# NCAR/SPERR

Hardware: AMD Instinct MI355X
Metric: compress+decompress GB/s/GPU on 256^3 fp32 chunks @ BPP=2.0; bitstream-exact vs ref (higher is better)
Workload: dtype f64; 1 GPU; synthetic 1024^3 fp32 turbulence per GPU, 256^3 chunks, BPP=2.0, step = compress + decompress, volume and container resident in HBM; chunks_per_gpu=64, parallelism=chunks farmed over 1 GPU(s), no collective

## Files before the change

sperr_amd/csrc/engine.hip:

```cpp
#include <algorithm>
#include <array>
#include <chrono>
#include <cstdlib>
#include <cstring>
#include <atomic>
#include <deque>
#include <map>
#include <memory>
#include <condition_variable>
#include <mutex>
#include <numeric>
#include <thread>
#include <string>
#include <vector>

#include "../../include/sperr_hip.h"
#include "engine_internal.h"
#include "host_container.hpp"
#include "speck_dec.h"
#include "dequant.h"
#include "speck_enc.h"
#include "speck_tree_host.hpp"
#include "outlier.h"
#include "quality.h"
// ... 87 lines not shown

void prof_begin(const char* name, hipStream_t stream)
{
  Profiler* P = t_prof;
  if (!P || !P->on || (!P->only.empty() && P->only != name))
    return;
  std::lock_guard<std::mutex> lock(P->mu);
  if (!P->ref) {
    P->ref = P->get();
    if (P->ref)
      hipEventRecord(P->ref, stream);
  }
  t_prof_cur = name;
  t_prof_a = P->get();
  if (t_prof_a)
    hipEventRecord(t_prof_a, stream);
}

void prof_end(hipStream_t stream)
{
  Profiler* P = t_prof;
  if (!P || !P->on || !t_prof_cur)
    return;
  std::lock_guard<std::mutex> lock(P->mu);
  hipEvent_t b = P->get();
  if (b)
    hipEventRecord(b, stream);
  P->open.push_back({t_prof_cur, t_prof_a, b});
  t_prof_cur = nullptr;
}

thread_local bool t_shared_device = false;

namespace {

struct DevBuf {
  void* p = nullptr;
  size_t n = 0;
  void drop()
  {
    if (p)
      (void)hipFree(p);
    p = nullptr;
    n = 0;
  }
  int ensure(size_t bytes)
  {
    if (bytes <= n)
      return 0;
    if (p)
      (void)hipFree(p);
    p = nullptr;
    n = 0;
    size_t want = bytes < (size_t(256) << 20) ? bytes + bytes / 4 + 4096 : bytes;
    if (want != bytes && hipMalloc(&p, want) != hipSuccess) {
      (void)hipGetLastError();
      p = nullptr;
      want = bytes;
    }
    if (!p)
      HIP_CHECK(hipMalloc(&p, want));
    n = want;
    return 0;
  }
};

std::atomic<unsigned long long> g_dbg_counter[4];

struct Arena {
  char* base = nullptr;
  size_t cap = 0, used = 0;
  template <typename T>
  T* take(size_t count)
  {
    if (used > cap || count > (cap - used) / sizeof(T))
      return nullptr;
    const size_t bytes = (count * sizeof(T) + 255) / 256 * 256;
    if (bytes > cap - used)
      return nullptr;
    T* r = reinterpret_cast<T*>(base + used);
    used += bytes;
    return r;
  }
};

inline uint64_t bytes_of_bits(uint64_t bits)
{
  return bits / 8 + (bits % 8 != 0);
}

size_t round_up(size_t v, size_t m)
{
  return (v + m - 1) / m * m;
}

using hostc::Dims;
using hostc::chunk_count;
using hostc::box_chunks;
using hostc::chunk_volume;
using hostc::ContainerInfo;
using hostc::parse_container_host;
using hostc::keep_portion;

uint32_t condi_num_strides(size_t len)
{
  const size_t dflt = 2048;
  if (len % dflt == 0)
    return (uint32_t)dflt;
  for (size_t n = dflt; n <= 32768; n++)
    if (len % n == 0)
      return (uint32_t)n;
  size_t n = dflt;
  while (len % n != 0)
    n--;
  return (uint32_t)n;
}

struct LiftPass {
  int axis;
  uint32_t region[3];
};

struct ShapePlan {
  uint32_t dims[3];
  uint32_t N = 0;
  spk::HostTree ht;
  spk::Tree dtree{};
  DevBuf tables;
  const uint64_t* d_initLIS = nullptr;
  const uint32_t* d_initLen = nullptr;
  const uint32_t* d_levelOff = nullptr;
  const uint16_t* d_tileLevel = nullptr;
  const uint32_t* d_tileStart = nullptr;
  const uint32_t* d_levelFirstTile = nullptr;
  const uint32_t* d_levelNumTiles = nullptr;
  const uint32_t* d_depthBlocks = nullptr;
  const uint8_t* d_levelSlot = nullptr;
  const uint64_t* d_iRoots = nullptr;
  const uint8_t* d_slotLevel = nullptr;
  const spk::LevelClass* d_levelClass = nullptr;
  const uint32_t* d_wordLeaf = nullptr;
  const FusedRoot* d_fusedRoots = nullptr;
  const uint8_t* d_mxSlot = nullptr;
  const uint8_t* d_mxLevelGroup = nullptr;
  int l0Level = -1;
  int l1Level = -1;
  int l2Level = -1;
  int maxK = 0;
  std::vector<uint32_t> depthBlockOff;
  uint32_t nListTiles = 0, nSlots = 0, nPixTiles = 0, nstrides = 0;
  uint64_t maxPhaseBits = 0;
  size_t lisEntries = 0;
  std::vector<LiftPass> fwd;
};
bool use_tables(const ShapePlan& P);


std::vector<FusedRoot> fused_head_roots(const spk::HostTree& h)
{
  std::vector<FusedRoot> out;
  const uint32_t dx = h.dims[0], dy = h.dims[1], dz = h.dims[2];
  if (!(h.flags & spk::kTreeAllOct) || (h.flags & spk::kTree2D) || h.roots.empty() || h.roots.size() > (size_t)spk::kMaxRoots)
    return out;
  if ((dx & (dx - 1)) != 0 || dx < 8 || dx > (uint32_t)kPixTile / 2 || ((size_t)dx * dy) % kPixTile != 0 || dz % 2 != 0)
    return out;
  uint64_t covered = 0;
  for (const spk::Root& r : h.roots) {
    const spk::Grid& g = h.grids[r.gridFirst + r.Dmax - 1];
    const uint32_t side = r.len[0];
    if (!(g.kind & spk::kGridOct) || g.e[0] < 2 || g.e[1] != g.e[0] || g.e[2] != g.e[0] || r.org[0] % 8 != 0 ||
        r.org[1] % 2 != 0 || r.org[2] % 2 != 0 || r.len[1] != side || r.len[2] != side || side != (2u << g.e[0]))
      return std::vector<FusedRoot>();
    out.push_back(FusedRoot{(uint32_t)r.org[0] | ((uint32_t)r.org[1] << 16), (uint32_t)r.org[2] | (side << 16), g.nodeOff, g.e[0]});
    covered += (uint64_t)side * side * side;
  }
  if (covered != (uint64_t)dx * dy * dz)
    return std::vector<FusedRoot>();
  return out;
}

struct Blob {
  std::vector<char> bytes;
  template <typename T>
  size_t add(const std::vector<T>& v)
  {
    const size_t off = round_up(bytes.size(), 256);
    bytes.resize(off + std::max<size_t>(v.size(), 1) * sizeof(T), 0);
    if (!v.empty())
      memcpy(bytes.data() + off, v.data(), v.size() * sizeof(T));
    return off;
  }
};

int build_plan(ShapePlan& P, size_t dx, size_t dy, size_t dz, bool twoD = false)
{
  const unsigned __int128 samples = (unsigned __int128)dx * dy * dz;
  if (dx == 0 || dy == 0 || dz == 0 || dx > 0xffff || dy > 0xffff || dz > 0xffff || samples > (1ull << 31)) {
    fprintf(stderr, "[sperr_hip] chunk of %zu x %zu x %zu not supported (at most 65535 per axis, 2^31 samples)\n",
            dx, dy, dz);
    return -1;
  }
  P.dims[0] = (uint32_t)dx;
  P.dims[1] = (uint32_t)dy;
  P.dims[2] = (uint32_t)dz;
  P.N = (uint32_t)(dx * dy * dz);
  P.ht = spk::build_tree(dx, dy, dz, twoD, false);
  P.maxK = 0;
  for (const auto& lc : P.ht.levelClass)
    P.maxK = std::max<int>(P.maxK, lc.K);
  if (!use_tables(P))
    spk::build_mx_columns(P.ht);
  const spk::HostTree& h = P.ht;
  const uint32_t nlev = h.nlevels;

  std::vector<uint32_t> cap(nlev), levelOff(nlev + 1, 0), initLen(nlev);
  for (uint32_t l = 0; l < nlev; l++) {
    cap[l] = std::max<uint32_t>(h.levelCap[l], (uint32_t)h.initLIS[l].size());
    levelOff[l + 1] = levelOff[l] + cap[l];
    initLen[l] = (uint32_t)h.initLIS[l].size();
  }
  P.lisEntries = levelOff[nlev] + 8;
  std::vector<uint64_t> initLIS(levelOff[nlev] ? levelOff[nlev] : 1, 0);
  for (uint32_t l = 0; l < nlev; l++)
    for (size_t k = 0; k < h.initLIS[l].size(); k++)
      initLIS[levelOff[l] + k] = h.initLIS[l][k];

  std::vector<uint16_t> tileLevel;
  std::vector<uint32_t> tileStart, levelFirstTile(nlev, 0), levelNumTiles(nlev, 0);
  for (uint32_t l = nlev; l-- > 0;) {
    levelFirstTile[l] = (uint32_t)tileLevel.size();
    const uint32_t nt = (cap[l] + kListTile - 1) / kListTile;
    levelNumTiles[l] = nt;
    for (uint32_t t = 0; t < nt; t++) {
      tileLevel.push_back((uint16_t)l);
      tileStart.push_back(t * kListTile);
    }
  }
  P.nListTiles = (uint32_t)tileLevel.size();

  std::vector<uint32_t> depthBlocks;
  P.depthBlockOff.assign(h.maxDepth + 1, 0);
  for (uint32_t d = 0; d < h.maxDepth; d++) {
    P.depthBlockOff[d] = (uint32_t)depthBlocks.size();
    for (uint32_t b = 0; b < h.blockGrid.size(); b++)
      if (h.grids[h.blockGrid[b]].depth == d)
        depthBlocks.push_back(b);
  }
  P.depthBlockOff[h.maxDepth] = (uint32_t)depthBlocks.size();

  std::vector<uint8_t> levelSlot(nlev, 0xff), slotLevel;
  for (uint32_t l = 0; l < nlev; l++)
    if (cap[l]) {
      levelSlot[l] = (uint8_t)slotLevel.size();
      slotLevel.push_back((uint8_t)l);
    }
  P.nSlots = (uint32_t)slotLevel.size();
  P.maxPhaseBits = (uint64_t)h.nsets + 2ull * P.N + 64;
  P.nPixTiles = (P.N + kPixTile - 1) / kPixTile;
  P.nstrides = condi_num_strides(P.N);

  std::vector<uint32_t> wordLeaf;
  for (const spk::Root& r : h.roots) {
    const spk::Grid& g = h.grids[r.gridFirst + r.Dmax - 1];
    if (!(g.kind & spk::kGridLeafWord))
      continue;
    if (wordLeaf.empty())
      wordLeaf.assign((P.N + 63) / 64, 0xffffffffu);
    for (uint32_t z = 0; z < r.len[2]; z++)
      for (uint32_t y = 0; y < r.len[1]; y++)
        for (uint32_t x = 0; x < r.len[0]; x += 64) {
          const size_t idx = ((size_t)(r.org[2] + z) * dy + r.org[1] + y) * dx + r.org[0] + x;
          const uint32_t fid = g.nodeOff + ((((z / 2) << g.e[1]) + y / 2) << g.e[0]) + x / 2;
          wordLeaf[idx / 64] = fid | (y & 1u) | ((z & 1u) << 1);
        }
  }

  Blob blob;
  const size_t oRoots = blob.add(h.roots), oGrids = blob.add(h.grids), oTab = blob.add(h.tab),
               oBG = blob.add(h.blockGrid), oInit = blob.add(initLIS), oInitLen = blob.add(initLen),
               oLevOff = blob.add(levelOff), oTL = blob.add(tileLevel), oTS = blob.add(tileStart),
               oLFT = blob.add(levelFirstTile), oLNT = blob.add(levelNumTiles),
               oDB = blob.add(depthBlocks), oLS = blob.add(levelSlot), oSL = blob.add(slotLevel),
               oLC = blob.add(h.levelClass), oWL = blob.add(wordLeaf), oCls = blob.add(h.cls),
               oGC = blob.add(h.gridCls), oIR = blob.add(h.iRoots),
               oMS = blob.add(h.mxSlot), oMG = blob.add(h.mxLevelGroup);
  const std::vector<FusedRoot> fusedRoots = twoD ? std::vector<FusedRoot>() : fused_head_roots(h);
  const size_t oFR = blob.add(fusedRoots);
  P.maxK = 0;
  for (const auto& lc : h.levelClass)
    P.maxK = std::max<int>(P.maxK, lc.K);
  P.l0Level = -1;
  for (uint32_t l = nlev; l-- > 0;) {
    if (cap[l] == 0)
      continue;
    if (h.allRegular && h.levelClass[l].regular && h.levelClass[l].K == 1 &&
        h.levelClass[l].arity[0] == 8)
      P.l0Level = (int)l;
    break;
  }
  P.l1Level = -1;
  if (P.l0Level >= 0)
    for (uint32_t l = (uint32_t)P.l0Level; l-- > 0;) {
      if (cap[l] == 0)
        continue;
      const spk::LevelClass& lc = h.levelClass[l];
      if (lc.regular && lc.K == 2 && lc.arity[0] == 8 && lc.arity[1] == 8 &&
          lc.lev[0] == (uint8_t)P.l0Level)
        P.l1Level = (int)l;
      break;
    }
  P.l2Level = -1;
  static const bool l2Env = !(getenv("SPERR_HIP_LIS_L2") && atoi(getenv("SPERR_HIP_LIS_L2")) == 0);
  if (P.l1Level >= 0 && l2Env)
    for (uint32_t l = (uint32_t)P.l1Level; l-- > 0;) {
      if (cap[l] == 0)
        continue;
      const spk::LevelClass& lc = h.levelClass[l];
      if (lc.regular && lc.K == 3 && lc.arity[0] == 8 && lc.arity[1] == 8 && lc.arity[2] == 8 &&
          lc.lev[0] == (uint8_t)P.l0Level && lc.lev[1] == (uint8_t)P.l1Level)
        P.l2Level = (int)l;
      break;
    }
  if (P.tables.ensure(blob.bytes.size()))
    return -1;
  HIP_CHECK(hipMemcpy(P.tables.p, blob.bytes.data(), blob.bytes.size(), hipMemcpyHostToDevice));
  char* base = static_cast<char*>(P.tables.p);
  P.dtree = h.view();
  P.dtree.roots = reinterpret_cast<const spk::Root*>(base + oRoots);
  P.dtree.grids = reinterpret_cast<const spk::Grid*>(base + oGrids);
  P.dtree.tab = reinterpret_cast<const uint16_t*>(base + oTab);
  P.dtree.blockGrid = reinterpret_cast<const uint16_t*>(base + oBG);
  P.dtree.cls = reinterpret_cast<const spk::ShapeCls*>(base + oCls);
  P.dtree.gridCls = reinterpret_cast<const uint8_t*>(base + oGC);
  P.d_mxSlot = reinterpret_cast<const uint8_t*>(base + oMS);
  P.d_mxLevelGroup = reinterpret_cast<const uint8_t*>(base + oMG);
  P.d_iRoots = h.iRoots.empty() ? nullptr : reinterpret_cast<const uint64_t*>(base + oIR);
  P.d_initLIS = reinterpret_cast<const uint64_t*>(base + oInit);
  P.d_initLen = reinterpret_cast<const uint32_t*>(base + oInitLen);
  P.d_levelOff = reinterpret_cast<const uint32_t*>(base + oLevOff);
  P.d_tileLevel = reinterpret_cast<const uint16_t*>(base + oTL);
  P.d_tileStart = reinterpret_cast<const uint32_t*>(base + oTS);
  P.d_levelFirstTile = reinterpret_cast<const uint32_t*>(base + oLFT);
  P.d_levelNumTiles = reinterpret_cast<const uint32_t*>(base + oLNT);
  P.d_depthBlocks = reinterpret_cast<const uint32_t*>(base + oDB);
  P.d_levelSlot = reinterpret_cast<const uint8_t*>(base + oLS);
  P.d_slotLevel = reinterpret_cast<const uint8_t*>(base + oSL);
  P.d_levelClass = reinterpret_cast<const spk::LevelClass*>(base + oLC);
  P.d_wordLeaf = wordLeaf.empty() ? nullptr : reinterpret_cast<const uint32_t*>(base + oWL);
  P.d_fusedRoots = fusedRoots.empty() ? nullptr : reinterpret_cast<const FusedRoot*>(base + oFR);

  P.fwd.clear();
  size_t levels = 0;
  auto approx = [](size_t len, size_t lev) { return (uint32_t)spk::approx_detail_len(len, lev)[0]; };
  if (spk::can_use_dyadic({dx, dy, dz}, levels)) {
    for (size_t lev = 0; lev < levels; lev++) {
      LiftPass ps{0, {approx(dx, lev), approx(dy, lev), approx(dz, lev)}};
      for (int a = 0; a < 3; a++) {
        ps.axis = a;
        P.fwd.push_back(ps);
      }
    }
  }
  else {
    const size_t nz = spk::num_of_xforms(dz), nxy = spk::num_of_xforms(std::min(dx, dy));
    for (size_t lev = 0; lev < nz; lev++)
      P.fwd.push_back({2, {(uint32_t)dx, (uint32_t)dy, approx(dz, lev)}});
    for (size_t lev = 0; lev < nxy; lev++) {
      P.fwd.push_back({0, {approx(dx, lev), approx(dy, lev), (uint32_t)dz}});
      P.fwd.push_back({1, {approx(dx, lev), approx(dy, lev), (uint32_t)dz}});
    }
  }
  return 0;
}

constexpr uint32_t kSubStreams = 8;

struct Engine {
  int dev = -1;
  bool busy = false;
  bool ready = false;
  Profiler prof;
  hipStream_t sub[kSubStreams] = {};
  hipEvent_t evFork = nullptr, evJoin[kSubStreams] = {};
  hipStream_t outl = nullptr;
  hipStream_t outlQ[kSubStreams] = {};
  hipStream_t sideQ[kSubStreams] = {};
  hipEvent_t evOutl[kSubStreams] = {}, evOutlFork[kSubStreams] = {};
  hipEvent_t evPweFork = nullptr;
  hipEvent_t evPweJoin = nullptr;
  std::map<Dims, std::unique_ptr<ShapePlan>> plans;
  std::vector<Dims> planOrder;
  DevBuf arena, slots, misc;
  DevBuf outlFixed, outlVar, outlStream;
  DevBuf pweBox;
  hipStream_t pweLastStream = nullptr;
  DevBuf outlDec[kSubStreams];
  DevBuf decBox[kSubStreams];
  uint32_t* liveHost[kSubStreams] = {};
  void* pweHost = nullptr;
  size_t pweHostBytes = 0;
  hipEvent_t liveEv[kSubStreams][kLiveSlots] = {};
  DevBuf wideScratch;
  std::vector<std::unique_ptr<DevBuf>> pweBufs;
  size_t freeMemAtInit = 0;

  int init()
  {
    if (ready)
      return 0;
    const int rc = init_handles();
    if (rc)
      destroy_handles();
    return rc;
  }
  void destroy_handles()
  {
    auto ds = [](hipStream_t& s) { if (s) (void)hipStreamDestroy(s); s = nullptr; };
    auto de = [](hipEvent_t& e) { if (e) (void)hipEventDestroy(e); e = nullptr; };
    for (uint32_t q = 0; q < kSubStreams; q++) {
      ds(sub[q]);
      de(evJoin[q]);
      if (q > 0)
        ds(outlQ[q]);
      ds(sideQ[q]);
      de(evOutl[q]);
      de(evOutlFork[q]);
      if (q == 0) {
        de(evPweFork);
        de(evPweJoin);
      }
      if (liveHost[q])
        (void)hipHostFree(liveHost[q]);
      liveHost[q] = nullptr;
      if (q == 0 && pweHost) {
        (void)hipHostFree(pweHost);
        pweHost = nullptr;
        pweHostBytes = 0;
      }
      for (int k = 0; k < kLiveSlots; k++)
        de(liveEv[q][k]);
    }
    de(evFork);
    ds(outl);
    outlQ[0] = nullptr;
    ready = false;
  }
  int init_handles()
  {
    size_t fr = 0, tot = 0;
    HIP_CHECK(hipMemGetInfo(&fr, &tot));
    freeMemAtInit = fr;
    for (uint32_t q = 0; q < kSubStreams; q++) {
      HIP_CHECK(hipStreamCreateWithFlags(&sub[q], hipStreamNonBlocking));
      HIP_CHECK(hipEventCreateWithFlags(&evJoin[q], hipEventDisableTiming));
    }
    HIP_CHECK(hipEventCreateWithFlags(&evFork, hipEventDisableTiming));
    int prLeast = 0, prGreatest = 0;
    if (hipDeviceGetStreamPriorityRange(&prLeast, &prGreatest) != hipSuccess) {
      (void)hipGetLastError();
      prLeast = prGreatest = 0;
    }
    static const int sidePrio = getenv("SPERR_HIP_SIDE_PRIORITY") ? atoi(getenv("SPERR_HIP_SIDE_PRIORITY")) : 1;
    const int prSide = sidePrio > 0 ? prGreatest : sidePrio < 0 ? prLeast : 0;
    HIP_CHECK(hipStreamCreateWithPriority(&outl, hipStreamNonBlocking, prSide));
    outlQ[0] = outl;
    for (uint32_t q = 1; q < kSubStreams; q++)
      HIP_CHECK(hipStreamCreateWithPriority(&outlQ[q], hipStreamNonBlocking, prSide));
    for (uint32_t q = 0; q < kSubStreams; q++)
      HIP_CHECK(hipStreamCreateWithFlags(&sideQ[q], hipStreamNonBlocking));
    for (uint32_t q = 0; q < kSubStreams; q++) {
      HIP_CHECK(hipEventCreateWithFlags(&evOutl[q], hipEventDisableTiming));
      HIP_CHECK(hipEventCreateWithFlags(&evOutlFork[q], hipEventDisableTiming));
    }
    HIP_CHECK(hipEventCreateWithFlags(&evPweFork, hipEventDisableTiming));
    HIP_CHECK(hipEventCreateWithFlags(&evPweJoin, hipEventDisableTiming));
    for (uint32_t q = 0; q < kSubStreams; q++) {
      HIP_CHECK(hipHostMalloc(reinterpret_cast<void**>(&liveHost[q]), kLiveSlots * sizeof(uint32_t), hipHostMallocDefault));
      for (int k = 0; k < kLiveSlots; k++)
        HIP_CHECK(hipEventCreateWithFlags(&liveEv[q][k], hipEventDisableTiming));
    }
    ready = true;
    return 0;
  }

  static constexpr size_t kMaxPlans = 64;
  ShapePlan* plan(size_t dx, size_t dy, size_t dz)
  {
    const Dims key{dx, dy, dz};
    auto it = plans.find(key);
    if (it != plans.end()) {
      auto pos = std::find(planOrder.begin(), planOrder.end(), key);
      if (pos != planOrder.end())
        planOrder.erase(pos);
      planOrder.push_back(key);
      return it->second.get();
    }
    auto p = std::make_unique<ShapePlan>();
    if (dz == 0 ? build_plan(*p, dx, dy, 1, true) : build_plan(*p, dx, dy, dz))
      return nullptr;
    ShapePlan* raw = p.get();
    plans[key] = std::move(p);
    planOrder.push_back(key);
    return raw;
  }
  void drop_memory()
  {
    for (auto& kv : plans)
      kv.second->tables.drop();
    plans.clear();
    planOrder.clear();
    for (DevBuf* b : {&arena, &slots, &misc, &outlFixed, &outlVar, &outlStream, &pweBox, &wideScratch})
      b->drop();
    for (auto& b : outlDec)
      b.drop();
    for (auto& b : decBox)
      b.drop();
    for (auto& b : pweBufs)
      if (b)
        b->drop();
    pweBufs.clear();
  }
  size_t device_bytes() const
  {
    size_t n = 0;
// ... 496 lines not shown
  memset(&e, 0, sizeof(e));
  e.tree = P.dtree;
  e.nchunks = B;
#define TAKE(dst, T, count)                                                            \
  dst = A.take<T>((size_t)(count));                                                    \
  if (!dst)                                                                            \
    return false;                                                                      \
  if (arena_debug())                                                                   \
    fprintf(stderr, "[sperr_hip] arena %-18s %10.2f MB\n", #dst, (double)((size_t)(count) * sizeof(T)) / 1048576.0);
  TAKE(e.cst, CoderState, B);
  TAKE(e.st, EncState, B);
  TAKE(o.geom, ChunkGeom, B);
  TAKE(o.gids, uint32_t, B);
  o.valsStride = Npad;
  TAKE(o.vals, double, Npad * B);
  o.strideMeanStride = round_up(std::max<size_t>(P.nstrides, P.N / 4096 + 2), 32);
  TAKE(o.strideMean, double, o.strideMeanStride * B);
  e.coefStride = Npad;
  TAKE(o.coef32, uint32_t, Npad * B);
  e.coef = o.coef32;
  e.signStride = Npad / 64;
  uint64_t* sign;
  TAKE(sign, uint64_t, e.signStride * B);
  e.sign = sign;
  e.pixStride = Npad;
  TAKE(o.msb, int8_t, Npad * B);
  e.msb = o.msb;
  TAKE(e.bplane, int8_t, Npad * B);
  {
    Arena over;
    over.base = reinterpret_cast<char*>(o.vals);
    over.cap = alias ? Npad * B * sizeof(double) : 0;
    const size_t before = A.used;
    o.fusedHead = enc_fused_head(P);
    if (!carve_enc_coder(over, &A, P, B, e, o.fusedHead))
      return false;
    o.aliased = over.used != 0;
    o.coderBytes = over.used + (A.used - before);
    if (arena_debug())
      fprintf(stderr, "[sperr_hip] arena %-18s %10.2f MB, %.2f MB of them over o.vals\n", "coder arrays",
              (double)o.coderBytes / 1048576.0, (double)over.used / 1048576.0);
  }
  e.lisStride = P.lisEntries;
  TAKE(e.lis[0], uint64_t, P.lisEntries * B);
  e.levelOff = P.d_levelOff;
  e.nListTiles = P.nListTiles;
  e.tileLevel = P.d_tileLevel;
  e.tileStart = P.d_tileStart;
  e.levelFirstTile = P.d_levelFirstTile;
  e.levelNumTiles = P.d_levelNumTiles;
  e.tileStride = round_up(P.nListTiles, 32);
  TAKE(e.tileBits, uint64_t, e.tileStride * B);
  TAKE(e.tileSurv, uint32_t, e.tileStride * B);
  TAKE(e.tileBitsOff, uint64_t, e.tileStride * B);
  TAKE(e.tileSurvOff, uint32_t, e.tileStride * B);
  e.iRoots = P.d_iRoots;
  e.iLevels = P.ht.iLevels;
  e.levelSlot = P.d_levelSlot;
  e.slotLevel = P.d_slotLevel;
  e.nSlots = P.nSlots;
  e.maskWords = (uint32_t)maskWords;
  e.maskStride = (size_t)P.nSlots * maskWords;
  TAKE(e.mask, uint64_t, std::max<size_t>(e.maskStride, 1) * B);
  e.prefWords = (uint32_t)((maskWords + 3) / 4);
  e.prefStride = (size_t)P.nSlots * e.prefWords;
  TAKE(e.maskPrefix, uint32_t, std::max<size_t>(e.prefStride, 1) * B);
  e.nPixTiles = P.nPixTiles;
  e.pixCntStride = (size_t)kMaxPlanes * 2 * P.nPixTiles;
  TAKE(e.pixCnt, uint32_t, e.pixCntStride * B);
  TAKE(e.pixOff, uint32_t, e.pixCntStride * B);
  e.streamStride = streamWords;
  TAKE(e.stream, uint64_t, streamWords * B);
#undef TAKE
  return true;
}

size_t enc_bytes_for(const ShapePlan& P, uint32_t B, uint64_t raw_budget, bool alias = true)
{
  Arena probe;
  probe.base = reinterpret_cast<char*>(uintptr_t(4096));
  probe.cap = ~size_t(0) / 2;
  EncBatchBufs tmp;
  carve_enc(probe, P, std::max<uint32_t>(B, 1), raw_budget, tmp, alias);
  return probe.used;
}
size_t enc_bytes_per_chunk(const ShapePlan& P, uint64_t raw_budget, bool alias = true)
{
  return enc_bytes_for(P, 1, raw_budget, alias);
}

int reset_enc_pass(hipStream_t st, const EncBatchBufs& bb, uint32_t B, bool fusedHead = false)
{
  const EncBuffers& e = bb.eb;
  if (!fusedHead)
    HIP_CHECK(hipMemsetAsync(e.bplane, 0xff, e.pixStride * B, st));
  HIP_CHECK(hipMemsetAsync(e.M, 0xff, e.nodeStride * B, st));
  HIP_CHECK(hipMemsetAsync(e.mask, 0, std::max<size_t>(e.maskStride, 1) * B * sizeof(uint64_t), st));
  HIP_CHECK(hipMemsetAsync(e.stream, 0, e.streamStride * B * sizeof(uint64_t), st));
  return 0;
}

bool fuse_xy(const ShapePlan& P)
{
  if (P.fwd.size() < 2 || P.fwd[0].axis != 0 || P.fwd[1].axis != 1)
    return false;
  for (int a = 0; a < 3; a++)
    if (P.fwd[0].region[a] != P.dims[a] || P.fwd[1].region[a] != P.dims[a])
      return false;
  return lift_xy_applicable(P.dims);
}

bool fuse_xyz(const ShapePlan& P)
{
  if (!fuse_xy(P) || P.fwd.size() < 3 || P.fwd[2].axis != 2)
    return false;
  for (int a = 0; a < 3; a++)
    if (P.fwd[2].region[a] != P.dims[a])
      return false;
  return lift_xyz_applicable(P.dims);
}

int pass_fuse(const ShapePlan& P, size_t k, uint32_t inner[3])
{
  const LiftPass& ps = P.fwd[k];
  inner[0] = inner[1] = inner[2] = 0;
  for (size_t j = k + 1; j < P.fwd.size(); j++)
    for (int a = 0; a < 3; a++)
      inner[a] = std::max(inner[a], P.fwd[j].region[a]);
  bool nested = k + 1 >= P.fwd.size();
  for (size_t j = k + 1; j < P.fwd.size(); j++)
    nested = nested || (P.fwd[j].region[0] == inner[0] && P.fwd[j].region[1] == inner[1] &&
                        P.fwd[j].region[2] == inner[2]);
  if (!nested)
    return -1;
  bool covers = true;
  for (int a = 0; a < 3; a++)
    covers = covers && inner[a] >= ps.region[a];
  return covers ? 0 : 1;
}

bool plan_fusable(const ShapePlan& P)
{
  if (P.fwd.empty())
    return false;
  uint32_t inner[3];
  for (size_t k = 0; k < P.fwd.size(); k++)
    if (pass_fuse(P, k, inner) < 0)
      return false;
  if (fuse_xy(P) && (pass_fuse(P, 0, inner) != 0 || pass_fuse(P, 1, inner) != 0))
    return false;
  return true;
}

template <typename T>
int float_stages(hipStream_t ss, const ShapePlan& P, EncBatchBufs& bb, uint32_t nb, const uint32_t cd[3],
                 const T* d_src, VolDesc vd, bool orgAligned, bool wantRange)
{
  EncBuffers& e = bb.eb;
  const bool fuse = !P.fwd.empty();
  const int io = std::is_same<T, float>::value ? 1 : 2;
  if (launch_condition<T>(ss, d_src, vd, bb.geom, nb, cd, P.nstrides, bb.strideMean, bb.strideMeanStride,
                          bb.vals, bb.valsStride, e.cst, !fuse, wantRange, orgAligned))
    return -1;
  size_t k0 = 0;
  const bool fuseMax = plan_fusable(P);
  if (fuse_xyz(P)) {
    LiftFuse lf;
    if (fuseMax && pass_fuse(P, 2, lf.inner) > 0)
      lf.mode = 1;
    if (launch_lift_xyz(ss, true, bb.vals, bb.valsStride, nb, cd, e.cst, io, const_cast<T*>(d_src), vd,
                        bb.geom, &lf))
      return -1;
    k0 = 3;
  }
  else if (fuse_xy(P)) {
    if (launch_lift_xy(ss, true, bb.vals, bb.valsStride, nb, cd, e.cst, io, const_cast<T*>(d_src), vd,
                       bb.geom))
      return -1;
    k0 = 2;
  }
  for (size_t k = k0; k < P.fwd.size(); k++) {
    const LiftPass& ps = P.fwd[k];
    LiftFuse lf;
    if (fuseMax && pass_fuse(P, k, lf.inner) > 0)
      lf.mode = 1;
    if (launch_lift(ss, true, bb.vals, bb.valsStride, nb, cd, ps.axis, ps.region, e.cst, k == 0 ? io : 0,
                    const_cast<T*>(d_src), vd, bb.geom, &lf))
      return -1;
  }
  return 0;
}

int unalias_coder(hipStream_t ss, Engine& E, const ShapePlan& P, EncBatchBufs& bb, uint32_t nb)
{
  HIP_CHECK(hipStreamSynchronize(ss));
  if (E.wideScratch.ensure(bb.coderBytes + 4096))
    return -1;
  Arena W;
  W.base = static_cast<char*>(E.wideScratch.p);
  W.cap = E.wideScratch.n;
  if (!carve_enc_coder(W, nullptr, P, nb, bb.eb))
    return -1;
  bb.aliased = false;
  return 0;
}

template <typename T>
int wide_retry_prepare(hipStream_t ss, Engine& E, const ShapePlan& P, EncBatchBufs& bb, uint32_t nb,
                       const uint32_t cd[3], const T* d_src, VolDesc vd, bool orgAligned, bool wantRange)
{
  if (unalias_coder(ss, E, P, bb, nb))
    return -1;
  g_dbg_counter[0]++;
  return float_stages<T>(ss, P, bb, nb, cd, d_src, vd, orgAligned, wantRange);
}

int psnr_q_search(hipStream_t st, const ShapePlan& P, EncBatchBufs& bb, uint32_t nb, double psnr,
                  std::vector<CoderState>& hc, std::vector<CoderState>& got)
{
  EncBuffers& e = bb.eb;
  hc.assign(nb, CoderState{});
  HIP_CHECK(hipMemcpyAsync(hc.data(), e.cst, nb * sizeof(CoderState), hipMemcpyDeviceToHost, st));
  HIP_CHECK(hipStreamSynchronize(st));
  std::vector<double> tmse(nb, 0.0);
  bool any = false;
  for (uint32_t i = 0; i < nb; i++) {
    CoderState& c = hc[i];
    c.mse_active = 0;
    if (c.is_const)
      continue;
    const double vmax = order_key_value(c.vmaxKey), vmin = -order_key_value(c.vnegmaxKey);
    const double range = (vmax - c.mean) - (vmin - c.mean);
    tmse[i] = (range * range) * std::pow(10.0, -psnr / 10.0);
    c.q = 2.0 * std::sqrt(tmse[i] * 3.0);
    if (!(c.q > 0.0))
      return -1;
    c.mse_active = 1;
    any = true;
  }
  const double step = std::exp2(0.25);
  while (any) {
    HIP_CHECK(hipMemcpyAsync(e.cst, hc.data(), nb * sizeof(CoderState), hipMemcpyHostToDevice, st));
    if (launch_mse(st, bb.vals, bb.valsStride, nb, P.N, bb.strideMean, bb.strideMeanStride, e.cst))
      return -1;
    got.assign(nb, CoderState{});
    HIP_CHECK(hipMemcpyAsync(got.data(), e.cst, nb * sizeof(CoderState), hipMemcpyDeviceToHost, st));
    HIP_CHECK(hipStreamSynchronize(st));
    any = false;
    for (uint32_t i = 0; i < nb; i++) {
      if (!hc[i].mse_active)
        continue;
      if (got[i].mse > tmse[i]) {
        hc[i].q /= step;
        any = true;
      }
      else
        hc[i].mse_active = 0;
    }
  }
  for (uint32_t i = 0; i < nb; i++) {
    CoderState& c = hc[i];
    c.mse_active = 0;
    c.wide = 0;
    c.need_retry = 0;
    if (c.is_const)
      continue;
    const double m = c.maxabs / c.q;
    if (!(m < 0x1p63))
      return -1;
    c.need_retry = std::llrint(m) > (long long)0xffffffffll ? 1u : 0u;
  }
  HIP_CHECK(hipMemcpyAsync(e.cst, hc.data(), nb * sizeof(CoderState), hipMemcpyHostToDevice, st));
  HIP_CHECK(hipStreamSynchronize(st));
  return 0;
}

struct HostMarks {
  bool on = getenv("SPERR_HIP_TIMING") != nullptr;
  std::chrono::steady_clock::time_point t0 = std::chrono::steady_clock::now();
  void mark(const char* what, hipStream_t st)
  {
    if (!on)
      return;
    (void)hipStreamSynchronize(st);
    const auto t1 = std::chrono::steady_clock::now();
    fprintf(stderr, "[sperr_hip] %-28s %8.2f ms\n", what,
            std::chrono::duration<double, std::milli>(t1 - t0).count());
    t0 = t1;
  }
};

int pwe_q_setup(hipStream_t st, EncBatchBufs& bb, uint32_t nb, double tol, std::vector<CoderState>& hc, bool* anyWide = nullptr)
{
  EncBuffers& e = bb.eb;
  hc.assign(nb, CoderState{});
  HIP_CHECK(hipMemcpyAsync(hc.data(), e.cst, nb * sizeof(CoderState), hipMemcpyDeviceToHost, st));
  HIP_CHECK(hipStreamSynchronize(st));
  for (uint32_t i = 0; i < nb; i++) {
    CoderState& c = hc[i];
    c.wide = 0;
    c.need_retry = 0;
    if (c.is_const)
      continue;
    c.q = 1.5 * tol;
    const double m = c.maxabs / c.q;
    if (!(m < 0x1p63))
      return -1;
    c.need_retry = std::llrint(m) > (long long)0xffffffffll ? 1u : 0u;
    if (anyWide && c.need_retry)
      *anyWide = true;
  }
  HIP_CHECK(hipMemcpyAsync(e.cst, hc.data(), nb * sizeof(CoderState), hipMemcpyHostToDevice, st));
  return 0;
}

struct PweKeep {
  void* mem = nullptr;
  uint32_t nb = 0;
  uint32_t* gids = nullptr;
  uint64_t* slotOff = nullptr;
  uint8_t* slots = nullptr;
  std::vector<uint64_t> off2;
};
using PweKeepList = std::vector<PweKeep>;

void speck1d_level_offsets(OutlierBufs& ob, uint32_t N, uint64_t most)
{
  ob.nlists = (uint32_t)spk::num_of_partitions(N) + 1;
  uint64_t off = 0;
  for (uint32_t l = 0; l <= (uint32_t)kO1MaxLevels; l++) {
    ob.levelOff[l] = (uint32_t)std::min<uint64_t>(off, 0xffffffffull);
    if (l < ob.nlists)
      off += l < 40 ? std::min<uint64_t>(1ull << l, most) : most;
  }
  ob.runStride = round_up((size_t)off + 64, 64);
}

struct PweStage {
  OutlierBufs ob;
  std::vector<OutlierChunk> hoc;
  std::vector<ChunkGeom> bricks;
  HostMarks hm;
};
static DequantSrc enc_dequant_src(const EncBatchBufs& bb, bool wide)
{
  DequantSrc s;
  s.coef = wide ? static_cast<const void*>(bb.vals) : bb.coef32;
  s.coefStride = wide ? bb.valsStride : bb.eb.coefStride;
  s.sign = bb.eb.sign;
  s.signStride = bb.eb.signStride;
  return s;
}
template <typename T>
int pwe_stage_begin(hipStream_t st, Engine& E, const ShapePlan& P, EncBatchBufs& bb, uint32_t nb,
                    const T* d_src, VolDesc vd, const uint32_t cd[3], double tol, bool anyWide, PweStage& S)
{
  EncBuffers& e = bb.eb;
  HostMarks& hm = S.hm;
  OutlierBufs& ob = S.ob;
  std::vector<OutlierChunk>& hoc = S.hoc;
  std::vector<ChunkGeom>& bricks = S.bricks;
  if (E.pweLastStream) {
    HIP_CHECK(hipStreamSynchronize(E.pweLastStream));
    E.pweLastStream = nullptr;
  }
  hm.mark("(3D coder done)", st);
  bricks.assign(nb, ChunkGeom{});
// ... 753 lines not shown
    d_bytes = reinterpret_cast<uint8_t*>(d_at + arr / 8);
    std::vector<uint8_t> hdr(at[nvol]);
    HIP_CHECK(hipMemcpyAsync(d_off, off.data(), nvol * 8, hipMemcpyHostToDevice, st));
    HIP_CHECK(hipMemcpyAsync(d_len, need.data(), nvol * 8, hipMemcpyHostToDevice, st));
    HIP_CHECK(hipMemcpyAsync(d_at, at.data(), nvol * 8, hipMemcpyHostToDevice, st));
    LAUNCH_K(k_gather_bytes, dim3(4, std::min<uint32_t>(n, 65535u)), dim3(kThreads), 0, st, d_src, d_off, d_len, d_at,
             d_bytes, n);
    HIP_CHECK(hipMemcpyAsync(hdr.data(), d_bytes, hdr.size(), hipMemcpyDeviceToHost, st));
    HIP_CHECK(hipStreamSynchronize(st));
    for (size_t v = 0; v < nvol; v++) {
      size_t nd = 0;
      if (need[v] && parse_container_host(hdr.data() + at[v], need[v], len[v], ci[v], &nd) != 0)
        return -1;
    }
  }
  return 0;
}

int read_batch_info(Engine& E, const uint8_t* d_src, const size_t* offs, size_t nvol, ContainerInfo& all,
                    std::vector<std::array<size_t, 6>>& list, hipStream_t st)
{
  std::vector<ContainerInfo> ci;
  std::vector<uint8_t> heads;
  if (read_batch_headers(E, d_src, offs, nvol, ci, heads, st))
    return -1;
  const Dims vol = ci[0].vol;
  for (size_t v = 1; v < nvol; v++)
    if (ci[v].vol != vol)
      return -1;
  if (nvol > 0xffffffffull / vol[2] || ci[0].nvals > SIZE_MAX / 8 / nvol)
    return -1;
  all.vol = {vol[0], vol[1], vol[2] * nvol};
  all.chunk = ci[0].chunk;
  all.nvals = ci[0].nvals * nvol;
  all.off.clear();
  all.len.clear();
  list.clear();
  for (size_t v = 0; v < nvol; v++) {
    const auto per = chunk_volume(ci[v].vol, ci[v].chunk);
    if (per.size() != ci[v].off.size() || list.size() + per.size() > 0xffffffffull)
      return -1;
    for (size_t i = 0; i < per.size(); i++) {
      auto c = per[i];
      c[4] += v * vol[2];
      list.push_back(c);
      all.off.push_back(offs[v] + ci[v].off[i]);
      all.len.push_back(ci[v].len[i]);
    }
  }
  return 0;
}

int trunc_impl(Engine& E, const uint8_t* d_src, const size_t* offs, size_t nvol, unsigned pct, uint8_t* d_dst,
               size_t dst_cap, size_t* outOffs, hipStream_t st)
{
  std::vector<ContainerInfo> ci;
  std::vector<uint8_t> heads;
  if (read_batch_headers(E, d_src, offs, nvol, ci, heads, st))
    return -1;
  const bool whole = pct == 0 || pct >= 100;
  size_t npieces = 0, hdrBytes = 0;
  for (const ContainerInfo& c : ci) {
    npieces += 1 + c.len.size();
    hdrBytes += (c.multi ? 20 : 14) + 4 * c.len.size();
  }
  if (npieces >= 0xffffffffull)
    return -1;
  const size_t addrBytes = round_up(npieces * 8, 256), offBytes = round_up((npieces + 1) * 8, 256);
  if (E.misc.ensure(addrBytes + offBytes + hdrBytes + 256))
    return -1;
  uint8_t* d_up = static_cast<uint8_t*>(E.misc.p);
  std::vector<uint8_t> up(addrBytes + offBytes + hdrBytes, 0);
  uint64_t* srcAddr = reinterpret_cast<uint64_t*>(up.data());
  uint64_t* outOff = reinterpret_cast<uint64_t*>(up.data() + addrBytes);
  uint8_t* hdr = up.data() + addrBytes + offBytes;
  size_t k = 0, hat = 0;
  uint64_t out = 0;
  for (size_t v = 0; v < nvol; v++) {
    const ContainerInfo& c = ci[v];
    const size_t pos = c.multi ? 20 : 14, hlen = pos + 4 * c.len.size();
    uint8_t* h = hdr + hat;
    memcpy(h, heads.data() + v * 32, pos);
    if (!whole) {
      h[0] = 0;
      h[1] |= 0x80;
    }
    outOffs[v] = (size_t)out;
    srcAddr[k] = reinterpret_cast<uint64_t>(d_up + addrBytes + offBytes + hat);
    outOff[k++] = out;
    out += hlen;
    for (size_t i = 0; i < c.len.size(); i++) {
      const uint32_t keep = (uint32_t)hostc::portion_len((size_t)c.len[i], pct);
      memcpy(h + pos + 4 * i, &keep, 4);
      srcAddr[k] = reinterpret_cast<uint64_t>(d_src + offs[v] + c.off[i]);
      outOff[k++] = out;
      out += keep;
    }
    hat += hlen;
  }
  outOff[k] = out;
  outOffs[nvol] = (size_t)out;
  if (!d_dst || out > dst_cap)
    return 1;
  const uintptr_t s0 = reinterpret_cast<uintptr_t>(d_src) + offs[0], s1 = reinterpret_cast<uintptr_t>(d_src) + offs[nvol];
  const uintptr_t d0 = reinterpret_cast<uintptr_t>(d_dst), d1 = d0 + out;
  if (s0 < d1 && d0 < s1)
    return -1;
  const uint64_t nblocks = (out + kTruncSlice - 1) / kTruncSlice;
  if (nblocks > 0x7fffffffull)
    return -1;
  HIP_CHECK(hipMemcpyAsync(d_up, up.data(), up.size(), hipMemcpyHostToDevice, st));
  LAUNCH_K(k_trunc_container, dim3((uint32_t)nblocks), dim3(kThreads), 0, st, d_dst,
           reinterpret_cast<const uint64_t*>(d_up), reinterpret_cast<const uint64_t*>(d_up + addrBytes), (uint32_t)npieces,
           out);
  HIP_CHECK(hipGetLastError());
  HIP_CHECK(hipStreamSynchronize(st));
  E.prof.collect();
  return 0;
}

bool g_lis_stamps_on = false;
constexpr int kHiMaxK = 9;
bool use_lis_hi(const ShapePlan& P, bool tables)
{
  static const bool hiEnv = !(getenv("SPERR_HIP_LIS_HI") && atoi(getenv("SPERR_HIP_LIS_HI")) == 0);
  return hiEnv && tables && P.ht.grids.size() <= 288 && P.ht.roots.size() <= 48 &&
         P.maxK >= 1 && P.maxK <= kHiMaxK;
}
bool use_tables(const ShapePlan& P)
{
  if (!P.ht.allRegular || P.maxK < 1)
    return false;
  return use_lis_hi(P, true);
}
bool use_mixed(const ShapePlan& P)
{
  static const bool mixEnv = !(getenv("SPERR_HIP_LIS_MIXED") && atoi(getenv("SPERR_HIP_LIS_MIXED")) == 0);
  const bool twoD = (P.ht.flags & spk::kTree2D) != 0;
  if ((!twoD && !mixEnv) || use_tables(P) || P.ht.cls.empty() || P.ht.roots.size() > 48 || P.ht.grids.size() > 352 ||
      P.ht.mxSlot.size() != P.ht.cls.size())
    return false;
  return 2 * kMxS + 256 <= kMxRing && ((kMxS + kMxM) >> 6) + 5 <= 64 && kMxM >= 192 &&
         mx_smem_bytes(kMxS, kMxM, kMxQ) <= 138u * 1024u;
}
std::vector<uint64_t> g_lis_stamps_host;

struct DecBatchBufs {
  DecBuffers db;
  ChunkGeom* geom;
  CropGeom* crop;
  uint64_t *chunkOff, *chunkLen;
  double* vals;
  size_t valsStride;
  uint32_t* coef32;
  uint32_t* live;
};

bool carve_dec(Arena& A, const ShapePlan& P, uint32_t B, uint64_t maxPayloadBytes, DecBatchBufs& o,
               size_t valsElems = 0, uint32_t refNPlanes = 0, bool crop = false)
{
  const size_t N = P.N, Npad = round_up(N, 512);
  DecBuffers& d = o.db;
  memset(&d, 0, sizeof(d));
  d.tree = P.dtree;
  d.treeTabLen = (uint32_t)P.ht.tab.size();
  d.nchunks = B;
#define TAKE(dst, T, count)                                                            \
  dst = A.take<T>((size_t)(count));                                                    \
  if (!dst)                                                                            \
    return false;                                                                      \
  if (arena_debug())                                                                   \
    fprintf(stderr, "[sperr_hip] arena %-18s %10.2f MB\n", #dst, (double)((size_t)(count) * sizeof(T)) / 1048576.0);
  TAKE(d.cst, CoderState, B);
  TAKE(d.st, DecState, B);
  TAKE(o.geom, ChunkGeom, B);
  o.crop = nullptr;
  if (crop) {
    TAKE(o.crop, CropGeom, B);
  }
  TAKE(o.chunkOff, uint64_t, B);
  TAKE(o.chunkLen, uint64_t, B);
  TAKE(o.live, uint32_t, 64);
  o.valsStride = valsElems ? round_up(valsElems, 256) : Npad;
  TAKE(o.vals, double, o.valsStride * B);
  d.coefStride = Npad;
  TAKE(o.coef32, uint32_t, Npad * B);
  d.coef = o.coef32;
  d.signStride = Npad / 64;
  TAKE(d.sign, uint64_t, d.signStride * B);
  d.maskPixStride = Npad / 64;
  d.refPlanes = nullptr;
  d.refMask = nullptr;
  d.wordTop = nullptr;
  d.refNPlanes = 0;
  d.refPlaneStride = d.wordTopStride = 0;
  if (refNPlanes) {
    d.refNPlanes = std::min<uint32_t>(refNPlanes, 32u);
    d.refPlaneStride = d.coefStride / 2;
    d.wordTopStride = round_up(d.maskPixStride, 64);
    d.refPlanes = reinterpret_cast<uint64_t*>(o.coef32);
    TAKE(d.refMask, uint64_t, d.maskPixStride * B);
    TAKE(d.wordTop, uint8_t, d.wordTopStride * B);
  }
  TAKE(d.bornM, uint64_t, d.maskPixStride * B);
  TAKE(d.sigOld, uint64_t, d.maskPixStride * B);
  TAKE(d.sigNew, uint64_t, d.maskPixStride * B);
  d.lisStride = P.lisEntries;
  TAKE(d.lis[0], uint64_t, P.lisEntries * B);
  TAKE(d.lis[1], uint64_t, P.lisEntries * B);
  d.levelOff = P.d_levelOff;
  d.nPixTiles = (uint32_t)((Npad / 64 + kThreads - 1) / kThreads);
  d.tileStride = round_up(d.nPixTiles, 32);
  TAKE(d.tileLip, uint32_t, d.tileStride * B);
  TAKE(d.tileRef, uint32_t, d.tileStride * B);
  TAKE(d.tileLipOff, uint32_t, d.tileStride * B);
  TAKE(d.tileRefOff, uint32_t, d.tileStride * B);
  {
    uint8_t* tb = nullptr;
    TAKE(tb, uint8_t, d.tileStride * B);
    d.tileBorn = use_tables(P) ? tb : nullptr;
  }
  d.lipResStride = Npad / 64 + 2;
  TAKE(d.lipSig, uint64_t, d.lipResStride * B);
  TAKE(d.lipNeg, uint64_t, d.lipResStride * B);
  d.tokStride = (2 * N + 1 + 63) / 64 + 2;
  TAKE(d.tokMask, uint64_t, d.tokStride * B);
  TAKE(d.tokCnt, uint32_t, d.tokStride * B);
  TAKE(d.tokOff, uint32_t, d.tokStride * B);
  d.tokSegStride = round_up(d.tokStride / 2048 + 2, 32);
  TAKE(d.tokSegSum, uint32_t, d.tokSegStride * B);
  TAKE(d.tokSegBase, uint32_t, d.tokSegStride * B);
  d.streamStride = (size_t)(maxPayloadBytes / 8) + 4;
  TAKE(d.stream, uint64_t, d.streamStride * B);
  d.levelClass = P.d_levelClass;
  d.levelSlot = P.d_levelSlot;
  d.slotLevel = P.d_slotLevel;
  d.nSlots = P.nSlots;
  d.maskWords = (uint32_t)d.streamStride;
  d.maskStride = (size_t)P.nSlots * d.maskWords;
  TAKE(d.mask, uint64_t, std::max<size_t>(d.maskStride, 1) * B);
  d.prefWords = (d.maskWords + 3u) / 4u;
  d.prefStride = (size_t)P.nSlots * d.prefWords;
  TAKE(d.maskPrefix, uint32_t, std::max<size_t>(d.prefStride, 1) * B);
  d.bornStride = P.ht.nsets + 8;
  d.hiGroupsMax = 8;
  d.bornSeg = (uint32_t)((P.ht.nsets + 8) / 16 + 64);
  d.bornPitch = d.bornStride + (size_t)d.bornSeg * d.hiGroupsMax;
  TAKE(d.bornPacked, uint64_t, d.bornPitch * B);
  TAKE(d.bornPosLev, uint64_t, d.bornPitch * B);
  d.lisStamps = nullptr;
  if (g_lis_stamps_on) {
    TAKE(d.lisStamps, uint64_t, 64 * B);
  }
  d.queueCap = 28672 + 64;
  static const int hiKcap = tune_getenv("SPERR_HIP_HI_KCAP") ? std::max(2, atoi(tune_getenv("SPERR_HIP_HI_KCAP"))) : 5;
  d.hiK = (uint32_t)std::min(std::max(2, P.maxK), hiKcap);
  static const uint32_t ahead = tune_getenv("SPERR_HIP_HI_AHEAD") ? (uint32_t)atoi(tune_getenv("SPERR_HIP_HI_AHEAD")) : 512u;
  d.hiAhead = ahead;
  static const uint32_t extra = tune_getenv("SPERR_HIP_HI_EXTRA") ? (uint32_t)atoi(tune_getenv("SPERR_HIP_HI_EXTRA")) : 1u;
  d.hiExtra = extra;
  d.hiHop2 = 0;
  d.hiCand = 1;
  d.hiSmemBytes = 148 * 1024;
  d.hiW = hi_window((int)d.hiK, d.hiSmemBytes, d.hiHop2);
  d.queueStride = (size_t)d.queueCap * 4 * d.hiGroupsMax;
  TAKE(d.queue, uint64_t, d.queueStride * B);
  d.hiAhead = std::min(d.hiAhead / 64 * 64, d.hiW / 2);
  d.hiFlagStride = ((d.streamStride * 64 + N) / std::max<uint32_t>(512u, d.hiW - d.hiAhead) + 12) * 4;
  d.mxSlot = P.d_mxSlot;
  d.mxLevelGroup = P.d_mxLevelGroup;
  d.mxS = kMxS;
  d.mxM = kMxM;
  d.mxQ = kMxQ;
  d.mxSmemBytes = mx_smem_bytes(kMxS, kMxM, kMxQ);
  if (use_mixed(P))
    d.hiFlagStride = std::max<size_t>(d.hiFlagStride, ((d.streamStride * 64 + N) / kMxS + 4) * kMxWordsPerRegion);
  TAKE(d.hiFlags, unsigned long long, d.hiFlagStride * B);
  d.iRoots = P.d_iRoots;
  d.iLevels = P.ht.iLevels;
  d.leafCap = P.ht.nsets + 8;
  d.leafSeg = (uint32_t)((P.ht.nsets + 8) / 16 + 64);
  d.leafStride = d.leafCap + (size_t)d.leafSeg * d.hiGroupsMax;
  TAKE(d.leafEv, uint64_t, d.leafStride * B);
  d.sigbitsStride = P.lisEntries / 64 + 4;
  TAKE(d.sigbits, uint64_t, d.sigbitsStride * B);
  d.l0FlagStride = (d.streamStride * 64 + N) / 4096 + 4;
  TAKE(d.l0Flags, unsigned long long, d.l0FlagStride * B);
  TAKE(d.l0Tab, unsigned long long, d.l0FlagStride * 17 * B);
  d.l0Level = P.l0Level;
  TAKE(d.l1Flags, unsigned long long, d.l0FlagStride * B);
  d.l1Level = P.l1Level;
  TAKE(d.l2Flags, unsigned long long, d.l0FlagStride * B);
  d.l2Level = P.l2Level;
  d.wordLeaf = P.d_wordLeaf;
  d.leafStateStride = round_up(P.ht.nnodes, 64);
  TAKE(d.leafState, uint16_t, d.leafStateStride * B);
  d.leafDirtyStride = d.leafStateStride / 32 + 1;
  TAKE(d.leafDirty, uint8_t, d.leafDirtyStride * B);
#undef TAKE
  return true;
}

int reset_dec_call(const DecBuffers& d, uint32_t nb, hipStream_t ss)
{
  HIP_CHECK(hipMemsetAsync(d.cst, 0, nb * sizeof(CoderState), ss));
  HIP_CHECK(hipMemsetAsync(d.st, 0, nb * sizeof(DecState), ss));
  HIP_CHECK(hipMemsetAsync(d.mask, 0, std::max<size_t>(d.maskStride, 1) * nb * 8, ss));
  HIP_CHECK(hipMemsetAsync(d.l0Flags, 0, d.l0FlagStride * nb * 8, ss));
  HIP_CHECK(hipMemsetAsync(d.l0Tab, 0, d.l0FlagStride * 17 * nb * 8, ss));
  HIP_CHECK(hipMemsetAsync(d.l1Flags, 0, d.l0FlagStride * nb * 8, ss));
  HIP_CHECK(hipMemsetAsync(d.l2Flags, 0, d.l0FlagStride * nb * 8, ss));
  HIP_CHECK(hipMemsetAsync(d.hiFlags, 0, d.hiFlagStride * nb * 8, ss));
  HIP_CHECK(hipMemsetAsync(d.sigbits, 0, d.sigbitsStride * nb * 8, ss));
  if (d.lisStamps)
    HIP_CHECK(hipMemsetAsync(d.lisStamps, 0, 64 * 8 * nb, ss));
  return 0;
}

int reset_dec_pass(const DecBatchBufs& bb, uint32_t nb, bool wide, hipStream_t ss)
{
  const DecBuffers& d = bb.db;
  HIP_CHECK(hipMemsetAsync(d.bornM, 0, d.maskPixStride * nb * 8, ss));
  if (d.tileBorn)
    HIP_CHECK(hipMemsetAsync(d.tileBorn, 0, d.tileStride * nb, ss));
  HIP_CHECK(hipMemsetAsync(d.sigOld, 0, d.maskPixStride * nb * 8, ss));
  HIP_CHECK(hipMemsetAsync(d.sigNew, 0, d.maskPixStride * nb * 8, ss));
  HIP_CHECK(hipMemsetAsync(d.sign, 0xff, d.signStride * nb * 8, ss));
  HIP_CHECK(hipMemsetAsync(d.leafState, 0, d.leafStateStride * nb * 2, ss));
  HIP_CHECK(hipMemsetAsync(d.leafDirty, 0, d.leafDirtyStride * nb, ss));
  HIP_CHECK(hipMemsetAsync(d.stream, 0, d.streamStride * nb * 8, ss));
  if (wide)
    HIP_CHECK(hipMemsetAsync(bb.vals, 0, bb.valsStride * nb * 8, ss));
  else if (d.refPlanes)
    HIP_CHECK(hipMemsetAsync(d.wordTop, 0, d.wordTopStride * nb, ss));
  else
    HIP_CHECK(hipMemsetAsync(bb.coef32, 0, d.coefStride * nb * 4, ss));
  return 0;
// ... 59 lines not shown
  std::vector<uint32_t> ids;
  bool crop = false;
  bool level = false;
  size_t h = 0;
  MultiRes m;
  void place(const uint32_t org[3], const uint32_t cd[3], size_t o[3], size_t ext[3]) const
  {
    for (int a = 0; a < 3; a++) {
      ext[a] = level ? m.cres[h][a] : cd[a];
      o[a] = level ? org[a] / cd[a] * ext[a] : org[a];
    }
  }
  CropGeom crop_geom(const size_t o[3], const size_t ext[3]) const
  {
    CropGeom g;
    for (int a = 0; a < 3; a++) {
      const size_t hi = lo[a] + dims[a];
      g.rel[a] = (int32_t)((int64_t)o[a] - (int64_t)lo[a]);
      g.lo[a] = (uint32_t)(lo[a] > o[a] ? lo[a] - o[a] : 0);
      g.hi[a] = (uint32_t)std::min<size_t>(hi - o[a], ext[a]);
    }
    return g;
  }
};

bool window_select(const Dims& full, const Dims& chunk, const size_t lo[3], const size_t dims[3], Window& w)
{
  for (int a = 0; a < 3; a++) {
    if (dims[a] > (size_t)INT32_MAX)
      return false;
    w.lo[a] = lo[a];
    w.dims[a] = dims[a];
  }
  w.crop = !(w.lo == Dims{0, 0, 0} && w.dims == full);
  return box_chunks(full, chunk, w.lo, w.dims, w.ids);
}

__global__ void __launch_bounds__(kThreads)
k_dequant_corner(double* vals, size_t valsStride, uint32_t bx, uint32_t by, uint32_t cx, uint32_t cy, uint32_t sx,
                 uint32_t sy, uint32_t sz, const CoderState* cst, DequantSrc Q)
{
  const uint32_t c = blockIdx.y;
  const CoderState& cs = cst[c];
  if (cs.is_const || cs.wide)
    return;
  const uint32_t i = blockIdx.x * kThreads + threadIdx.x;
  if (i >= sx * sy * sz)
    return;
  const uint32_t x = i % sx, r = i / sx;
  const uint32_t y = r % sy, z = r / sy;
  const size_t idx = ((size_t)z * cy + y) * cx + x;
  const DequantRule<uint32_t> rule = dequant_rule<uint32_t>(cs.q, true, Q.dst + c, Q.coefSigned != 0);
  const uint32_t v = Q.coefs<uint32_t>(c)[idx];
  double out;
  if (rule.scheme)
    out = dequant_signed(rule, v);
  else {
    const uint32_t w = (uint32_t)(idx >> 6), sh = (uint32_t)(idx & 63);
    const uint64_t sgw = Q.sign[c * Q.signStride + w];
    const uint64_t mnw = Q.sigNew[c * Q.maskStride + w], mow = Q.sigOld[c * Q.maskStride + w];
    out = dequant_masks(rule, v, mnw, mow, sgw, sh);
  }
  vals[c * valsStride + ((size_t)z * by + y) * bx + x] = out;
}

template <typename OT, bool kCrop>
__global__ void __launch_bounds__(kThreads)
k_level_write(const double* vals, size_t valsStride, const CoderState* cst, const GeomOf<kCrop>* geom, uint32_t bx,
              uint32_t by, uint32_t cdx, uint32_t cdy, uint32_t cdz, uint32_t sx, uint32_t sy, uint32_t sz,
              VolDesc vd, OT* out)
{
  const uint32_t c = blockIdx.y;
  const uint32_t n = sx * sy * sz, i0 = blockIdx.x * kThreads;
  const GeomOf<kCrop> g = geom[c];
  if constexpr (kCrop) {
    const uint32_t r0 = i0 / sx, r1 = (min(i0 + (uint32_t)kThreads, n) - 1) / sx;
    const uint32_t z0 = r0 / sy, y0 = r0 % sy, z1 = r1 / sy, y1 = r1 % sy;
    auto zin = [&](uint32_t z) { return z >= g.lo[2] && z < g.hi[2]; };
    auto ymeet = [&](uint32_t a, uint32_t b) { return a < g.hi[1] && b >= g.lo[1]; };
    bool any = zin(z0) && ymeet(y0, z1 > z0 ? sy - 1 : y1);
    any = any || (z1 > z0 && zin(z1) && ymeet(0, y1));
    any = any || (max(z0 + 1, g.lo[2]) < min(z1, g.hi[2]));
    if (!any)
      return;
  }
  const uint32_t i = i0 + threadIdx.x;
  if (i >= n)
    return;
  const uint32_t x = i % sx, r = i / sx;
  const uint32_t y = r % sy, z = r / sy;
  size_t o;
  if constexpr (kCrop) {
    if (x < g.lo[0] || x >= g.hi[0] || y < g.lo[1] || y >= g.hi[1] || z < g.lo[2] || z >= g.hi[2])
      return;
    o = ((size_t)((int64_t)g.rel[2] + z) * vd.dims[1] + (size_t)((int64_t)g.rel[1] + y)) * vd.dims[0] +
        (size_t)((int64_t)g.rel[0] + x);
  }
  else
    o = (((size_t)(g.org[2] / cdz) * sz + z) * vd.dims[1] + (size_t)(g.org[1] / cdy) * sy + y) * vd.dims[0] +
        (size_t)(g.org[0] / cdx) * sx + x;
  const CoderState& cs = cst[c];
  const double v = cs.is_const ? cs.mean : vals[c * valsStride + ((size_t)z * by + y) * bx + x] + cs.mean;
  out[o] = (OT)v;
}

struct DecodeRequest {
  using ChunkList = std::vector<std::array<size_t, 6>>;
  const ChunkList* stacked = nullptr;
  bool slices = false;
  const uint32_t* sliceHdr = nullptr;
  const Window* window = nullptr;
  const MultiRes* levels = nullptr;

  void set_window(const Window& w) { window = (w.level || w.crop) ? &w : nullptr; }

  bool valid() const
  {
    if (window && slices)
      return false;
    if (window && levels)
      return false;
    if (stacked && levels)
      return false;
    if (level() && stacked)
      return false;
    if (level() && level()->h >= level()->m.nlev)
      return false;
    return true;
  }

  const Window* level() const { return window && window->level ? window : nullptr; }
  bool cropped() const { return window && window->crop; }
  bool reads_outliers() const { return !level(); }
  ChunkList chunks(const ContainerInfo& ci) const { return stacked ? *stacked : chunk_volume(ci.vol, ci.chunk); }
  std::vector<uint32_t> slots(size_t nchunks) const
  {
    if (window)
      return window->ids;
    std::vector<uint32_t> sel(nchunks);
    std::iota(sel.begin(), sel.end(), 0u);
    return sel;
  }
  VolDesc out_desc(const ContainerInfo& ci) const
  {
    return window ? VolDesc{{window->dims[0], window->dims[1], window->dims[2]}}
                  : VolDesc{{ci.vol[0], ci.vol[1], ci.vol[2]}};
  }
  size_t out_vals(const ContainerInfo& ci) const
  {
    return window ? window->dims[0] * window->dims[1] * window->dims[2] : ci.nvals;
  }
};

size_t dec_bytes_per_chunk(const ShapePlan& P, uint64_t maxPayload, size_t valsElems, uint32_t refNPlanes, bool crop)
{
  Arena probe;
  probe.base = reinterpret_cast<char*>(uintptr_t(4096));
  probe.cap = ~size_t(0) / 2;
  DecBatchBufs tmp;
  carve_dec(probe, P, 1, maxPayload, tmp, valsElems, refNPlanes, crop);
  return probe.used;
}

DecPlanHost dec_plan_host(const ShapePlan& P)
{
  DecPlanHost ph{P.d_initLIS, P.d_initLen, use_tables(P), P.l0Level >= 0 && P.ht.grids.size() <= 288,
                 P.l1Level >= 0 && P.ht.grids.size() <= 288, P.maxK};
  ph.l2 = ph.l1 && P.l2Level >= 0;
  ph.hi = use_lis_hi(P, ph.tables);
  ph.mixed = use_mixed(P);
  return ph;
}

template <typename T>
struct DecodeCall {
  struct Ref {
    uint32_t gid;
    uint32_t slot;
    uint32_t org[3];
  };
  struct OutHead {
    bool has = false;
    uint64_t off = 0, total_bits = 0;
    int nbp = 0;
  };
  struct SubHost {
    std::vector<ChunkGeom> hg, bricks;
    std::vector<CropGeom> hc;
    std::vector<uint64_t> ho, hl;
    std::vector<DecState> hs;
    std::vector<OutlierChunk> hoc;
    DecBatchBufs bb;
    OutlierBufs ob;
    uint32_t nb = 0;
    size_t first = 0;
    int maxNarrow = 0, maxWide = 0;
    bool outliers = false;
  };
  struct Batch {
    const std::vector<Ref>* refs;
    ShapePlan* P;
    uint32_t cbox[3], refNPlanes, nsub = 1;
    uint64_t maxPayload = 0;
    size_t compactElems;
    bool deferG, fuseDq;
    hipStream_t deferStream = nullptr;
    std::vector<SubHost>* subs = nullptr;
    int devId = 0;
  };
  Engine& E;
  const uint8_t* d_src;
  T* d_dst;
  const ContainerInfo& ci;
  hipStream_t st;
  const DecodeRequest& req;
  const VolDesc vd = req.out_desc(ci);
  std::vector<uint32_t> sel;
  std::vector<uint64_t> selOff, selLen, tailOff, tailLen;
  std::vector<uint8_t> heads, tails;
  std::vector<OutHead> outHead;
  bool anyOutlier = false;
  std::map<Dims, std::vector<Ref>> groups;
  uint32_t mxGroupsCall = 0;
  std::deque<std::vector<SubHost>> subHosts;
  bool deferOK = false, deferSized = false, deferForked = false;
  std::vector<SubHost*> pending;
  size_t deferOff = 0;
  uint32_t deferNext = 0;
  hipEvent_t timingFork = nullptr;
  std::vector<std::pair<hipEvent_t, std::array<uint32_t, 4>>> timingEnds;
  bool ok = false;
  ~DecodeCall() { if (!ok) drain_after_error(E, st); }
  int run(size_t dst_cap_vals)
  {
    if (!req.valid())
      return -1;
    const auto chunks = req.chunks(ci);
    sel = req.slots(chunks.size());
    const uint32_t nchunks = (uint32_t)sel.size();
    const size_t outVals = req.out_vals(ci);
    if (outVals == 0 || outVals > dst_cap_vals || nchunks == 0)
      return -1;
    for (uint32_t i = 0; i < nchunks; i++) {
      const auto& c = chunks[sel[i]];
      selOff.push_back(ci.off[sel[i]]);
      selLen.push_back(ci.len[sel[i]]);
      groups[Dims{c[1], c[3], c[5]}].push_back({sel[i], i, {(uint32_t)c[0], (uint32_t)c[2], (uint32_t)c[4]}});
    }
    if (read_heads())
      return -1;
    deferOK = !anyOutlier && !req.levels && !req.slices && groups.size() > 1;
    count_mx_groups();
    for (int pass = 0; pass < 2; pass++)
      for (auto& g : groups)
        if (decode_group(g.first, g.second, pass))
          return -1;
    if (drain())
      return -1;
    HIP_CHECK(hipStreamSynchronize(st));
    HIP_CHECK(hipGetLastError());
    E.prof.collect();
    ok = true;
    return 0;
  }
  int read_heads()
  {
    const uint32_t nchunks = (uint32_t)sel.size();
    if (E.misc.ensure(round_up((size_t)nchunks * 8, 256) * 4 + (size_t)nchunks * 64 + 256))
      return -1;
    uint64_t* d_off = reinterpret_cast<uint64_t*>(E.misc.p);
    uint64_t* d_len = d_off + round_up(nchunks, 32);
    uint64_t* d_hoff = d_len + round_up(nchunks, 32);
    uint64_t* d_hlen = d_hoff + round_up(nchunks, 32);
    uint8_t* d_heads = reinterpret_cast<uint8_t*>(d_hlen + round_up(nchunks, 32));
    auto gather = [&](const std::vector<uint64_t>& off, const std::vector<uint64_t>& len, std::vector<uint8_t>& out,
                      bool withHdr) -> int {
      HIP_CHECK(hipMemcpyAsync(d_off, off.data(), nchunks * 8, hipMemcpyHostToDevice, st));
      HIP_CHECK(hipMemcpyAsync(d_len, len.data(), nchunks * 8, hipMemcpyHostToDevice, st));
      LAUNCH_K(k_gather_heads, dim3((nchunks + 63) / 64), dim3(64), 0, st, d_src, d_off, d_len, d_heads, nchunks);
      std::vector<uint64_t> hoff, hlen;
      if (withHdr) {
        hoff.resize(nchunks);
        hlen.assign(nchunks, 10);
        for (uint32_t i = 0; i < nchunks; i++)
          hoff[i] = off[i] - 10;
        HIP_CHECK(hipMemcpyAsync(d_hoff, hoff.data(), nchunks * 8, hipMemcpyHostToDevice, st));
        HIP_CHECK(hipMemcpyAsync(d_hlen, hlen.data(), nchunks * 8, hipMemcpyHostToDevice, st));
        LAUNCH_K(k_gather_heads, dim3((nchunks + 63) / 64), dim3(64), 0, st, d_src, d_hoff, d_hlen,
                 d_heads + (size_t)nchunks * 32, nchunks);
      }
      out.resize((size_t)nchunks * (withHdr ? 64 : 32));
      HIP_CHECK(hipMemcpyAsync(out.data(), d_heads, out.size(), hipMemcpyDeviceToHost, st));
      HIP_CHECK(hipStreamSynchronize(st));
      return 0;
    };
    if (gather(selOff, selLen, heads, req.sliceHdr != nullptr))
      return -1;
    if (const uint32_t* sliceHdr = req.sliceHdr)
      for (uint32_t i = 0; i < nchunks; i++) {
        uint32_t d2[2];
        memcpy(d2, heads.data() + (size_t)(nchunks + i) * 32 + 2, 8);
        if (d2[0] != sliceHdr[0] || d2[1] != sliceHdr[1]) {
          fprintf(stderr, "[sperr_hip] slice %u of the batch: its header says %u x %u, the call %u x %u\n", i, d2[0], d2[1],
                  sliceHdr[0], sliceHdr[1]);
          return -1;
        }
      }
    outHead.resize(nchunks);
    tailOff.assign(nchunks, 0);
    tailLen.assign(nchunks, 0);
    bool anyTail = false;
    if (!req.reads_outliers())
      return 0;
    for (uint32_t i = 0; i < nchunks; i++) {
      const uint8_t* hd = heads.data() + (size_t)i * 32;
      if (selLen[i] < 26 || (hd[0] & 0x01))
        continue;
      uint64_t tb;
      memcpy(&tb, hd + 18, 8);
      const uint64_t speckLen = std::min<uint64_t>(9 + bytes_of_bits(tb), selLen[i] - 17);
      if (17 + speckLen + 9 <= selLen[i]) {
        tailOff[i] = selOff[i] + 17 + speckLen;
        tailLen[i] = selLen[i] - 17 - speckLen;
        anyTail = true;
      }
    }
    if (!anyTail)
      return 0;
    if (gather(tailOff, tailLen, tails, false))
      return -1;
    for (uint32_t i = 0; i < nchunks; i++) {
      if (tailLen[i] < 9)
        continue;
      const uint8_t* t = tails.data() + (size_t)i * 32;
      uint64_t ob;
      memcpy(&ob, t + 1, 8);
      if (tailLen[i] != 9 + bytes_of_bits(ob))
        continue;
      outHead[i].has = true;
      outHead[i].off = tailOff[i];
      outHead[i].total_bits = ob;
      outHead[i].nbp = t[0];
      anyOutlier = true;
    }
    return 0;
  }
  ShapePlan* plan_of(const Dims& d) { return E.plan(d[0], d[1], req.slices ? 0 : d[2]); }
  void count_mx_groups()
  {
    size_t nmx = 0;
    for (auto& h : groups) {
      ShapePlan* Q = plan_of(h.first);
      if (Q && use_mixed(*Q))
        nmx += h.second.size();
    }
    static const uint32_t mxBudget = getenv("SPERR_HIP_MX_WGS") ? (uint32_t)atoi(getenv("SPERR_HIP_MX_WGS")) : 208u;
    size_t sharers = 1;
    int devNow = 0;
    if (hipGetDevice(&devNow) == hipSuccess)
      sharers = std::max<size_t>(1, g_pool.busy_on(devNow));
    if (nmx)
      mxGroupsCall = std::min<uint32_t>(8u, std::max<uint32_t>(2u, (uint32_t)(mxBudget / (nmx * sharers))));
  }
  static bool deferrable(const ShapePlan& P, size_t nchunksOfShape) { return nchunksOfShape < 32 || !use_tables(P); }
  uint32_t ref_planes_of(const ShapePlan& P, const std::vector<Ref>& refs) const
  {
    uint32_t n = 0;
    for (const Ref& r : refs) {
      const uint8_t* hd = heads.data() + (size_t)r.slot * 32;
      if (ci.len[r.gid] >= 26 && !(hd[0] & 0x01) && hd[17] <= 32)
        n = std::max<uint32_t>(n, hd[17]);
    }
    return n;
  }
  size_t compact_box(const ShapePlan& P, const std::vector<Ref>& refs, uint32_t cbox[3]) const
  {
    cbox[0] = cbox[1] = cbox[2] = 0;
    if (!fuse_xyz(P) || !plan_fusable(P) || req.levels || req.slices || anyOutlier || P.fwd.size() < 3)
      return 0;
    for (const Ref& r : refs) {
      const uint8_t* hd = heads.data() + (size_t)r.slot * 32;
      if (ci.len[r.gid] >= 26 && !(hd[0] & 0x01) && hd[17] > 32)
        return 0;
    }
    for (size_t k = 3; k < P.fwd.size(); k++)
      for (int a = 0; a < 3; a++)
        cbox[a] = std::max(cbox[a], P.fwd[k].region[a]);
    for (int a = 0; a < 3; a++)
      cbox[a] = std::max(cbox[a], 1u);
    if (const Window* lvl = req.level())
      for (int a = 0; a < 3; a++)
        cbox[a] = std::max(cbox[a], lvl->m.cres[lvl->h][a]);
    return (size_t)cbox[0] * cbox[1] * cbox[2];
  }
  int size_deferred()
  {
    deferSized = true;
    size_t sum = 0;
    for (auto& h : groups) {
      ShapePlan* Q = E.plan(h.first[0], h.first[1], h.first[2]);
      if (!Q)
        return -1;
      if (!deferrable(*Q, h.second.size()))
        continue;
      uint64_t mp = 0;
      for (auto& r : h.second)
        mp = std::max<uint64_t>(mp, ci.len[r.gid]);
      uint32_t qbox[3];
      sum += round_up(h.second.size() * dec_bytes_per_chunk(*Q, mp, compact_box(*Q, h.second, qbox), ref_planes_of(*Q, h.second), req.cropped()) + (1 << 20), 4096);
    }
    size_t fr = 0, tot = 0;
    HIP_CHECK(hipMemGetInfo(&fr, &tot));
    const size_t room = arena_room(E.arena.n, fr);
    return E.arena.ensure(std::min(sum, room)) ? -1 : 0;
  }
  int decode_group(const Dims& shape, const std::vector<Ref>& refs, int pass)
  {
    ShapePlan* P = plan_of(shape);
    if (!P)
      return -1;
    if (req.slices && !use_mixed(*P)) {
      fprintf(stderr, "[sperr_hip] slice of %u x %u: its forest does not fit k_lis_mx\n", P->dims[0], P->dims[1]);
      return -1;
    }
    Batch b{&refs, P};
    b.deferG = deferOK && deferrable(*P, refs.size());
    if (b.deferG != (pass == 1))
      return 0;
    if (b.deferG && !deferSized && size_deferred())
      return -1;
    for (auto& r : refs)
      b.maxPayload = std::max<uint64_t>(b.maxPayload, ci.len[r.gid]);
    b.compactElems = compact_box(*P, refs, b.cbox);
    b.refNPlanes = ref_planes_of(*P, refs);
    b.fuseDq = plan_fusable(*P) && !req.levels && !req.slices;
    const size_t per = dec_bytes_per_chunk(*P, b.maxPayload, b.compactElems, b.refNPlanes, req.cropped());
    size_t fr = 0, tot = 0;
    HIP_CHECK(hipMemGetInfo(&fr, &tot));
    const size_t budgetBytes = arena_budget(E.arena.n, fr);
    uint32_t B = (uint32_t)std::min<size_t>(refs.size(), std::max<size_t>(1, budgetBytes / per));
    B = std::min<uint32_t>(B, 256);
    const size_t needBytes = (size_t)B * per + (1 << 20);
    if (b.deferG && deferOff + needBytes > E.arena.n && drain())
      return -1;
    if (E.arena.ensure(needBytes))
      return -1;
    for (size_t b0 = 0; b0 < refs.size(); b0 += B) {
      const uint32_t nbAll = (uint32_t)std::min<size_t>(B, refs.size() - b0);
      if (b.deferG && deferOff + needBytes > E.arena.n && drain())
        return -1;
      if (decode_batch(b, b0, nbAll, needBytes))
        return -1;
    }
    return 0;
  }
  int decode_batch(Batch& b, size_t b0, uint32_t nbAll, size_t needBytes)
  {
    Arena A;
    A.base = static_cast<char*>(E.arena.p) + (b.deferG ? deferOff : 0);
    A.cap = E.arena.n - (b.deferG ? deferOff : 0);
    b.deferStream = nullptr;
    if (b.deferG) {
      if (!deferForked) {
        HIP_CHECK(hipEventRecord(E.evFork, st));
        for (uint32_t q = 0; q < kSubStreams; q++)
          HIP_CHECK(hipStreamWaitEvent(E.sub[q], E.evFork, 0));
        HIP_CHECK(hipStreamWaitEvent(E.outlQ[1], E.evFork, 0));
        deferForked = true;
      }
      b.deferStream = (mxGroupsCall != 0 && use_tables(*b.P)) ? E.outlQ[1] : E.sub[deferNext++ % kSubStreams];
      deferOff += round_up(needBytes, 4096);
    }
    if (pick_sub_batches(b, A, b0, nbAll))
      return -1;
    std::vector<SubHost>& subs = *b.subs;
    if (b.nsub == 1) {
      static const bool enqTiming = getenv("SPERR_HIP_ENQ_TIMING") != nullptr;
      const auto tq0 = std::chrono::steady_clock::now();
      if (enqueue(b, 0))
        return -1;
      if (enqTiming) {
        fprintf(stderr, "[sperr_hip] group %u x %u x %u, %u chunks: enqueued in %.2f ms\n", b.P->dims[0], b.P->dims[1], b.P->dims[2], nbAll,
                std::chrono::duration<double, std::milli>(std::chrono::steady_clock::now() - tq0).count());
        hipEvent_t evEnd = nullptr;
        if (b.deferStream && hipEventCreate(&evEnd) == hipSuccess) {
          if (!timingFork && hipEventCreate(&timingFork) == hipSuccess)
            (void)hipEventRecord(timingFork, st);
          (void)hipEventRecord(evEnd, b.deferStream);
          timingEnds.push_back({evEnd, {b.P->dims[0], b.P->dims[1], b.P->dims[2], nbAll}});
        }
      }
      if (b.deferG) {
        pending.push_back(&subs[0]);
        return 0;
      }
    }
    else {
      std::vector<int> rc(b.nsub, 0);
      std::vector<std::thread> workers;
      for (uint32_t q = 0; q < b.nsub; q++)
        workers.emplace_back([&, q]() { rc[q] = enqueue(b, q); });
      for (auto& w : workers)
        w.join();
      for (uint32_t q = 0; q < b.nsub; q++) {
        if (rc[q])
          return -1;
        if (subs[q].nb)
          HIP_CHECK(hipStreamWaitEvent(st, E.evJoin[q], 0));
      }
    }
    return collect_states(b);
  }
  int pick_sub_batches(Batch& b, Arena& A, size_t b0, uint32_t nbAll)
  {
    static const int subEnv = getenv("SPERR_HIP_SUBSTREAMS") ? atoi(getenv("SPERR_HIP_SUBSTREAMS")) : 0;
    uint32_t nsub = nbAll >= 32 ? 2u : 1u;
    int devNow = 0;
    if (!t_shared_device && hipGetDevice(&devNow) == hipSuccess && g_pool.busy_on(devNow) <= 1)
      nsub = nbAll >= 56 ? 3u : nbAll >= 8 ? 4u : nbAll >= 4 ? 2u : 1u;
    if (subEnv > 0)
      nsub = std::min<uint32_t>(kSubStreams, (uint32_t)subEnv);
    if (nbAll < 2 * nsub || b.deferG)
      nsub = 1;
    b.nsub = nsub;
    b.subs = &subHosts.emplace_back(nsub);
    if (nsub > 1) {
      HIP_CHECK(hipEventRecord(E.evFork, st));
      for (uint32_t q = 0; q < nsub; q++)
        HIP_CHECK(hipStreamWaitEvent(E.sub[q], E.evFork, 0));
    }
    uint32_t done = 0;
    for (uint32_t q = 0; q < nsub; q++) {
      SubHost& S = (*b.subs)[q];
      S.nb = (nbAll - done + (nsub - q) - 1) / (nsub - q);
      S.first = b0 + done;
      done += S.nb;
      if (S.nb && !carve_dec(A, *b.P, S.nb, b.maxPayload, S.bb, b.compactElems, b.refNPlanes, req.cropped()))
        return -1;
      if (S.nb && b.compactElems)
        g_dbg_counter[2]++;
    }
    HIP_CHECK(hipGetDevice(&b.devId));
    return 0;
  }
  int enqueue(const Batch& b, uint32_t q)
  {
    SubHost& S = (*b.subs)[q];
    const uint32_t nb = S.nb;
    if (nb == 0)
      return 0;
    if (b.nsub > 1) {
      HIP_CHECK(hipSetDevice(b.devId));
      t_prof = &E.prof;
    }
    const hipStream_t ss = b.deferStream ? b.deferStream : (b.nsub > 1 ? E.sub[q] : st);
    S.hg.resize(nb);
    S.ho.resize(nb);
    S.hl.resize(nb);
    for (uint32_t i = 0; i < nb; i++) {
      const Ref& r = (*b.refs)[S.first + i];
      for (int a = 0; a < 3; a++)
        S.hg[i].org[a] = r.org[a];
      S.ho[i] = ci.off[r.gid];
      S.hl[i] = ci.len[r.gid];
      const uint8_t* hd = heads.data() + (size_t)r.slot * 32;
      if (S.hl[i] >= 26 && !(hd[0] & 0x01)) {
        const int nbp = hd[17];
        if (nbp > 32)
          S.maxWide = std::max(S.maxWide, nbp);
        else
          S.maxNarrow = std::max(S.maxNarrow, nbp);
      }
      S.outliers |= outHead[r.slot].has;
    }
    if (S.maxWide > kMaxPlanes || (b.compactElems && S.maxWide))
      return -1;
    if (enqueue_outlier_decode(b, S, q, ss) || enqueue_lists(b, S, q, ss) || enqueue_inverse(b, S, q, ss))
      return -1;
    if (b.nsub > 1)
      HIP_CHECK(hipEventRecord(E.evJoin[q], ss));
    return 0;
  }
  int enqueue_outlier_decode(const Batch& b, SubHost& S, uint32_t q, hipStream_t ss)
  {
    if (!S.outliers)
      return 0;
    const uint32_t nb = S.nb, N = b.P->N;
    hipStream_t so = E.outlQ[q];
    HIP_CHECK(hipEventRecord(E.evOutlFork[q], ss));
    HIP_CHECK(hipStreamWaitEvent(so, E.evOutlFork[q], 0));
    S.hoc.assign(nb, OutlierChunk{});
    memset(S.hoc.data(), 0, nb * sizeof(OutlierChunk));
    uint64_t maxBits = 0;
    int maxNbp = 1;
    for (uint32_t i = 0; i < nb; i++) {
      const OutHead& oh = outHead[(*b.refs)[S.first + i].slot];
      if (!oh.has)
        continue;
      S.hoc[i].has = 1;
      S.hoc[i].streamOff = oh.off;
      S.hoc[i].total_bits = oh.total_bits;
      S.hoc[i].nbp = oh.nbp;
      if (oh.nbp > kMaxPlanes)
        return -1;
      maxBits = std::max(maxBits, oh.total_bits);
      maxNbp = std::max(maxNbp, oh.nbp);
    }
    OutlierBufs& ob = S.ob;
    memset(&ob, 0, sizeof(ob));
    ob.nchunks = nb;
    ob.N = N;
    ob.nw = (N + 63) / 64;
    ob.wordStride = round_up((size_t)ob.nw + 2, 32);
    ob.kStride = round_up((size_t)std::min<uint64_t>(N, maxBits) + 1, 64);
    speck1d_level_offsets(ob, N, std::min<uint64_t>(maxBits + 2, 2ull * N));
    ob.streamStride = (size_t)(maxBits / 64) + 4;
    ob.planeStride = (size_t)maxNbp * ob.wordStride;
    const size_t bytes = round_up(nb * sizeof(OutlierChunk), 256) +
                         (size_t)nb * (ob.wordStride * 16 + ob.kStride * 5 + ob.runStride * 8 +
                                       ob.streamStride * 8 + ob.planeStride * 8) + 8192;
    if (E.outlDec[q].ensure(bytes))
      return -1;
    Arena OA;
    OA.base = static_cast<char*>(E.outlDec[q].p);
    OA.cap = E.outlDec[q].n;
    ob.oc = OA.take<OutlierChunk>(nb);
    ob.lip = OA.take<uint64_t>(nb * ob.wordStride);
    ob.lsp = OA.take<uint64_t>(nb * ob.wordStride);
    ob.runs = OA.take<uint64_t>(nb * ob.runStride);
    ob.stream = OA.take<uint64_t>(nb * ob.streamStride);
    ob.planeBits = OA.take<uint64_t>(nb * ob.planeStride);
    ob.pos = OA.take<uint32_t>(nb * ob.kStride);
    ob.sgn = OA.take<uint8_t>(nb * ob.kStride);
    if (!ob.oc || !ob.lip || !ob.lsp || !ob.runs || !ob.stream || !ob.planeBits || !ob.pos || !ob.sgn)
      return -1;
    HIP_CHECK(hipMemcpyAsync(ob.oc, S.hoc.data(), nb * sizeof(OutlierChunk), hipMemcpyHostToDevice, so));
    HIP_CHECK(hipMemsetAsync(ob.lip, 0, (size_t)nb * ob.wordStride * 16, so));
    if (launch_speck1d_decode(so, ob, d_src))
      return -1;
    HIP_CHECK(hipEventRecord(E.evOutl[q], so));
    return 0;
  }
  int enqueue_lists(const Batch& b, SubHost& S, uint32_t q, hipStream_t ss)
  {
    const ShapePlan& P = *b.P;
    const uint32_t nb = S.nb;
    DecBatchBufs& bb = S.bb;
    DecBuffers& d = bb.db;
    HIP_CHECK(hipMemcpyAsync(bb.geom, S.hg.data(), nb * sizeof(ChunkGeom), hipMemcpyHostToDevice, ss));
    if (req.cropped()) {
      S.hc.resize(nb);
      for (uint32_t i = 0; i < nb; i++) {
        size_t o[3], ext[3];
        req.window->place(S.hg[i].org, P.dims, o, ext);
        S.hc[i] = req.window->crop_geom(o, ext);
      }
      HIP_CHECK(hipMemcpyAsync(bb.crop, S.hc.data(), nb * sizeof(CropGeom), hipMemcpyHostToDevice, ss));
    }
    HIP_CHECK(hipMemcpyAsync(bb.chunkOff, S.ho.data(), nb * 8, hipMemcpyHostToDevice, ss));
    HIP_CHECK(hipMemcpyAsync(bb.chunkLen, S.hl.data(), nb * 8, hipMemcpyHostToDevice, ss));
    DecPlanHost ph = dec_plan_host(P);
    ph.skipFinish = true;
    ph.mxGroups = mxGroupsCall;
    if (!ph.tables && !ph.mixed) {
      static std::atomic<bool> warned{false};
      if (!warned.exchange(true))
        fprintf(stderr, "[sperr_hip] note: chunks of %u x %u x %u decode through the serial walk (k_lis_walk): their tree "
                        "(%zu grids, %zu roots) exceeds what the parallel list kernels hold in LDS -- expect it to be slow\n",
                b.P->dims[0], b.P->dims[1], b.P->dims[2], P.ht.grids.size(), P.ht.roots.size());
    }
    static const uint32_t gdivEnv = tune_getenv("SPERR_HIP_MX_GRID_DIV") ? (uint32_t)atoi(tune_getenv("SPERR_HIP_MX_GRID_DIV")) : 4u;
    ph.gridDiv = (b.deferStream && mxGroupsCall != 0 && groups.size() >= 4) ? std::max<uint32_t>(1u, gdivEnv) : 1u;
    ph.d_live = !b.deferStream ? bb.live : nullptr;
    ph.h_live = E.liveHost[q % kSubStreams];
    ph.liveEv = E.liveEv[q % kSubStreams];
    static const bool gpuWide = !(getenv("SPERR_HIP_LIS_GPUWIDE") && atoi(getenv("SPERR_HIP_LIS_GPUWIDE")) == 0);
    if (!gpuWide)
      ph.l0 = ph.l1 = ph.l2 = false;
    if (reset_dec_call(d, nb, ss))
      return -1;
    for (int wide = 1; wide >= 0; wide--) {
      if (wide && S.maxWide == 0)
        continue;
      if (reset_dec_pass(bb, nb, wide != 0, ss))
        return -1;
      DecBuffers dw = d;
      if (wide) {
        dw.coef = bb.vals;
        dw.coefStride = bb.valsStride;
        dw.refPlanes = nullptr;
      }
      else
        dw.coefSigned = packed_signs(b, bb, false) ? 1u : 0u;
      if (launch_speck_decode(ss, dw, ph, d_src, bb.chunkOff, bb.chunkLen, wide != 0, wide ? S.maxWide : S.maxNarrow))
        return -1;
      if ((wide || !b.fuseDq) &&
          launch_inv_quantize(ss, wide != 0, dequant_src(b, bb, wide != 0), nb, P.N, bb.vals, bb.valsStride, d.cst))
        return -1;
    }
    return 0;
  }
  DequantSrc dequant_src(const Batch& b, const DecBatchBufs& bb, bool wide) const
  {
    const DecBuffers& d = bb.db;
    DequantSrc s;
    s.coef = wide ? static_cast<const void*>(bb.vals) : bb.coef32;
    s.coefStride = wide ? bb.valsStride : d.coefStride;
    s.sign = d.sign;
    s.signStride = d.signStride;
    s.sigNew = d.sigNew;
    s.sigOld = d.sigOld;
    s.maskStride = d.maskPixStride;
    s.dst = d.st;
    s.coefSigned = packed_signs(b, bb, wide) ? 1 : 0;
    return s;
  }
  static bool packed_signs(const Batch& b, const DecBatchBufs& bb, bool wide) { return !wide && bb.db.refPlanes && b.fuseDq; }
  void pass_dequant(const Batch& b, const DecBatchBufs& bb, size_t k, LiftFuse& lf) const
  {
    if (b.fuseDq && pass_fuse(*b.P, k, lf.inner) > 0) {
      lf.mode = 2;
      lf.src = dequant_src(b, bb, false);
    }
    if (b.compactElems) {
      lf.bufx = b.cbox[0];
      lf.bufy = b.cbox[1];
    }
  }
  int enqueue_inverse(const Batch& b, SubHost& S, uint32_t q, hipStream_t ss)
  {
    if (const Window* lvl = req.level())
      return enqueue_level(b, S, ss, *lvl);
    const ShapePlan& P = *b.P;
    const uint32_t nb = S.nb;
    const uint32_t* cd = P.dims;
    DecBatchBufs& bb = S.bb;
    DecBuffers& d = bb.db;
    const int io = std::is_same<T, float>::value ? 1 : 2;
    const bool fxyz = fuse_xyz(P) && !S.outliers;
    const bool fxy = fuse_xy(P) && !S.outliers && !fxyz;
    const bool fbrick = S.outliers && fuse_xyz(P) && b.fuseDq && S.maxWide == 0 && P.fwd.size() >= 3 &&
                        b.compactElems == 0 && (uint64_t)nb * bb.valsStride <= 0xffffffffull;
    uint32_t bbox[3] = {1, 1, 1};
    double* boxVals = nullptr;
    size_t boxStride = 0;
    ChunkGeom* d_bricks = nullptr;
    if (fbrick) {
      for (size_t k = 3; k < P.fwd.size(); k++)
        for (int a = 0; a < 3; a++)
          bbox[a] = std::max(bbox[a], P.fwd[k].region[a]);
      boxStride = round_up((size_t)bbox[0] * bbox[1] * bbox[2], 64);
      const size_t geomOff = round_up((size_t)nb * boxStride * 8, 256);
      if (E.decBox[q].ensure(geomOff + (size_t)nb * sizeof(ChunkGeom) + 256))
        return -1;
      boxVals = static_cast<double*>(E.decBox[q].p);
      d_bricks = reinterpret_cast<ChunkGeom*>(static_cast<char*>(E.decBox[q].p) + geomOff);
      S.bricks.resize(nb);
      for (uint32_t i = 0; i < nb; i++) {
        S.bricks[i].org[0] = (uint32_t)((size_t)i * bb.valsStride);
        S.bricks[i].org[1] = S.bricks[i].org[2] = 0;
      }
      HIP_CHECK(hipMemcpyAsync(d_bricks, S.bricks.data(), nb * sizeof(ChunkGeom), hipMemcpyHostToDevice, ss));
    }
    const size_t perLevel = req.slices ? 2 : 3;
    auto sub_volume = [&](size_t k) -> int {
      const MultiRes* mr = req.levels;
      if (!mr || !mr->nlev)
        return 0;
      const size_t h = mr->nlev - (k / perLevel + 1);
      const auto& r = mr->cres[h];
      const uint32_t blocks = capped_blocks((r[0] * r[1] * r[2] + kThreads - 1) / kThreads, nb);
      LAUNCH_K(k_sub_volume, dim3(blocks, nb), dim3(kThreads), 0, ss, bb.vals, bb.valsStride, d.cst, bb.geom,
               cd[0], cd[1], cd[0], cd[1], cd[2], r[0], r[1], r[2], mr->grid[0], mr->grid[1], mr->d_level[h]);
      return 0;
    };
    auto dequant_fuse = [&](size_t k, LiftFuse& lf) {
      pass_dequant(b, bb, k, lf);
      if (fbrick) {
        lf.bufx = bbox[0];
        lf.bufy = bbox[1];
      }
    };
    for (size_t k = P.fwd.size(); k-- > ((fxyz || fbrick) ? 3u : fxy ? 2u : 0u);) {
      const LiftPass& ps = P.fwd[k];
      if (k % perLevel == perLevel - 1 && sub_volume(k))
        return -1;
      LiftFuse lf;
      dequant_fuse(k, lf);
      const bool last = k == 0 && !S.outliers;
      if (launch_lift(ss, false, fbrick ? boxVals : bb.vals, fbrick ? boxStride : bb.valsStride, nb, cd, ps.axis,
                      ps.region, d.cst, last ? io : 0, d_dst, vd, bb.geom, &lf, last ? bb.crop : nullptr))
        return -1;
    }
    if (fbrick) {
      LiftFuse lf;
      dequant_fuse(2, lf);
      lf.noMean = 1;
      const VolDesc brickVol{{cd[0], cd[1], cd[2]}};
      if (launch_lift_xyz(ss, false, boxVals, boxStride, nb, cd, d.cst, 2, bb.vals, brickVol, d_bricks, &lf))
        return -1;
    }
    if (fxyz) {
      if (sub_volume(2))
        return -1;
      LiftFuse lf;
      dequant_fuse(2, lf);
      if (launch_lift_xyz(ss, false, bb.vals, bb.valsStride, nb, cd, d.cst, io, d_dst, vd, bb.geom, &lf, bb.crop))
        return -1;
    }
    if (fxy && req.slices && sub_volume(1))
      return -1;
    if (fxy && launch_lift_xy(ss, false, bb.vals, bb.valsStride, nb, cd, d.cst, io, d_dst, vd, bb.geom, bb.crop))
      return -1;
    if (S.outliers) {
      HIP_CHECK(hipStreamWaitEvent(ss, E.evOutl[q], 0));
      if (launch_outlier_apply(ss, S.ob, d.cst, bb.vals, bb.valsStride))
        return -1;
      HIP_CHECK(hipMemcpyAsync(S.hoc.data(), S.ob.oc, nb * sizeof(OutlierChunk), hipMemcpyDeviceToHost, ss));
      HIP_CHECK(hipStreamSynchronize(ss));
      for (auto& o : S.hoc)
        if (o.error) {
          fprintf(stderr, "[sperr_hip] outlier decoder failed (code %u)\n", o.error);
          return -1;
        }
    }
    if ((P.fwd.empty() || S.outliers) &&
        launch_scatter<T>(ss, d_dst, vd, bb.geom, nb, cd, bb.vals, bb.valsStride, d.cst, bb.crop))
      return -1;
    return 0;
  }
  int enqueue_level(const Batch& b, SubHost& S, hipStream_t ss, const Window& lvl)
  {
    const ShapePlan& P = *b.P;
    const uint32_t nb = S.nb;
    const uint32_t* cd = P.dims;
    DecBatchBufs& bb = S.bb;
    DecBuffers& d = bb.db;
    const size_t h = lvl.h, nlev = lvl.m.nlev;
    if (P.fwd.size() != 3 * nlev)
      return -1;
    const uint32_t bx = b.compactElems ? b.cbox[0] : cd[0], by = b.compactElems ? b.cbox[1] : cd[1];
    const auto& r = lvl.m.cres[h];
    if (b.compactElems && (r[0] > b.cbox[0] || r[1] > b.cbox[1] || r[2] > b.cbox[2]))
      return -1;
    for (size_t k = P.fwd.size(); k-- > 3 * (nlev - h);) {
      const LiftPass& ps = P.fwd[k];
      LiftFuse lf;
      pass_dequant(b, bb, k, lf);
      if (launch_lift(ss, false, bb.vals, bb.valsStride, nb, cd, ps.axis, ps.region, d.cst, 0, d_dst, vd, bb.geom, &lf))
        return -1;
    }
    const uint32_t blocks = (r[0] * r[1] * r[2] + kThreads - 1) / kThreads;
    if (h == 0 && b.fuseDq)
      LAUNCH_K(k_dequant_corner, dim3(blocks, nb), dim3(kThreads), 0, ss, bb.vals, bb.valsStride, bx, by, cd[0], cd[1],
               r[0], r[1], r[2], d.cst, dequant_src(b, bb, false));
    if (lvl.crop)
      LAUNCH_K((k_level_write<T, true>), dim3(blocks, nb), dim3(kThreads), 0, ss, bb.vals, bb.valsStride, d.cst, bb.crop,
               bx, by, cd[0], cd[1], cd[2], r[0], r[1], r[2], vd, d_dst);
    else
      LAUNCH_K((k_level_write<T, false>), dim3(blocks, nb), dim3(kThreads), 0, ss, bb.vals, bb.valsStride, d.cst, bb.geom,
               bx, by, cd[0], cd[1], cd[2], r[0], r[1], r[2], vd, d_dst);
    HIP_CHECK(hipGetLastError());
    return 0;
  }
  int collect_states(const Batch& b)
  {
    for (uint32_t q = 0; q < b.nsub; q++) {
      SubHost& S = (*b.subs)[q];
      if (S.nb == 0)
        continue;
      hipStream_t ss = b.nsub > 1 ? E.sub[q] : st;
      if (S.bb.db.lisStamps && q == 0) {
        g_lis_stamps_host.assign(64, 0);
        const uint32_t sc = getenv("SPERR_HIP_STAMP_CHUNK")
                                ? std::min<uint32_t>(S.nb - 1, (uint32_t)atoi(getenv("SPERR_HIP_STAMP_CHUNK")))
                                : 0u;
        HIP_CHECK(hipMemcpyAsync(g_lis_stamps_host.data(), S.bb.db.lisStamps + (size_t)sc * 64, 64 * 8,
                                 hipMemcpyDeviceToHost, ss));
      }
      S.hs.resize(S.nb);
      HIP_CHECK(hipMemcpyAsync(S.hs.data(), S.bb.db.st, S.nb * sizeof(DecState), hipMemcpyDeviceToHost, ss));
    }
    HIP_CHECK(hipStreamSynchronize(st));
    if (b.nsub > 1)
      for (uint32_t q = 0; q < b.nsub; q++)
        HIP_CHECK(hipStreamSynchronize(E.sub[q]));
    for (auto& S : *b.subs)
      for (auto& hsx : S.hs)
        if (hsx.error) {
          report_dec_error(hsx.error);
          return -1;
        }
    return 0;
  }
  int drain()
  {
    int rc = 0;
    for (uint32_t q = 0; q < kSubStreams; q++)
      HIP_CHECK(hipStreamSynchronize(E.sub[q]));
    HIP_CHECK(hipStreamSynchronize(E.outlQ[1]));
    for (auto& te : timingEnds) {
      float ms = 0.f;
      if (timingFork && hipEventElapsedTime(&ms, timingFork, te.first) == hipSuccess)
        fprintf(stderr, "[sperr_hip] group %u x %u x %u, %u chunks: through %.2f ms after the first group's fork\n",
                te.second[0], te.second[1], te.second[2], te.second[3], ms);
      (void)hipEventDestroy(te.first);
    }
    timingEnds.clear();
    if (timingFork) {
      (void)hipEventDestroy(timingFork);
      timingFork = nullptr;
    }
    for (SubHost* S : pending) {
      S->hs.resize(S->nb);
      HIP_CHECK(hipMemcpy(S->hs.data(), S->bb.db.st, S->nb * sizeof(DecState), hipMemcpyDeviceToHost));
      for (auto& hsx : S->hs)
        if (hsx.error) {
          report_dec_error(hsx.error);
          rc = -1;
        }
    }
    pending.clear();
    deferOff = 0;
    return rc;
  }
};

template <typename T>
int decompress_impl(Engine& E, const uint8_t* d_src, T* d_dst, size_t dst_cap_vals, const ContainerInfo& ci,
                    hipStream_t st, const DecodeRequest& req)
{
  DecodeCall<T> call{E, d_src, d_dst, ci, st, req};
  return call.run(dst_cap_vals);
}


template <typename CT>
__global__ void k_msb_of(const CT* coef, int8_t* msb, uint32_t n)
{
  const uint32_t i = blockIdx.x * blockDim.x + threadIdx.x;
  if (i >= n)
    return;
  const unsigned long long v = coef[i];
  msb[i] = v ? (int8_t)(63 - __clzll((long long)v)) : (int8_t)-1;
}

__global__ void __launch_bounds__(kThreads)
k_speck_stream_out(const CoderState* cst, const uint64_t* stream, uint8_t* dst, uint64_t cap,
                   uint64_t* len_out)
{
  const CoderState& cs = cst[0];
  const uint64_t len = cs.stream_len - 17;
  if (blockIdx.x == 0 && threadIdx.x == 0)
    *len_out = len;
  if (len > cap)
    return;
  if (blockIdx.x == 0 && threadIdx.x == 0) {
    dst[0] = (uint8_t)cs.nbp;
    memcpy(dst + 1, &cs.total_bits, 8);
  }
// ... 1366 lines not shown
```

sperr_amd/csrc/xform.h:

```cpp
#ifndef SPERR_AMD_XFORM_H
#define SPERR_AMD_XFORM_H

#include <string.h>

#include "common.h"

namespace sperrhip {

struct LiftConsts {
  double alpha, beta, gamma, delta, eps, inv_eps;
};
LiftConsts lift_consts();

template <typename T>
int launch_condition(hipStream_t stream, const T* vol, VolDesc vd, const ChunkGeom* geom,
                     uint32_t nchunks, const uint32_t cdims[3], uint32_t nstrides,
                     double* strideMean, size_t strideMeanStride, double* vals,
                     size_t valsStride, CoderState* st, bool gather, bool want_range = false,
                     bool org_x_aligned = false);

template <typename T>
int launch_scatter(hipStream_t stream, T* vol, VolDesc vd, const ChunkGeom* geom,
                   uint32_t nchunks, const uint32_t cdims[3], const double* vals,
                   size_t valsStride, const CoderState* st, const CropGeom* crop = nullptr);

struct DecState;

struct DequantSrc {
  const void* coef = nullptr;
  size_t coefStride = 0;
  const uint64_t* sign = nullptr;
  size_t signStride = 0;
  const uint64_t* sigNew = nullptr;
  const uint64_t* sigOld = nullptr;
  size_t maskStride = 0;
  const DecState* dst = nullptr;
  int coefSigned = 0;

  __host__ __device__ bool has_masks() const { return sigNew != nullptr && dst != nullptr; }
  template <typename CT>
  __host__ __device__ const CT* coefs(uint32_t c) const { return static_cast<const CT*>(coef) + c * coefStride; }
};

struct LiftFuse {
  int mode = 0;
  uint32_t inner[3] = {0, 0, 0};
  [[no_unique_address]] DequantSrc src;
  int noMean = 0;
  uint32_t bufx = 0, bufy = 0;
};
static_assert(sizeof(LiftFuse) == 96 && __builtin_offsetof(LiftFuse, noMean) == 84, "the argument block of the lifting kernels");

int launch_lift(hipStream_t stream, bool forward, double* vals, size_t valsStride,
                uint32_t nchunks, const uint32_t cdims[3], int axis, const uint32_t region[3],
                CoderState* st, int io = 0, void* volume = nullptr, VolDesc vd = VolDesc{},
                const ChunkGeom* geom = nullptr, const LiftFuse* fuse = nullptr,
                const CropGeom* crop = nullptr);

bool lift_xy_applicable(const uint32_t cdims[3]);
int launch_lift_xy(hipStream_t stream, bool forward, double* vals, size_t valsStride,
                   uint32_t nchunks, const uint32_t cdims[3], const CoderState* st, int io,
                   void* volume, VolDesc vd, const ChunkGeom* geom, const CropGeom* crop = nullptr);

bool lift_xyz_applicable(const uint32_t cdims[3]);
int launch_lift_xyz(hipStream_t stream, bool forward, double* vals, size_t valsStride, uint32_t nchunks,
                    const uint32_t cdims[3], CoderState* st, int io, void* volume, VolDesc vd,
                    const ChunkGeom* geom, const LiftFuse* fuse, const CropGeom* crop = nullptr);

int launch_maxabs_q(hipStream_t stream, const double* vals, size_t valsStride, uint32_t nchunks,
                    uint32_t n, CoderState* st, bool have_max = false);
int launch_make_q_wide(hipStream_t stream, uint32_t nchunks, CoderState* st);
int launch_mark_wide(hipStream_t stream, uint32_t nchunks, CoderState* st);

int launch_mse(hipStream_t stream, const double* vals, size_t valsStride, uint32_t nchunks,
               uint32_t n, double* partial, size_t partialStride, CoderState* st);

__host__ __device__ inline unsigned long long order_key(double v)
{
  unsigned long long b;
  memcpy(&b, &v, 8);
  return (b >> 63) ? ~b : (b | 0x8000000000000000ull);
}
__host__ __device__ inline double order_key_value(unsigned long long k)
{
  const unsigned long long b = (k >> 63) ? (k & 0x7fffffffffffffffull) : ~k;
  double v;
  memcpy(&v, &b, 8);
  return v;
}

int launch_quantize(hipStream_t stream, bool wide, const double* vals, size_t valsStride,
                    uint32_t nchunks, uint32_t n, void* coef, size_t coefStride, uint64_t* sign,
                    size_t signStride, int8_t* msb, size_t msbStride, const CoderState* st);

int launch_inv_quantize(hipStream_t stream, bool wide, const DequantSrc& src, uint32_t nchunks, uint32_t n,
                        double* vals, size_t valsStride, const CoderState* st);

}

#endif
```

sperr_amd/csrc/xform.hip:

```cpp
#include <type_traits>

#include "xform.h"
#include "lift_window.h"
#include "dequant.h"

namespace sperrhip {


constexpr int kSumStrides = 64, kSumSeg = 64;


template <typename T>
__global__ void __launch_bounds__(kThreads)
k_stride_sums(const T* __restrict__ vol, VolDesc vd, const ChunkGeom* geom, uint32_t cx,
              uint32_t cy, uint32_t cz, uint32_t nstrides, uint32_t ssz, double* strideMean,
              size_t strideMeanStride, CoderState* st, int want_range)
{
  __shared__ double tile[kSumStrides][kSumSeg + 1];
  __shared__ uint32_t sh_differs;
  double vmax = -INFINITY, vnegmax = -INFINITY;
  const uint32_t c = blockIdx.y;
  const uint32_t s0 = blockIdx.x * kSumStrides;
  const ChunkGeom g = geom[c];
  const size_t vx = vd.dims[0], vy = vd.dims[1];
// ... 656 lines not shown
#define XYZ_INV_PREFETCH 2
#endif
#ifndef XYZ_FWD_THREADS
#define XYZ_FWD_THREADS 1024
#endif
constexpr int kXYZThreadsF = XYZ_FWD_THREADS, kXYZThreadsI = XYZ_INV_THREADS;
constexpr int kXYZRows = 16;
constexpr int kXYZStaged = kXYZRows + 2 * kXYHalo;
constexpr int kXYZPosF = (4096 + kXYZThreadsF - 1) / kXYZThreadsF;
constexpr int kXYZStageF = (6144 + kXYZThreadsF - 1) / kXYZThreadsF;
constexpr int kXYZPosI = 6144 / kXYZThreadsI;
#ifndef XYZ_INV_GROUP
#define XYZ_INV_GROUP 3
#endif
constexpr int kXYZGroupI = XYZ_INV_GROUP;
#ifndef XYZ_FWD_YOUT
#define XYZ_FWD_YOUT 4
#endif
#ifndef XYZ_FWD_XOUT
#define XYZ_FWD_XOUT 8
#endif
#ifndef XYZ_INV_YOUT
#define XYZ_INV_YOUT 4
#endif
#ifndef XYZ_INV_XOUT
#define XYZ_INV_XOUT 4
#endif
#ifndef XYZ_INV_XSTORE
#define XYZ_INV_XSTORE 1
#endif
#ifndef XYZ_FWD_OFF
#define XYZ_FWD_OFF 0
#endif
#ifndef XYZ_INV_OFF
#define XYZ_INV_OFF 0
#endif
template <int MASK>
__device__ __forceinline__ bool xyz_off(int bit, uint32_t nseg)
{
  return (MASK & bit) != 0 && nseg != ~0u;
}
constexpr int kXYZOutFY = XYZ_FWD_YOUT, kXYZOutFX = XYZ_FWD_XOUT, kXYZOutIY = XYZ_INV_YOUT, kXYZOutIX = XYZ_INV_XOUT;
constexpr bool xyz_out_ok(int n) { return n == 2 || n == 4 || n == 8; }
static_assert(xyz_out_ok(kXYZOutFY) && xyz_out_ok(kXYZOutFX) && xyz_out_ok(kXYZOutIY) && xyz_out_ok(kXYZOutIX), "2, 4 or 8 outputs a task");
constexpr int kXYZBoxSlots = 48;

__host__ __device__ inline uint32_t xyz_row_stride(uint32_t cx)
{
  return ((cx + 7u) & ~7u) + 9u;
}

#define XYZ_LDS_BARRIER() asm volatile("s_waitcnt lgkmcnt(0)\n\ts_barrier" ::: "memory")

__device__ __forceinline__ void xyz_put(double* row, uint32_t x, uint32_t cx, double v)
{
  row[4 + x] = v;
  if (x - 1u < 4u)
    row[4 - x] = v;
  if (cx - 2u - x < 4u)
    row[2 * cx + 2 - x] = v;
}

template <bool FORWARD, int NT, int NOUT>
__device__ __forceinline__ void xyz_lift_x(const double* src, double* dst, uint32_t RS, uint32_t cx, uint32_t jlo,
                                           uint32_t jhi, uint32_t tid, const LiftConsts& K)
{
  const uint32_t nseg = (cx + NOUT - 1) / NOUT;
  const uint32_t ntask = (jhi - jlo) * nseg;
#pragma unroll 1
  for (uint32_t t = tid; t < ntask; t += NT) {
    const uint32_t rows = jhi - jlo, sg = t / rows, rb = jlo + (t - sg * rows);
    const double* row = src + (size_t)rb * RS + sg * NOUT;
    double r[NOUT + 8];
#pragma unroll
    for (int k = 0; k < NOUT + 8; k++)
      r[k] = row[k];
    lift_window<FORWARD, NOUT + 8>(r, K);
    double* out = dst + (size_t)rb * RS + 4 + sg * NOUT;
#pragma unroll
    for (int k = 0; k < NOUT; k++)
      if (sg * NOUT + k < cx)
        out[k] = r[4 + k];
  }
}

template <int NT, int NOUT, typename VT>
__device__ __forceinline__ void xyz_lift_x_store(const double* src, VT* vrows, size_t vsy, uint32_t RS, uint32_t cx, uint32_t jlo,
                                                 uint32_t jhi, uint32_t tid, const LiftConsts& K, double mean, bool noMean,
                                                 bool doStore)
{
  const uint32_t nseg = (cx + NOUT - 1) / NOUT;
  const uint32_t ntask = (jhi - jlo) * nseg;
#pragma unroll 1
  for (uint32_t t = tid; t < ntask; t += NT) {
    const uint32_t rows = jhi - jlo, sg = t / rows, rb = t - sg * rows;
    const double* row = src + (size_t)(jlo + rb) * RS + sg * NOUT;
    double r[NOUT + 8];
#pragma unroll
    for (int k = 0; k < NOUT + 8; k++)
      r[k] = row[k];
    lift_window<false, NOUT + 8>(r, K);
    VT* out = vrows + (size_t)rb * vsy + sg * NOUT;
    VT v[NOUT];
#pragma unroll
    for (int k = 0; k < NOUT; k++)
      v[k] = (VT)(noMean ? r[4 + k] : r[4 + k] + mean);
    if (!doStore)
      continue;
    if (sg * NOUT + NOUT <= cx) {
      typedef VT Seg __attribute__((ext_vector_type(NOUT), aligned(sizeof(VT))));
      Seg s;
#pragma unroll
      for (int k = 0; k < NOUT; k++)
        s[k] = v[k];
      *reinterpret_cast<Seg*>(out) = s;
    }
    else {
#pragma unroll
      for (int k = 0; k < NOUT; k++)
        if (sg * NOUT + k < cx)
          out[k] = v[k];
    }
  }
}

template <bool FORWARD, bool APRON, int NT, int NOUT>
__device__ __forceinline__ void xyz_lift_y(const double* src, double* dst, uint32_t RS, uint32_t cx, uint32_t nt,
                                           uint32_t tid, const LiftConsts& K)
{
  const uint32_t nq = (nt + NOUT - 1) / NOUT;
  const uint32_t ntask = nq * cx;
#pragma unroll 1
  for (uint32_t t = tid; t < ntask; t += NT) {
    const uint32_t q = t / cx, x = t - q * cx;
    const double* top = src + (size_t)(q * NOUT) * RS + 4 + x;
    double r[NOUT + 8];
#pragma unroll
    for (int k = 0; k < NOUT + 8; k++)
      r[k] = top[(size_t)k * RS];
    lift_window<FORWARD, NOUT + 8>(r, K);
#pragma unroll
    for (int k = 0; k < NOUT; k++) {
      if (q * NOUT + k < nt) {
        double* row = dst + (size_t)(4 + q * NOUT + k) * RS;
        if (APRON)
          xyz_put(row, x, cx, r[4 + k]);
        else
          row[4 + x] = r[4 + k];
      }
    }
  }
}

template <int IO>
__global__ void __launch_bounds__(kXYZThreadsF) __attribute__((amdgpu_waves_per_eu(kXYZThreadsF / 256, kXYZThreadsF / 256)))
k_lift_xyz_fwd(double* vals, size_t valsStride, uint32_t cx, uint32_t cy, uint32_t cz, LiftConsts K,
               CoderState* st, const void* volume, VolDesc vd, const ChunkGeom* geom, int wantMax,
               uint32_t in0, uint32_t in1, uint32_t in2, uint32_t nseg)
{
  static_assert(IO == 1 || IO == 2, "float or double volume");
  using VT = typename std::conditional<IO == 1, float, double>::type;
  const uint32_t c = blockIdx.y;
  if (st[c].is_const != 0)
    return;
  const uint32_t tid = threadIdx.x;
  const uint32_t seg = blockIdx.x % nseg, npairsAll = (cz + 1) / 2;
  const uint32_t mA = seg == 0 ? 0u : (uint32_t)((uint64_t)npairsAll * seg / nseg);
  const uint32_t mB = seg + 1 == nseg ? npairsAll : (uint32_t)((uint64_t)npairsAll * (seg + 1) / nseg);
  const uint32_t zFirst = mA >= 6 ? 2 * (mA - 6) : 0u;
  const uint32_t zEnd = seg + 1 == nseg ? cz : 2 * mB - 1;
  const uint32_t y0 = (blockIdx.x / nseg) * kXYZRows;
  const uint32_t nt = min((uint32_t)kXYZRows, cy - y0);
  const uint32_t RS = xyz_row_stride(cx);
  double* sm = reinterpret_cast<double*>(dyn_smem);
  const uint32_t bufN = (uint32_t)kXYZStaged * RS;
  const uint32_t xe = cx - cx / 2, ye = cy - cy / 2, ze = cz - cz / 2;
  const VT* vol = reinterpret_cast<const VT*>(volume);
  const size_t vsy = vd.dims[0], vsz = (size_t)vd.dims[0] * vd.dims[1];
  const VT* volc = vol + ((size_t)geom[c].org[2] * vsz + (size_t)geom[c].org[1] * vsy + geom[c].org[0]);
  double* buf = vals + c * valsStride;
  const size_t sliceN = (size_t)cx * cy;
  const double mean = st[c].mean;

  const uint32_t nstage = (uint32_t)kXYZStaged * cx;
  uint32_t pk[kXYZStageF];
#pragma unroll
  for (int k = 0; k < kXYZStageF; k++) {
    const uint32_t q = tid + (uint32_t)k * kXYZThreadsF;
    const uint32_t j = q / cx, x = q - j * cx;
    pk[k] = (j << 27) | (reflect_index((int)y0 - kXYHalo + (int)j, (int)cy) << 12) | x;
  }
  const uint32_t npos = nt * cx;
  uint32_t srow[kXYZPosF], ooff[kXYZPosF];
  uint32_t outerMask = 0;
#pragma unroll
  for (int k = 0; k < kXYZPosF; k++) {
    const uint32_t q = tid + (uint32_t)k * kXYZThreadsF;
    const uint32_t row = q / cx, col = q - row * cx, y = y0 + row;
    srow[k] = ((row + kXYHalo) << 16) | col;
    const uint32_t drow = (y & 1) ? ye + (y >> 1) : (y >> 1), dcol = (col & 1) ? xe + (col >> 1) : (col >> 1);
    ooff[k] = drow * cx + dcol;
    if (!(dcol < in0 && drow < in1))
      outerMask |= 1u << k;
  }
  double sxe[kXYZPosF], sxo[kXYZPosF], d1p[kXYZPosF], e1p[kXYZPosF], d2p[kXYZPosF];
#pragma unroll
  for (int k = 0; k < kXYZPosF; k++)
    sxe[k] = sxo[k] = d1p[k] = e1p[k] = d2p[k] = 0.0;
  double vmax = 0.0;
  auto emit = [&](int k, uint32_t zp, double v) {
    if (!xyz_off<XYZ_FWD_OFF>(4, nseg))
      buf[(size_t)zp * sliceN + ooff[k]] = v;
    if (wantMax && (((outerMask >> k) & 1u) || zp >= in2))
      vmax = fmax(vmax, fabs(v));
  };

  VT pre[kXYZStageF];
  auto issue = [&](uint32_t z) {
    const VT* src = volc + (size_t)z * vsz;
#pragma unroll
    for (int k = 0; k < kXYZStageF; k++) {
      if (xyz_off<XYZ_FWD_OFF>(1, nseg)) {
        pre[k] = (VT)(((pk[k] + z * 40503u) * 2654435761u) >> 20);
      }
      else {
        pre[k] = (tid + (uint32_t)k * kXYZThreadsF) < nstage
                     ? src[(size_t)((pk[k] >> 12) & 0x7fffu) * vsy + (pk[k] & 0xfffu)] : (VT)0;
      }
    }
  };
  issue(zFirst);
  for (uint32_t z = zFirst; z < zEnd; z++) {
    uint32_t RSv = RS, tidv = tid;
    asm volatile("" : "+s"(RSv), "+v"(tidv));
#pragma unroll
    for (int k = 0; k < kXYZStageF; k++)
      asm volatile("" : "+v"(pk[k]));
#pragma unroll
    for (int k = 0; k < kXYZPosF; k++)
      asm volatile("" : "+v"(srow[k]), "+v"(ooff[k]));
    double* A = sm + ((z & 1) ? bufN : 0u);
    double* B = sm + ((z & 1) ? 0u : bufN);
#pragma unroll
    for (int k = 0; k < kXYZStageF; k++)
      if ((tid + (uint32_t)k * kXYZThreadsF) < nstage)
        xyz_put(A + (pk[k] >> 27) * RSv, pk[k] & 0xfffu, cx, (double)pre[k] - mean);
    if (z + 1 < zEnd)
      issue(z + 1);
    XYZ_LDS_BARRIER();
    if (!xyz_off<XYZ_FWD_OFF>(2, nseg))
      xyz_lift_x<true, kXYZThreadsF, kXYZOutFX>(A, B, RSv, cx, 0, kXYZStaged, tidv, K);
    XYZ_LDS_BARRIER();
    if (!xyz_off<XYZ_FWD_OFF>(2, nseg))
      xyz_lift_y<true, false, kXYZThreadsF, kXYZOutFY>(B, A, RSv, cx, nt, tidv, K);
    XYZ_LDS_BARRIER();
    const uint32_t m = z >> 1;
    if (xyz_off<XYZ_FWD_OFF>(8, nseg))
      continue;
    if (z & 1) {
#pragma unroll
      for (int k = 0; k < kXYZPosF; k++)
        if ((tid + (uint32_t)k * kXYZThreadsF) < npos)
          sxo[k] = A[(srow[k] >> 16) * RSv + 4 + (srow[k] & 0xffffu)];
    }
    else {
#pragma unroll
      for (int k = 0; k < kXYZPosF; k++) {
        if ((tid + (uint32_t)k * kXYZThreadsF) >= npos)
          continue;
        const double v = A[(srow[k] >> 16) * RSv + 4 + (srow[k] & 0xffffu)];
        if (m >= 1) {
          const double d1n = fma(K.alpha, sxe[k] + v, sxo[k]);
          const double e1n = fma(K.beta, (m == 1 ? d1n : d1p[k]) + d1n, sxe[k]);
          if (m >= 2) {
            const double d2n = fma(K.gamma, e1p[k] + e1n, d1p[k]);
            const double e2 = K.eps * fma(K.delta, (m == 2 ? d2n : d2p[k]) + d2n, e1p[k]);
            if (m >= mA) {
              emit(k, m - 2, e2);
              emit(k, ze + m - 2, (-K.inv_eps) * d2n);
            }
            d2p[k] = d2n;
          }
          d1p[k] = d1n;
          e1p[k] = e1n;
        }
        sxe[k] = v;
      }
    }
  }
#pragma unroll
  for (int k = 0; k < kXYZPosF; k++) {
    if ((tid + (uint32_t)k * kXYZThreadsF) >= npos || seg + 1 != nseg)
      continue;
    if ((cz & 1) == 0) {
      const uint32_t M = cz / 2 - 1;
      const double d1L = fma(K.alpha, sxe[k] + sxe[k], sxo[k]);
      const double e1M = fma(K.beta, d1p[k] + d1L, sxe[k]);
      const double d2a = fma(K.gamma, e1p[k] + e1M, d1p[k]);
      const double e2a = K.eps * fma(K.delta, d2p[k] + d2a, e1p[k]);
      const double d2L = fma(K.gamma, e1M + e1M, d1L);
      const double e2L = K.eps * fma(K.delta, d2a + d2L, e1M);
      emit(k, M - 1, e2a);
      emit(k, ze + M - 1, (-K.inv_eps) * d2a);
      emit(k, M, e2L);
      emit(k, ze + M, (-K.inv_eps) * d2L);
    }
    else {
      const uint32_t M = cz / 2;
      const double e1M = fma(K.beta, d1p[k] + d1p[k], sxe[k]);
      const double d2a = fma(K.gamma, e1p[k] + e1M, d1p[k]);
      const double e2a = K.eps * fma(K.delta, d2p[k] + d2a, e1p[k]);
      const double e2L = K.eps * fma(K.delta, d2a + d2a, e1M);
      emit(k, M - 1, e2a);
      emit(k, ze + M - 1, (-K.inv_eps) * d2a);
      emit(k, M, e2L);
    }
  }
  if (wantMax) {
    for (int d = 32; d > 0; d >>= 1)
      vmax = fmax(vmax, __shfl_xor(vmax, d, 64));
    if ((tid & 63) == 0 && vmax > 0.0)
      atomicMax(reinterpret_cast<unsigned long long*>(&st[c].maxabs),
                (unsigned long long)__double_as_longlong(vmax));
  }
}

template <int IO, bool SG, bool kCrop = false>
__global__ void __launch_bounds__(kXYZThreadsI) __attribute__((amdgpu_waves_per_eu(kXYZThreadsI / 256, kXYZThreadsI / 256)))
k_lift_xyz_inv(const double* vals, size_t valsStride, uint32_t cx, uint32_t cy, uint32_t cz, LiftConsts K,
               const CoderState* st, void* volume, VolDesc vd, const GeomOf<kCrop>* geom, LiftFuse F, uint32_t nseg)
{
  static_assert(IO == 1 || IO == 2, "float or double volume");
  using VT = typename std::conditional<IO == 1, float, double>::type;
  const uint32_t c = blockIdx.y;
  const uint32_t tid = threadIdx.x;
  const uint32_t seg = blockIdx.x % nseg, npairsAll = cz / 2;
  const uint32_t mA = seg == 0 ? 0u : (uint32_t)((uint64_t)npairsAll * seg / nseg);
  const uint32_t mB = seg + 1 == nseg ? npairsAll : (uint32_t)((uint64_t)npairsAll * (seg + 1) / nseg);
  const uint32_t mFirst = mA >= 6 ? mA - 6 : 0u;
  const uint32_t y0 = (blockIdx.x / nseg) * kXYZRows;
  const uint32_t nt = min((uint32_t)kXYZRows, cy - y0);
  const uint32_t RS = xyz_row_stride(cx);
  double* sm = reinterpret_cast<double*>(dyn_smem);
  const uint32_t bufN = (uint32_t)kXYZStaged * RS;
  const uint32_t xe = cx - cx / 2, ye = cy - cy / 2, ze = cz - cz / 2;
  VT* vol = reinterpret_cast<VT*>(volume);
  const size_t vsy = vd.dims[0], vsz = (size_t)vd.dims[0] * vd.dims[1];
  VT* volc = vol;
  CropGeom cg{};
  uint32_t wy0 = 0, wy1 = 0;
  if constexpr (kCrop) {
    cg = geom[c];
    wy0 = max(y0, cg.lo[1]) - y0;
    wy1 = min(y0 + nt, cg.hi[1]);
    if (y0 + wy0 >= wy1)
      return;
    wy1 -= y0;
  }
  else
    volc = vol + ((size_t)geom[c].org[2] * vsz + (size_t)geom[c].org[1] * vsy + geom[c].org[0]);
  auto crop_row = [&](uint32_t z, uint32_t r) -> VT* { return vol + crop_addr(cg, vd, cg.lo[0], y0 + r, z); };
  (void)crop_row;
  const double* buf = vals + c * valsStride;
  const size_t sliceN = (size_t)cx * cy;
  const uint32_t bufx = F.bufx ? F.bufx : cx;
  const size_t bufSlice = (size_t)bufx * (F.bufy ? F.bufy : cy);
  const double mean = st[c].mean;
  const uint32_t lane = tid & 63u, nwaves = kXYZThreadsI / 64;
  const uint32_t wave = (uint32_t)__builtin_amdgcn_readfirstlane((int)(tid >> 6));

  if (st[c].is_const != 0) {
    if constexpr (kCrop) {
      const uint32_t w = cg.hi[0] - cg.lo[0], nr = wy1 - wy0;
      for (uint32_t z = cg.lo[2] + seg; z < cg.hi[2]; z += nseg)
        for (uint32_t k = tid; k < nr * w; k += kXYZThreadsI)
          crop_row(z, wy0 + k / w)[k % w] = (VT)mean;
    }
    else
    for (uint32_t z = seg; z < cz; z += nseg)
      for (uint32_t k = tid; k < nt * cx; k += kXYZThreadsI)
        volc[(size_t)z * vsz + (size_t)(y0 + k / cx) * vsy + k % cx] = (VT)mean;
    return;
  }

  const uint32_t npos = (uint32_t)kXYZStaged * cx;
  uint32_t pk[kXYZPosI];
  uint32_t innerMask = 0;
#pragma unroll
  for (int k = 0; k < kXYZPosI; k++) {
    const uint32_t q = tid + (uint32_t)k * kXYZThreadsI;
    const uint32_t j = q / cx, x = q - j * cx, y = reflect_index((int)y0 - kXYHalo + (int)j, (int)cy);
    const uint32_t drow = (y & 1) ? ye + (y >> 1) : (y >> 1), dcol = (x & 1) ? xe + (x >> 1) : (x >> 1);
    pk[k] = (j << 27) | (y << 12) | x;
    if (dcol < F.inner[0] && drow < F.inner[1])
      innerMask |= 1u << k;
  }
  const bool dequant = F.mode == 2 && !st[c].wide;
  const double fq = dequant ? st[c].q : 0.0;
  const DequantSrc& Q = F.src;
  const uint32_t* coef = Q.coefs<uint32_t>(c);
  const uint64_t* sign = Q.sign + c * Q.signStride;
  const bool haveMasks = dequant && Q.has_masks();
  const uint64_t* mNew = haveMasks ? Q.sigNew + c * Q.maskStride : sign;
  const uint64_t* mOld = haveMasks ? Q.sigOld + c * Q.maskStride : sign;
  const DequantRule<uint32_t> rule = dequant_rule<uint32_t>(fq, haveMasks, haveMasks ? Q.dst + c : nullptr, SG);
  const int scheme = rule.scheme;
  auto sg_value = [&](uint32_t sv) -> double { return dequant_signed(rule, sv); };
  auto fetch = [&](int k, uint32_t zp) -> double {
    const uint32_t y = (pk[k] >> 12) & 0x7fffu, x = pk[k] & 0xfffu;
    const uint32_t drow = (y & 1) ? ye + (y >> 1) : (y >> 1), dcol = (x & 1) ? xe + (x >> 1) : (x >> 1);
    const size_t idx = (size_t)zp * sliceN + drow * cx + dcol;
    const bool inBox = ((innerMask >> k) & 1u) && zp < F.inner[2];
    if (!dequant && !inBox && F.bufx)
      return 0.0;
    if (dequant && !inBox) {
      if (SG && scheme)
        return sg_value(coef[idx]);
      const uint32_t v = coef[idx];
      const uint32_t sh = (uint32_t)(idx & 63);
      const uint64_t sgw = sign[idx >> 6], mnw = mNew[idx >> 6], mow = mOld[idx >> 6];
      return dequant_masks(rule, v, mnw, mow, sgw, sh);
    }
    return buf[(size_t)zp * bufSlice + drow * bufx + dcol];
  };
  uint32_t flip = 0;
  auto stage = [&](int k, double v) {
    uint32_t p = pk[k];
    asm volatile("" : "+v"(p));
    (sm + (flip ? bufN : 0u))[(p >> 27) * RS + 4 + (p & 0xfffu)] = v;
  };
  auto stage_all = [&](const double (&v)[kXYZPosI]) {
#pragma unroll
    for (int k = 0; k < kXYZPosI; k++)
      if ((tid + (uint32_t)k * kXYZThreadsI) < npos)
        stage(k, v[k]);
  };
  auto store_rows = [&](uint32_t z, uint32_t which) {
    const double* X = sm + (which ? bufN : 0u);
    uint32_t lanev = lane;
    asm volatile("" : "+v"(lanev));
    if constexpr (kCrop) {
      if (z - cg.lo[2] >= cg.hi[2] - cg.lo[2])
        return;
      for (uint32_t r = wy0 + wave; r < wy1; r += nwaves) {
        VT* dstrow = crop_row(z, r);
        const double* srow = X + (size_t)(kXYHalo + r) * RS + 4;
        for (uint32_t x = cg.lo[0] + lanev; x < cg.hi[0]; x += 64)
          dstrow[x - cg.lo[0]] = (VT)(F.noMean ? srow[x] : srow[x] + mean);
      }
      return;
    }
    if (xyz_off<XYZ_INV_OFF>(4, nseg))
      return;
    for (uint32_t r = wave; r < nt; r += nwaves) {
      VT* dstrow = volc + (size_t)z * vsz + (size_t)(y0 + r) * vsy;
      const double* srow = X + (size_t)(kXYHalo + r) * RS + 4;
      if (F.noMean) {
        for (uint32_t x = lanev; x < cx; x += 64)
          dstrow[x] = (VT)srow[x];
      }
      else
        for (uint32_t x = lanev; x < cx; x += 64)
          dstrow[x] = (VT)(srow[x] + mean);
    }
  };
  constexpr bool kDirect = !kCrop && XYZ_INV_XSTORE != 0;
  auto finish_slice = [&](uint32_t z) {
    uint32_t RSv = RS, tidv = tid;
    asm volatile("" : "+s"(RSv), "+v"(tidv));
    const uint32_t which = flip;
    double* X = sm + (flip ? bufN : 0u);
    double* Y = sm + (flip ? 0u : bufN);
    if constexpr (!kDirect)
      flip ^= 1u;
    XYZ_LDS_BARRIER();
    if (!xyz_off<XYZ_INV_OFF>(2, nseg))
      xyz_lift_y<false, true, kXYZThreadsI, kXYZOutIY>(X, Y, RSv, cx, nt, tidv, K);
    XYZ_LDS_BARRIER();
    if constexpr (kDirect) {
      if (!xyz_off<XYZ_INV_OFF>(2, nseg))
        xyz_lift_x_store<kXYZThreadsI, kXYZOutIX>(Y, volc + (size_t)z * vsz + (size_t)y0 * vsy, vsy, RSv, cx, kXYHalo, kXYHalo + nt,
                                                   tidv, K, mean, F.noMean != 0, !xyz_off<XYZ_INV_OFF>(4, nseg));
      else
        store_rows(z, which ^ 1u);
    }
    else {
      if (!xyz_off<XYZ_INV_OFF>(2, nseg))
        xyz_lift_x<false, kXYZThreadsI, kXYZOutIX>(Y, X, RSv, cx, kXYHalo, kXYHalo + nt, tidv, K);
      XYZ_LDS_BARRIER();
      store_rows(z, which);
    }
  };

  double o1p[kXYZPosI], e1p[kXYZPosI], o2p[kXYZPosI], e2p[kXYZPosI];
#pragma unroll
  for (int k = 0; k < kXYZPosI; k++)
    o1p[k] = e1p[k] = o2p[k] = e2p[k] = 0.0;
  const uint32_t npairs = cz / 2;
  auto zstep = [&](int k, uint32_t m, bool mine, bool active, double E, double O) {
    const double o1 = (-K.eps) * O;
    const double t = K.delta * ((m == 0 ? o1 : o1p[k]) + o1);
    const double e1 = fma(E, K.inv_eps, -t);
    if (m >= 1) {
      const double o2 = fma(-K.gamma, e1p[k] + e1, o1p[k]);
      const double e2 = fma(-K.beta, (m == 1 ? o2 : o2p[k]) + o2, e1p[k]);
      if (m >= 2 && mine && active)
        stage(k, fma(-K.alpha, e2p[k] + e2, o2p[k]));
      o2p[k] = o2;
      e2p[k] = e2;
    }
    o1p[k] = o1;
    e1p[k] = e1;
  };
#if XYZ_INV_PREFETCH == 2
  uint32_t* myPre = reinterpret_cast<uint32_t*>(sm + 2 * (size_t)bufN) + (size_t)wave * (kXYZPosI * 2 * 64);
  const uint32_t* sign32 = reinterpret_cast<const uint32_t*>(sign);
  const uint32_t* mNew32 = reinterpret_cast<const uint32_t*>(mNew);
  const uint32_t* mOld32 = reinterpret_cast<const uint32_t*>(mOld);
  uint32_t activeMask = 0;
#pragma unroll
  for (int k = 0; k < kXYZPosI; k++)
    if ((tid + (uint32_t)k * kXYZThreadsI) < npos)
      activeMask |= 1u << k;
    else
      pk[k] = pk[0];
  uint32_t boxAny = 0;
#pragma unroll
  for (int k = 0; k < kXYZPosI; k++)
    boxAny |= __ballot((innerMask >> k) & 1u) != 0ull ? 1u << k : 0u;
  boxAny = (uint32_t)__builtin_amdgcn_readfirstlane((int)boxAny);
  auto pos_off = [&](int k, uint32_t& drow, uint32_t& dcol) {
    const uint32_t y = (pk[k] >> 12) & 0x7fffu, x = pk[k] & 0xfffu;
    drow = (y & 1) ? ye + (y >> 1) : (y >> 1);
    dcol = (x & 1) ? xe + (x >> 1) : (x >> 1);
  };
  const bool fastLoads = dequant && F.inner[2] <= ze && (!SG || scheme != 0);
  uint32_t boxLds = 0, boxSlot0 = 0;
  uint32_t* boxRows = reinterpret_cast<uint32_t*>(sm + 2 * (size_t)bufN) + (size_t)nwaves * (kXYZPosI * 2 * 64);
  if (SG && fastLoads) {
    uint32_t reg = 0;
#pragma unroll
    for (int k = 0; k < kXYZPosI; k++) {
      const uint64_t inb = __ballot((innerMask >> k) & 1u), act = __ballot((activeMask >> k) & 1u);
      if (inb == 0x5555555555555555ull && act == ~0ull && (cx & 63u) == 0)
        reg |= 1u << k;
    }
    reg = (uint32_t)__builtin_amdgcn_readfirstlane((int)reg);
    uint32_t* cnt = reinterpret_cast<uint32_t*>(sm);
    if (lane == 0)
      cnt[wave] = (uint32_t)__popc(reg);
    XYZ_LDS_BARRIER();
    uint32_t before = 0, total = 0;
    for (uint32_t w = 0; w < nwaves; w++) {
      const uint32_t v = cnt[w];
      before += w < wave ? v : 0u;
      total += v;
    }
    XYZ_LDS_BARRIER();
    if (total <= (uint32_t)kXYZBoxSlots && reg == (1u << kXYZPosI) - 1u) {
      boxLds = reg;
      boxSlot0 = (uint32_t)__builtin_amdgcn_readfirstlane((int)before);
    }
  }
  uint32_t* myBox = boxRows + (size_t)boxSlot0 * 64;
  auto pre_issue = [&](uint32_t m) {
    if (xyz_off<XYZ_INV_OFF>(1, nseg))
      return;
    if (SG && boxLds != 0 && m < F.inner[2]) {
#pragma unroll
      for (int k = 0; k < kXYZPosI; k++) {
        uint32_t drow, dcol;
        pos_off(k, drow, dcol);
        const uint32_t x0h = ((pk[k] & 0xfffu) - lane) >> 1;
        const uint32_t* src = reinterpret_cast<const uint32_t*>(buf + ((size_t)m * bufSlice + (size_t)drow * bufx + x0h)) + lane;
        __builtin_amdgcn_global_load_lds(src, myBox + k * 64, 4, 0, 0);
      }
    }
#pragma unroll
    for (int k = 0; k < kXYZPosI; k++) {
      uint32_t drow, dcol;
      pos_off(k, drow, dcol);
      const uint32_t off = drow * cx + dcol;
      __builtin_amdgcn_global_load_lds(coef + ((size_t)m * sliceN + off), myPre + (k * 2) * 64, 4, 0, 0);
      __builtin_amdgcn_global_load_lds(coef + ((size_t)(ze + m) * sliceN + off), myPre + (k * 2 + 1) * 64, 4, 0, 0);
    }
  };
  if (fastLoads && mFirst < mB)
    pre_issue(mFirst);
#endif
  for (uint32_t m = mFirst; m < mB; m++) {
    const bool mine = m >= mA;
#pragma unroll
    for (int k = 0; k < kXYZPosI; k++)
      asm volatile("" : "+v"(pk[k]));
#if XYZ_INV_PREFETCH == 2
    if (SG && fastLoads) {
      asm volatile("s_waitcnt vmcnt(0)" ::: "memory");
      const bool boxWave = boxAny != 0 && m < F.inner[2];
      const bool zOn = !xyz_off<XYZ_INV_OFF>(8, nseg);
      if (zOn && boxWave && boxLds != 0) {
#pragma unroll
        for (int k = 0; k < kXYZPosI; k++) {
          const double lo = sg_value(myPre[(k * 2) * 64 + lane]);
          const double hi = sg_value(myPre[(k * 2 + 1) * 64 + lane]);
          const double bxv = reinterpret_cast<const double*>(myBox + k * 64)[lane >> 1];
          zstep(k, m, mine, true, (lane & 1u) ? lo : bxv, hi);
        }
      }
      else if (zOn) {
#pragma unroll
      for (int g = 0; g < kXYZPosI; g += kXYZGroupI) {
        __builtin_amdgcn_sched_barrier(0);
        double bx[kXYZGroupI];
        uint32_t boxm = 0;
        if (boxWave) {
#pragma unroll
          for (int kk = 0; kk < kXYZGroupI; kk++) {
            const int k = g + kk;
            if (k >= kXYZPosI)
              continue;
            uint32_t drow, dcol;
            pos_off(k, drow, dcol);
            const bool inBox = ((innerMask >> k) & 1u) != 0;
            boxm |= inBox ? 1u << kk : 0u;
            bx[kk] = buf[inBox ? (size_t)m * bufSlice + drow * bufx + dcol : (size_t)0];
          }
        }
#pragma unroll
        for (int kk = 0; kk < kXYZGroupI; kk++) {
          const int k = g + kk;
          if (k >= kXYZPosI)
            continue;
          const double lo = sg_value(myPre[(k * 2) * 64 + lane]);
          const double hi = sg_value(myPre[(k * 2 + 1) * 64 + lane]);
          zstep(k, m, mine, ((activeMask >> k) & 1u) != 0, ((boxm >> kk) & 1u) ? bx[kk] : lo, hi);
        }
      }
      }
      __builtin_amdgcn_sched_barrier(0);
      if (m + 1 < mB)
        pre_issue(m + 1);
      __builtin_amdgcn_sched_barrier(0);
    }
    else if (!SG && fastLoads) {
      asm volatile("s_waitcnt vmcnt(0)" ::: "memory");
#pragma unroll
      for (int g = 0; g < kXYZPosI; g += kXYZGroupI) {
        __builtin_amdgcn_sched_barrier(0);
        constexpr int NV = 2 * kXYZGroupI;
        uint32_t sgw[NV], mnw[NV], mow[NV], cv[NV], shv[NV], boxm = 0;
        double bx[kXYZGroupI];
#pragma unroll
        for (int j = 0; j < NV; j++) {
          const int k = g + j / 2;
          if (k >= kXYZPosI)
            continue;
          const uint32_t zp = (j & 1) ? ze + m : m;
          uint32_t drow, dcol;
          pos_off(k, drow, dcol);
          const size_t idx = (size_t)zp * sliceN + drow * cx + dcol;
          sgw[j] = sign32[idx >> 5];
          mnw[j] = mNew32[idx >> 5];
          mow[j] = mOld32[idx >> 5];
          if ((j & 1) == 0) {
            const bool inBox = ((innerMask >> k) & 1u) && zp < F.inner[2];
            boxm |= inBox ? 1u << j : 0u;
            bx[j / 2] = buf[inBox ? (size_t)zp * bufSlice + drow * bufx + dcol : (size_t)0];
          }
          cv[j] = myPre[(k * 2 + (j & 1)) * 64 + lane];
          shv[j] = (uint32_t)idx & 31u;
        }
        double val[NV];
#pragma unroll
        for (int j = 0; j < NV; j++) {
          if (g + j / 2 >= kXYZPosI)
            continue;
          const double dq = dequant_masks(rule, cv[j], mnw[j], mow[j], sgw[j], shv[j]);
          val[j] = ((j & 1) == 0 && ((boxm >> j) & 1u)) ? bx[j / 2] : dq;
        }
#pragma unroll
        for (int kk = 0; kk < kXYZGroupI; kk++)
          if (g + kk < kXYZPosI)
            zstep(g + kk, m, mine, ((activeMask >> (g + kk)) & 1u) != 0, val[2 * kk], val[2 * kk + 1]);
      }
      __builtin_amdgcn_sched_barrier(0);
      if (m + 1 < mB)
        pre_issue(m + 1);
      __builtin_amdgcn_sched_barrier(0);
    }
    else
#endif
    {
#pragma unroll
      for (int k = 0; k < kXYZPosI; k++) {
        if ((k % 3) == 0)
          __builtin_amdgcn_sched_barrier(0);
        if ((tid + (uint32_t)k * kXYZThreadsI) >= npos)
          continue;
        const double E = fetch(k, m), O = fetch(k, ze + m);
        zstep(k, m, mine, true, E, O);
      }
    }
    if (m >= 2 && mine)
      finish_slice(2 * m - 3);
    if (m >= 1 && mine) {
      stage_all(e2p);
      finish_slice(2 * m - 2);
    }
  }
  if (seg + 1 != nseg)
    return;
  if ((cz & 1) == 0) {
    const uint32_t M = npairs - 1;
    double outC[kXYZPosI];
#pragma unroll
    for (int k = 0; k < kXYZPosI; k++) {
      outC[k] = 0.0;
      if ((tid + (uint32_t)k * kXYZThreadsI) >= npos)
        continue;
      const double o2 = fma(-K.gamma, e1p[k] + e1p[k], o1p[k]);
      const double e2 = fma(-K.beta, o2p[k] + o2, e1p[k]);
      stage(k, fma(-K.alpha, e2p[k] + e2, o2p[k]));
      e2p[k] = e2;
      outC[k] = fma(-K.alpha, e2 + e2, o2);
    }
    finish_slice(2 * M - 1);
    stage_all(e2p);
    finish_slice(2 * M);
    stage_all(outC);
    finish_slice(2 * M + 1);
  }
  else {
    const uint32_t M = npairs;
    double outC[kXYZPosI], outD[kXYZPosI];
#pragma unroll
    for (int k = 0; k < kXYZPosI; k++) {
      outC[k] = outD[k] = 0.0;
      if ((tid + (uint32_t)k * kXYZThreadsI) >= npos)
        continue;
      const double E = fetch(k, M);
      const double t = K.delta * (o1p[k] + o1p[k]);
      const double e1 = fma(E, K.inv_eps, -t);
      const double o2 = fma(-K.gamma, e1p[k] + e1, o1p[k]);
      const double e2 = fma(-K.beta, o2p[k] + o2, e1p[k]);
      stage(k, fma(-K.alpha, e2p[k] + e2, o2p[k]));
      e2p[k] = e2;
      const double e2L = fma(-K.beta, o2 + o2, e1);
      outC[k] = fma(-K.alpha, e2 + e2L, o2);
      outD[k] = e2L;
    }
    finish_slice(2 * M - 3);
    stage_all(e2p);
    finish_slice(2 * M - 2);
    stage_all(outC);
    finish_slice(2 * M - 1);
    stage_all(outD);
    finish_slice(2 * M);
  }
}


constexpr int kMaxPer = 16;
__global__ void __launch_bounds__(kThreads)
k_maxabs(const double* vals, size_t valsStride, uint32_t n, CoderState* st)
{
  const uint32_t c = blockIdx.y;
  if (st[c].is_const)
    return;
  __shared__ double wmax[kThreads / 64];
  const double* in = vals + c * valsStride;
  const uint32_t base = blockIdx.x * (kThreads * kMaxPer);
  double m = 0.0;
#pragma unroll
  for (int k = 0; k < kMaxPer / 2; k++) {
    const uint32_t i = base + (k * kThreads + threadIdx.x) * 2;
    if (i + 1 < n) {
      const double2 v = *reinterpret_cast<const double2*>(in + i);
      m = fmax(m, fmax(fabs(v.x), fabs(v.y)));
    }
    else if (i < n)
      m = fmax(m, fabs(in[i]));
  }
  for (int d = 32; d > 0; d >>= 1)
    m = fmax(m, __shfl_xor(m, d, 64));
  if ((threadIdx.x & 63) == 0)
    wmax[threadIdx.x >> 6] = m;
  __syncthreads();
  if (threadIdx.x == 0) {
    for (int w = 1; w < kThreads / 64; w++)
      m = fmax(m, wmax[w]);
    if (m > 0.0)
      atomicMax(reinterpret_cast<unsigned long long*>(&st[c].maxabs),
                (unsigned long long)__double_as_longlong(m));
  }
}

constexpr uint32_t kMseStride = 4096;

__global__ void __launch_bounds__(kThreads)
k_mse_strides(const double* vals, size_t valsStride, uint32_t n, double* partial,
              size_t partialStride, const CoderState* st)
{
  __shared__ double tile[kSumStrides][kSumSeg + 1];
  const uint32_t c = blockIdx.y;
  if (st[c].is_const || !st[c].mse_active)
    return;
  const double q = st[c].q, rcp_q = 1.0 / q;
  const double* in = vals + c * valsStride;
  const uint32_t npart = n / kMseStride + 1;
  const uint32_t s0 = blockIdx.x * kSumStrides;
  double acc = 0.0;
  for (uint32_t seg = 0; seg < kMseStride; seg += kSumSeg) {
    __syncthreads();
    for (uint32_t k = threadIdx.x; k < (uint32_t)(kSumStrides * kSumSeg); k += kThreads) {
      const uint32_t r = k / kSumSeg, j = k % kSumSeg;
      const uint64_t e = (uint64_t)(s0 + r) * kMseStride + seg + j;
      tile[r][j] = (s0 + r < npart && e < n) ? in[e] : 0.0;
    }
    __syncthreads();
    if (threadIdx.x < (uint32_t)kSumStrides && s0 + threadIdx.x < npart) {
      const uint64_t e0 = (uint64_t)(s0 + threadIdx.x) * kMseStride + seg;
      const uint32_t len = e0 >= n ? 0u : (uint32_t)min((uint64_t)kSumSeg, n - e0);
      for (uint32_t j = 0; j < len; j++) {
        const double v = tile[threadIdx.x][j];
        const double diff = fma(-q, rint(v * rcp_q), v);
        acc = fma(diff, diff, acc);
      }
    }
  }
  if (threadIdx.x < (uint32_t)kSumStrides && s0 + threadIdx.x < npart)
    partial[c * partialStride + s0 + threadIdx.x] = acc;
}

__global__ void k_mse_final(uint32_t n, const double* partial, size_t partialStride,
                            CoderState* st, uint32_t nchunks)
{
  const uint32_t c = blockIdx.x * blockDim.x + threadIdx.x;
  if (c >= nchunks || st[c].is_const || !st[c].mse_active)
    return;
  const uint32_t npart = n / kMseStride + 1;
  const double* pp = partial + c * partialStride;
  double total = 0.0;
  for (uint32_t s = 0; s < npart; s++)
    total += pp[s];
  st[c].mse = total / (double)n;
}

__global__ void k_make_q_rate(CoderState* st, uint32_t nchunks, int wide_pass)
{
  const uint32_t c = blockIdx.x * blockDim.x + threadIdx.x;
  if (c >= nchunks)
    return;
  if (wide_pass) {
    if (!st[c].need_retry)
      return;
    st[c].q = st[c].maxabs / 0x1.fffffffffffffp52;
    st[c].wide = 1;
  }
  else {
    st[c].q = st[c].maxabs / 4294967295.0;
    st[c].wide = 0;
  }
}

template <typename CT>
__global__ void k_quantize(const double* vals, size_t valsStride, uint32_t n, CT* coef,
                           size_t coefStride, uint64_t* sign, size_t signStride, int8_t* msb,
                           size_t msbStride, const CoderState* st, int wide_pass)
{
  const uint32_t c = blockIdx.y;
  const CoderState& s = st[c];
  if (s.is_const || (wide_pass && !s.need_retry))
    return;
  const double inv = 1.0 / s.q;
  const double* in = vals + c * valsStride;
  const uint32_t i = blockIdx.x * blockDim.x + threadIdx.x;
  long long ll = 0;
  bool nonneg = false;
  if (i < n) {
    ll = __double2ll_rn(in[i] * inv);
    nonneg = ll >= 0;
    const unsigned long long mag = (unsigned long long)(ll < 0 ? -ll : ll);
    coef[c * coefStride + i] = (CT)mag;
    msb[c * msbStride + i] = mag ? (int8_t)(63 - __clzll((long long)mag)) : (int8_t)-1;
  }
  const unsigned long long word = __ballot(nonneg);
  if ((threadIdx.x & 63) == 0 && i < n)
    sign[c * signStride + (i >> 6)] = word;
}

__global__ void __launch_bounds__(kThreads)
k_quantize4(const double* vals, size_t valsStride, uint32_t n, uint32_t* coef, size_t coefStride,
            uint64_t* sign, size_t signStride, int8_t* msb, size_t msbStride, const CoderState* st)
{
  const uint32_t c = blockIdx.y;
  const CoderState& s = st[c];
  if (s.is_const)
    return;
  const double inv = 1.0 / s.q;
  const uint32_t i = (blockIdx.x * blockDim.x + threadIdx.x) * 4;
  uint32_t nn = 0;
  if (i < n) {
    const double2* in = reinterpret_cast<const double2*>(vals + c * valsStride + i);
    const double2 a = in[0], b2 = in[1];
    const double v[4] = {a.x, a.y, b2.x, b2.y};
    uint32_t mag[4], mb = 0;
#pragma unroll
    for (int e = 0; e < 4; e++) {
      const long long ll = __double2ll_rn(v[e] * inv);
      nn |= (ll >= 0 ? 1u : 0u) << e;
      const unsigned long long m = (unsigned long long)(ll < 0 ? -ll : ll);
// ... 93 lines not shown
    const size_t bytes = (size_t)len * (nl + 1) * sizeof(double);
    if (bytes <= cap || nl == 1) {
      *smem = bytes;
      return nl;
    }
  }
  return 1;
}

int launch_lift(hipStream_t stream, bool forward, double* vals, size_t valsStride,
                uint32_t nchunks, const uint32_t cdims[3], int axis, const uint32_t region[3],
                CoderState* st, int io, void* volume, VolDesc vd, const ChunkGeom* geom,
                const LiftFuse* fuse, const CropGeom* crop)
{
  const LiftFuse F = fuse ? *fuse : LiftFuse{};
  if (crop && (forward || io == 0))
    return -1;
  {
    const void* fns[8] = {reinterpret_cast<const void*>(&k_lift_axis<true, 0>),
                          reinterpret_cast<const void*>(&k_lift_axis<true, 1>),
                          reinterpret_cast<const void*>(&k_lift_axis<true, 2>),
                          reinterpret_cast<const void*>(&k_lift_axis<false, 0>),
                          reinterpret_cast<const void*>(&k_lift_axis<false, 1>),
                          reinterpret_cast<const void*>(&k_lift_axis<false, 2>),
                          reinterpret_cast<const void*>(&k_lift_axis<false, 1, true>),
                          reinterpret_cast<const void*>(&k_lift_axis<false, 2, true>)};
    for (const void* f : fns)
      if (set_max_dyn_lds(f, 160 * 1024))
        return -1;
  }
  const uint32_t len = region[axis];
  if (len < 2)
    return io ? -1 : 0;
  size_t smem = 0;
  const int NL = pick_nl(len, axis, &smem);
  if (smem > 160 * 1024) {
    fprintf(stderr, "[sperr_hip] line of %u samples does not fit in LDS\n", len);
    return -1;
  }
  const int ua = (axis == 0) ? 1 : 0, wa = (axis == 2) ? 1 : 2;
  const uint32_t ntu = (region[ua] + NL - 1) / NL;
  dim3 grid(ntu * region[wa], nchunks);
  const LiftConsts K = lift_consts();
#define LIFT_ARGS vals, valsStride, cdims[0], cdims[1], axis, region[0], region[1], region[2], NL, K, st, volume, vd, geom, F
  if (forward) {
    if (io == 1)
      LAUNCH_K((k_lift_axis<true, 1>), grid, dim3(kThreads), smem, stream, LIFT_ARGS);
    else if (io == 2)
      LAUNCH_K((k_lift_axis<true, 2>), grid, dim3(kThreads), smem, stream, LIFT_ARGS);
    else
      LAUNCH_K((k_lift_axis<true, 0>), grid, dim3(kThreads), smem, stream, LIFT_ARGS);
  }
  else if (crop) {
#define CROP_ARGS vals, valsStride, cdims[0], cdims[1], axis, region[0], region[1], region[2], NL, K, st, volume, vd, crop, F
    if (io == 1)
      LAUNCH_K((k_lift_axis<false, 1, true>), grid, dim3(kThreads), smem, stream, CROP_ARGS);
    else
      LAUNCH_K((k_lift_axis<false, 2, true>), grid, dim3(kThreads), smem, stream, CROP_ARGS);
#undef CROP_ARGS
  }
  else {
    if (io == 1)
      LAUNCH_K((k_lift_axis<false, 1>), grid, dim3(kThreads), smem, stream, LIFT_ARGS);
    else if (io == 2)
      LAUNCH_K((k_lift_axis<false, 2>), grid, dim3(kThreads), smem, stream, LIFT_ARGS);
    else
      LAUNCH_K((k_lift_axis<false, 0>), grid, dim3(kThreads), smem, stream, LIFT_ARGS);
  }
#undef LIFT_ARGS
  HIP_CHECK(hipGetLastError());
  return 0;
}

static int xy_rows(uint32_t cx, uint32_t cy)
{
  if (cx < 2 || cy < 2)
    return 0;
  const size_t rowBytes = (size_t)(cx + 1) * sizeof(double);
  static const int ldsKB = tune_getenv("SPERR_HIP_XY_LDS_KB") ? atoi(tune_getenv("SPERR_HIP_XY_LDS_KB")) : 68;
  static const int maxRows = tune_getenv("SPERR_HIP_XY_ROWS") ? atoi(tune_getenv("SPERR_HIP_XY_ROWS")) : 32;
  int rows = (int)(((size_t)ldsKB * 1024) / rowBytes);
  if (rows > maxRows)
    rows = maxRows;
  int R = (rows - 2 * kXYHalo) & ~1;
  if ((uint32_t)R > cy)
    R = (int)((cy + 1) & ~1u);
  return R >= 8 ? R : 0;
}

bool lift_xy_applicable(const uint32_t cdims[3])
{
  return xy_rows(cdims[0], cdims[1]) > 0;
}

int launch_lift_xy(hipStream_t stream, bool forward, double* vals, size_t valsStride,
                   uint32_t nchunks, const uint32_t cdims[3], const CoderState* st, int io,
                   void* volume, VolDesc vd, const ChunkGeom* geom, const CropGeom* crop)
{
  if (crop && forward)
    return -1;
  {
    const void* fns[6] = {reinterpret_cast<const void*>(&k_lift_xy<true, 1>),
                          reinterpret_cast<const void*>(&k_lift_xy<true, 2>),
                          reinterpret_cast<const void*>(&k_lift_xy<false, 1>),
                          reinterpret_cast<const void*>(&k_lift_xy<false, 2>),
                          reinterpret_cast<const void*>(&k_lift_xy<false, 1, true>),
                          reinterpret_cast<const void*>(&k_lift_xy<false, 2, true>)};
    for (const void* f : fns)
      if (set_max_dyn_lds(f, 160 * 1024))
        return -1;
  }
  const int R = xy_rows(cdims[0], cdims[1]);
  if (R <= 0 || (io != 1 && io != 2))
    return -1;
  const size_t smem = (size_t)(R + 2 * kXYHalo) * (cdims[0] + 1) * sizeof(double);
  const uint32_t ntile = (cdims[1] + R - 1) / R;
  const dim3 grid(ntile * cdims[2], nchunks);
  const LiftConsts K = lift_consts();
#define XY_ARGS vals, valsStride, cdims[0], cdims[1], cdims[2], R, K, st, volume, vd, geom
  if (forward) {
    if (io == 1)
      LAUNCH_K((k_lift_xy<true, 1>), grid, dim3(kXYThreads), smem, stream, XY_ARGS);
    else
      LAUNCH_K((k_lift_xy<true, 2>), grid, dim3(kXYThreads), smem, stream, XY_ARGS);
  }
  else if (crop) {
#define CROP_ARGS vals, valsStride, cdims[0], cdims[1], cdims[2], R, K, st, volume, vd, crop
    if (io == 1)
      LAUNCH_K((k_lift_xy<false, 1, true>), grid, dim3(kXYThreads), smem, stream, CROP_ARGS);
    else
      LAUNCH_K((k_lift_xy<false, 2, true>), grid, dim3(kXYThreads), smem, stream, CROP_ARGS);
#undef CROP_ARGS
  }
  else {
    if (io == 1)
      LAUNCH_K((k_lift_xy<false, 1>), grid, dim3(kXYThreads), smem, stream, XY_ARGS);
    else
      LAUNCH_K((k_lift_xy<false, 2>), grid, dim3(kXYThreads), smem, stream, XY_ARGS);
  }
#undef XY_ARGS
  HIP_CHECK(hipGetLastError());
  return 0;
}

bool lift_xyz_applicable(const uint32_t cdims[3])
{
  if (cdims[0] < 9 || cdims[1] < 9 || cdims[2] < 9)
    return false;
  return (size_t)kXYZStaged * cdims[0] <= (size_t)kXYZPosI * kXYZThreadsI &&
         (size_t)kXYZStaged * cdims[0] <= (size_t)kXYZStageF * kXYZThreadsF &&
         (size_t)kXYZRows * cdims[0] <= (size_t)kXYZPosF * kXYZThreadsF && cdims[0] < 4096 && cdims[1] < 32768;
}

int launch_lift_xyz(hipStream_t stream, bool forward, double* vals, size_t valsStride, uint32_t nchunks,
                    const uint32_t cdims[3], CoderState* st, int io, void* volume, VolDesc vd,
                    const ChunkGeom* geom, const LiftFuse* fuse, const CropGeom* crop)
{
  if (!lift_xyz_applicable(cdims) || (io != 1 && io != 2) || (crop && forward))
    return -1;
  const LiftFuse F = fuse ? *fuse : LiftFuse{};
  size_t smem = 2 * (size_t)kXYZStaged * xyz_row_stride(cdims[0]) * sizeof(double);
#if XYZ_INV_PREFETCH == 2
  if (!forward)
    smem += (size_t)kXYZThreadsI * kXYZPosI * 2 * sizeof(uint32_t) +
            (size_t)kXYZBoxSlots * 64 * sizeof(uint32_t);
#endif
  {
    const void* fns[10] = {reinterpret_cast<const void*>(&k_lift_xyz_fwd<1>), reinterpret_cast<const void*>(&k_lift_xyz_fwd<2>),
                           reinterpret_cast<const void*>(&k_lift_xyz_inv<1, false>), reinterpret_cast<const void*>(&k_lift_xyz_inv<2, false>),
                           reinterpret_cast<const void*>(&k_lift_xyz_inv<1, true>), reinterpret_cast<const void*>(&k_lift_xyz_inv<2, true>),
                           reinterpret_cast<const void*>(&k_lift_xyz_inv<1, false, true>), reinterpret_cast<const void*>(&k_lift_xyz_inv<2, false, true>),
                           reinterpret_cast<const void*>(&k_lift_xyz_inv<1, true, true>), reinterpret_cast<const void*>(&k_lift_xyz_inv<2, true, true>)};
    for (const void* f : fns)
      if (set_max_dyn_lds(f, 160 * 1024))
        return -1;
  }
  const uint32_t ntile = (cdims[1] + kXYZRows - 1) / kXYZRows;
  uint32_t nseg = 1;
  while (nseg < 4 && (size_t)ntile * nchunks * nseg < 512 && cdims[2] / (2 * nseg) >= 24)
    nseg *= 2;
  const dim3 grid(ntile * nseg, nchunks);
  const LiftConsts K = lift_consts();
  if (forward) {
    const int wantMax = F.mode == 1 ? 1 : 0;
    if (io == 1)
      LAUNCH_K((k_lift_xyz_fwd<1>), grid, dim3(kXYZThreadsF), smem, stream, vals, valsStride, cdims[0], cdims[1],
               cdims[2], K, st, volume, vd, geom, wantMax, F.inner[0], F.inner[1], F.inner[2], nseg);
    else
      LAUNCH_K((k_lift_xyz_fwd<2>), grid, dim3(kXYZThreadsF), smem, stream, vals, valsStride, cdims[0], cdims[1],
               cdims[2], K, st, volume, vd, geom, wantMax, F.inner[0], F.inner[1], F.inner[2], nseg);
  }
  else {
    const bool sg = F.mode == 2 && F.src.coefSigned != 0;
#define XYZ_INV_LAUNCH(io_, sg_)                                                                                    \
  LAUNCH_K((k_lift_xyz_inv<io_, sg_>), grid, dim3(kXYZThreadsI), smem, stream, vals, valsStride, cdims[0], cdims[1], \
           cdims[2], K, st, volume, vd, geom, F, nseg)
#define XYZ_CROP_LAUNCH(io_, sg_)                                                                                   \
  LAUNCH_K((k_lift_xyz_inv<io_, sg_, true>), grid, dim3(kXYZThreadsI), smem, stream, vals, valsStride, cdims[0],      \
           cdims[1], cdims[2], K, st, volume, vd, crop, F, nseg)
    if (crop) {
      if (io == 1 && sg)
        XYZ_CROP_LAUNCH(1, true);
      else if (io == 1)
        XYZ_CROP_LAUNCH(1, false);
      else if (sg)
        XYZ_CROP_LAUNCH(2, true);
      else
        XYZ_CROP_LAUNCH(2, false);
    }
    else if (io == 1) {
      if (sg)
        XYZ_INV_LAUNCH(1, true);
      else
        XYZ_INV_LAUNCH(1, false);
    }
    else {
      if (sg)
        XYZ_INV_LAUNCH(2, true);
      else
        XYZ_INV_LAUNCH(2, false);
    }
#undef XYZ_INV_LAUNCH
#undef XYZ_CROP_LAUNCH
  }
  HIP_CHECK(hipGetLastError());
  return 0;
}

template <typename T>
int launch_condition(hipStream_t stream, const T* vol, VolDesc vd, const ChunkGeom* geom,
                     uint32_t nchunks, const uint32_t cdims[3], uint32_t nstrides,
                     double* strideMean, size_t strideMeanStride, double* vals,
                     size_t valsStride, CoderState* st, bool gather, bool want_range,
                     bool org_x_aligned)
{
  const uint32_t n = cdims[0] * cdims[1] * cdims[2];
  const uint32_t ssz = n / nstrides;
  const uint32_t perLoad = 8 * (16 / (uint32_t)sizeof(T));
  const bool rowsPath = cdims[0] % perLoad == 0 && ssz % cdims[0] == 0 &&
                        vd.dims[0] % (16 / sizeof(T)) == 0 &&
                        reinterpret_cast<uintptr_t>(vol) % 16 == 0 && org_x_aligned;
  if (rowsPath)
    LAUNCH_K(k_stride_sums_rows<T>, dim3((nstrides + 63) / 64, nchunks), dim3(64), 0, stream, vol,
             vd, geom, cdims[0], cdims[1], nstrides, ssz, strideMean, strideMeanStride, st,
             want_range ? 1 : 0);
  else
    LAUNCH_K(k_stride_sums<T>, dim3((nstrides + kSumStrides - 1) / kSumStrides, nchunks),
             dim3(kThreads), 0, stream, vol, vd, geom, cdims[0], cdims[1], cdims[2], nstrides, ssz,
             strideMean, strideMeanStride, st, want_range ? 1 : 0);
  LAUNCH_K(k_mean_finalize<T>, dim3(nchunks), dim3(kThreads), 0, stream, vol, vd, geom,
                     nstrides, strideMean, strideMeanStride, st);
  if (gather)
    LAUNCH_K(k_gather_condition<T>, dim3((n + kThreads * 4 - 1) / (kThreads * 4), nchunks),
             dim3(kThreads), 0, stream, vol, vd, geom, cdims[0], cdims[1], n, vals, valsStride, st);
  HIP_CHECK(hipGetLastError());
  return 0;
}
template int launch_condition<float>(hipStream_t, const float*, VolDesc, const ChunkGeom*,
                                     uint32_t, const uint32_t[3], uint32_t, double*, size_t,
                                     double*, size_t, CoderState*, bool, bool, bool);
template int launch_condition<double>(hipStream_t, const double*, VolDesc, const ChunkGeom*,
                                      uint32_t, const uint32_t[3], uint32_t, double*, size_t,
                                      double*, size_t, CoderState*, bool, bool, bool);

template <typename T>
int launch_scatter(hipStream_t stream, T* vol, VolDesc vd, const ChunkGeom* geom,
                   uint32_t nchunks, const uint32_t cdims[3], const double* vals,
                   size_t valsStride, const CoderState* st, const CropGeom* crop)
{
  const uint32_t n = cdims[0] * cdims[1] * cdims[2];
  if (crop)
    LAUNCH_K((k_scatter_uncondition<T, true>), dim3((n + kThreads * 4 - 1) / (kThreads * 4), nchunks), dim3(kThreads), 0,
             stream, vol, vd, crop, cdims[0], cdims[1], n, vals, valsStride, st);
  else
  LAUNCH_K(k_scatter_uncondition<T>,
                     dim3((n + kThreads * 4 - 1) / (kThreads * 4), nchunks), dim3(kThreads), 0,
                     stream, vol, vd, geom, cdims[0], cdims[1], n, vals, valsStride, st);
  HIP_CHECK(hipGetLastError());
  return 0;
}
template int launch_scatter<float>(hipStream_t, float*, VolDesc, const ChunkGeom*, uint32_t,
                                   const uint32_t[3], const double*, size_t, const CoderState*,
                                   const CropGeom*);
template int launch_scatter<double>(hipStream_t, double*, VolDesc, const ChunkGeom*, uint32_t,
                                    const uint32_t[3], const double*, size_t, const CoderState*,
                                    const CropGeom*);

int launch_maxabs_q(hipStream_t stream, const double* vals, size_t valsStride, uint32_t nchunks,
                    uint32_t n, CoderState* st, bool have_max)
{
  if (!have_max)
    LAUNCH_K(k_maxabs, dim3((n + kThreads * kMaxPer - 1) / (kThreads * kMaxPer), nchunks),
                       dim3(kThreads), 0, stream, vals, valsStride, n, st);
  LAUNCH_K(k_make_q_rate, dim3((nchunks + 63) / 64), dim3(64), 0, stream, st, nchunks,
                     0);
  HIP_CHECK(hipGetLastError());
  return 0;
}

int launch_mse(hipStream_t stream, const double* vals, size_t valsStride, uint32_t nchunks,
               uint32_t n, double* partial, size_t partialStride, CoderState* st)
{
  const uint32_t npart = n / kMseStride + 1;
  LAUNCH_K(k_mse_strides, dim3((npart + kSumStrides - 1) / kSumStrides, nchunks), dim3(kThreads), 0,
           stream, vals, valsStride, n, partial, partialStride, st);
  LAUNCH_K(k_mse_final, dim3((nchunks + 63) / 64), dim3(64), 0, stream, n, partial, partialStride,
           st, nchunks);
  HIP_CHECK(hipGetLastError());
  return 0;
}

__global__ void k_mark_wide(CoderState* st, uint32_t nchunks)
{
  const uint32_t c = blockIdx.x * blockDim.x + threadIdx.x;
  if (c < nchunks && st[c].need_retry)
    st[c].wide = 1;
}

int launch_mark_wide(hipStream_t stream, uint32_t nchunks, CoderState* st)
{
  LAUNCH_K(k_mark_wide, dim3((nchunks + 63) / 64), dim3(64), 0, stream, st, nchunks);
  HIP_CHECK(hipGetLastError());
  return 0;
}

int launch_make_q_wide(hipStream_t stream, uint32_t nchunks, CoderState* st)
{
  LAUNCH_K(k_make_q_rate, dim3((nchunks + 63) / 64), dim3(64), 0, stream, st, nchunks,
                     1);
  HIP_CHECK(hipGetLastError());
  return 0;
}

int launch_quantize(hipStream_t stream, bool wide, const double* vals, size_t valsStride,
                    uint32_t nchunks, uint32_t n, void* coef, size_t coefStride, uint64_t* sign,
                    size_t signStride, int8_t* msb, size_t msbStride, const CoderState* st)
{
  dim3 grid((n + kThreads - 1) / kThreads, nchunks);
  if (wide)
    LAUNCH_K(k_quantize<uint64_t>, grid, dim3(kThreads), 0, stream, vals, valsStride, n,
                       (uint64_t*)coef, coefStride, sign, signStride, msb, msbStride, st, 1);
  else if (n % 64 == 0 && valsStride % 4 == 0 && coefStride % 4 == 0 && msbStride % 4 == 0)
    LAUNCH_K(k_quantize4, dim3((n / 4 + kThreads - 1) / kThreads, nchunks), dim3(kThreads), 0, stream, vals,
             valsStride, n, (uint32_t*)coef, coefStride, sign, signStride, msb, msbStride, st);
  else
    LAUNCH_K(k_quantize<uint32_t>, grid, dim3(kThreads), 0, stream, vals, valsStride, n,
                       (uint32_t*)coef, coefStride, sign, signStride, msb, msbStride, st, 0);
  HIP_CHECK(hipGetLastError());
  return 0;
}

int launch_inv_quantize(hipStream_t stream, bool wide, const DequantSrc& src, uint32_t nchunks, uint32_t n,
                        double* vals, size_t valsStride, const CoderState* st)
{
  dim3 grid((n + kThreads * 4 - 1) / (kThreads * 4), nchunks);
  if (wide)
    LAUNCH_K(k_inv_quantize<uint64_t>, grid, dim3(kThreads), 0, stream, src, n, vals, valsStride, st, 1);
  else
    LAUNCH_K(k_inv_quantize<uint32_t>, grid, dim3(kThreads), 0, stream, src, n, vals, valsStride, st, 0);
  HIP_CHECK(hipGetLastError());
  return 0;
}

}
```

Before: 69.06 GB/s.

## Fuse second wavelet level into a dedicated xyz lift kernel via compact box

Adds a fused second-level 3D lifting path. The forward xyz kernel writes the low-pass octant into a compact scratch box (aliased onto the coef32 buffer), and a new k_lift2_fwd kernel runs all three axes of level 2 in one launch instead of three separate per-axis passes. Decode mirrors this with k_lift2_inv writing into a new vals2 buffer that the level-1 inverse xyz kernel then reads. The aim is to cut global memory traffic and kernel launches for the level-2 passes. The cost is extra decode memory, and the encoder aliases scratch onto the coef buffer, with a guard and a retry path that disables it.

```diff
diff --git a/sperr_amd/csrc/engine.hip b/sperr_amd/csrc/engine.hip
--- a/sperr_amd/csrc/engine.hip
+++ b/sperr_amd/csrc/engine.hip
@@ -263,8 +263,10 @@
   uint64_t maxPhaseBits = 0;
   size_t lisEntries = 0;
   std::vector<LiftPass> fwd;
+  bool level2 = false;
 };
 bool use_tables(const ShapePlan& P);
+bool plan_level2(const ShapePlan& P);
 
 
 std::vector<FusedRoot> fused_head_roots(const spk::HostTree& h)
@@ -481,6 +483,7 @@
       P.fwd.push_back({1, {approx(dx, lev), approx(dy, lev), (uint32_t)dz}});
     }
   }
+  P.level2 = plan_level2(P);
   return 0;
 }
 
@@ -1283,9 +1286,37 @@
   return true;
 }
 
+static bool level2_fits(const ShapePlan& P)
+{
+  if (!fuse_xyz(P) || !plan_fusable(P) || P.fwd.size() < 6)
+    return false;
+  for (int k = 3; k < 6; k++) {
+    if (P.fwd[k].axis != k - 3)
+      return false;
+    for (int a = 0; a < 3; a++)
+      if (P.fwd[k].region[a] != P.dims[a] - P.dims[a] / 2)
+        return false;
+  }
+  uint32_t inner[3];
+  if (pass_fuse(P, 2, inner) <= 0 || inner[0] != P.fwd[3].region[0] || inner[1] != P.fwd[3].region[1] ||
+      inner[2] != P.fwd[3].region[2])
+    return false;
+  return lift2_applicable(P.fwd[3].region);
+}
+constexpr uint32_t kLevel2Floor = 96;
+bool plan_level2(const ShapePlan& P)
+{
+  const char* env = getenv("SPERR_HIP_XYZ_LEVEL2");
+  const int sw = env ? atoi(env) : 1;
+  if (sw == 0 || !level2_fits(P))
+    return false;
+  const uint32_t* r = P.fwd[3].region;
+  return sw == 2 || std::min(r[0], std::min(r[1], r[2])) >= kLevel2Floor;
+}
+
 template <typename T>
 int float_stages(hipStream_t ss, const ShapePlan& P, EncBatchBufs& bb, uint32_t nb, const uint32_t cd[3],
-                 const T* d_src, VolDesc vd, bool orgAligned, bool wantRange)
+                 const T* d_src, VolDesc vd, bool orgAligned, bool wantRange, bool level2 = true)
 {
   EncBuffers& e = bb.eb;
   const bool fuse = !P.fwd.empty();
@@ -1299,10 +1330,23 @@
     LiftFuse lf;
     if (fuseMax && pass_fuse(P, 2, lf.inner) > 0)
       lf.mode = 1;
+    const bool l2 = level2 && P.level2;
+    double* box = l2 ? reinterpret_cast<double*>(bb.coef32) : nullptr;
+    const size_t boxStride = e.coefStride / 2;
+    if (l2 && (e.coefStride % 2 != 0 || (size_t)lf.inner[0] * lf.inner[1] * lf.inner[2] > boxStride))
+      return -1;
     if (launch_lift_xyz(ss, true, bb.vals, bb.valsStride, nb, cd, e.cst, io, const_cast<T*>(d_src), vd,
-                        bb.geom, &lf))
+                        bb.geom, &lf, nullptr, box, boxStride))
       return -1;
     k0 = 3;
+    if (l2) {
+      LiftFuse l5;
+      if (pass_fuse(P, 5, l5.inner) > 0)
+        l5.mode = 1;
+      if (launch_lift2_fwd(ss, box, boxStride, bb.vals, bb.valsStride, nb, cd, P.fwd[3].region, e.cst, &l5))
+        return -1;
+      k0 = 6;
+    }
   }
   else if (fuse_xy(P)) {
     if (launch_lift_xy(ss, true, bb.vals, bb.valsStride, nb, cd, e.cst, io, const_cast<T*>(d_src), vd,
@@ -1343,7 +1387,7 @@
   if (unalias_coder(ss, E, P, bb, nb))
     return -1;
   g_dbg_counter[0]++;
-  return float_stages<T>(ss, P, bb, nb, cd, d_src, vd, orgAligned, wantRange);
+  return float_stages<T>(ss, P, bb, nb, cd, d_src, vd, orgAligned, wantRange, false);
 }
 
 int psnr_q_search(hipStream_t st, const ShapePlan& P, EncBatchBufs& bb, uint32_t nb, double psnr,
@@ -2403,12 +2447,13 @@
   uint64_t *chunkOff, *chunkLen;
   double* vals;
   size_t valsStride;
+  double* vals2;
   uint32_t* coef32;
   uint32_t* live;
 };
 
 bool carve_dec(Arena& A, const ShapePlan& P, uint32_t B, uint64_t maxPayloadBytes, DecBatchBufs& o,
-               size_t valsElems = 0, uint32_t refNPlanes = 0, bool crop = false)
+               size_t valsElems = 0, uint32_t refNPlanes = 0, bool crop = false, bool box2 = false)
 {
   const size_t N = P.N, Npad = round_up(N, 512);
   DecBuffers& d = o.db;
@@ -2434,6 +2479,10 @@
   TAKE(o.live, uint32_t, 64);
   o.valsStride = valsElems ? round_up(valsElems, 256) : Npad;
   TAKE(o.vals, double, o.valsStride * B);
+  o.vals2 = nullptr;
+  if (box2 && valsElems) {
+    TAKE(o.vals2, double, o.valsStride * B);
+  }
   d.coefStride = Npad;
   TAKE(o.coef32, uint32_t, Npad * B);
   d.coef = o.coef32;
@@ -2799,13 +2848,14 @@
   }
 };
 
-size_t dec_bytes_per_chunk(const ShapePlan& P, uint64_t maxPayload, size_t valsElems, uint32_t refNPlanes, bool crop)
+size_t dec_bytes_per_chunk(const ShapePlan& P, uint64_t maxPayload, size_t valsElems, uint32_t refNPlanes, bool crop,
+                           bool box2 = false)
 {
   Arena probe;
   probe.base = reinterpret_cast<char*>(uintptr_t(4096));
   probe.cap = ~size_t(0) / 2;
   DecBatchBufs tmp;
-  carve_dec(probe, P, 1, maxPayload, tmp, valsElems, refNPlanes, crop);
+  carve_dec(probe, P, 1, maxPayload, tmp, valsElems, refNPlanes, crop, box2);
   return probe.used;
 }
 
@@ -2850,6 +2900,7 @@
     uint32_t cbox[3], refNPlanes, nsub = 1;
     uint64_t maxPayload = 0;
     size_t compactElems;
+    bool level2 = false;
     bool deferG, fuseDq;
     hipStream_t deferStream = nullptr;
     std::vector<SubHost>* subs = nullptr;
@@ -3040,6 +3091,7 @@
         cbox[a] = std::max(cbox[a], lvl->m.cres[lvl->h][a]);
     return (size_t)cbox[0] * cbox[1] * cbox[2];
   }
+  bool level2_of(const ShapePlan& P, size_t compactElems) const { return P.level2 && compactElems != 0 && !req.level(); }
   int size_deferred()
   {
     deferSized = true;
@@ -3054,7 +3106,8 @@
       for (auto& r : h.second)
         mp = std::max<uint64_t>(mp, ci.len[r.gid]);
       uint32_t qbox[3];
-      sum += round_up(h.second.size() * dec_bytes_per_chunk(*Q, mp, compact_box(*Q, h.second, qbox), ref_planes_of(*Q, h.second), req.cropped()) + (1 << 20), 4096);
+      const size_t qelems = compact_box(*Q, h.second, qbox);
+      sum += round_up(h.second.size() * dec_bytes_per_chunk(*Q, mp, qelems, ref_planes_of(*Q, h.second), req.cropped(), level2_of(*Q, qelems)) + (1 << 20), 4096);
     }
     size_t fr = 0, tot = 0;
     HIP_CHECK(hipMemGetInfo(&fr, &tot));
@@ -3081,7 +3134,8 @@
     b.compactElems = compact_box(*P, refs, b.cbox);
     b.refNPlanes = ref_planes_of(*P, refs);
     b.fuseDq = plan_fusable(*P) && !req.levels && !req.slices;
-    const size_t per = dec_bytes_per_chunk(*P, b.maxPayload, b.compactElems, b.refNPlanes, req.cropped());
+    b.level2 = level2_of(*P, b.compactElems) && b.fuseDq;
+    const size_t per = dec_bytes_per_chunk(*P, b.maxPayload, b.compactElems, b.refNPlanes, req.cropped(), b.level2);
     size_t fr = 0, tot = 0;
     HIP_CHECK(hipMemGetInfo(&fr, &tot));
     const size_t budgetBytes = arena_budget(E.arena.n, fr);
@@ -3182,7 +3236,7 @@
       S.nb = (nbAll - done + (nsub - q) - 1) / (nsub - q);
       S.first = b0 + done;
       done += S.nb;
-      if (S.nb && !carve_dec(A, *b.P, S.nb, b.maxPayload, S.bb, b.compactElems, b.refNPlanes, req.cropped()))
+      if (S.nb && !carve_dec(A, *b.P, S.nb, b.maxPayload, S.bb, b.compactElems, b.refNPlanes, req.cropped(), b.level2))
         return -1;
       if (S.nb && b.compactElems)
         g_dbg_counter[2]++;
@@ -3428,7 +3482,8 @@
         lf.bufy = bbox[1];
       }
     };
-    for (size_t k = P.fwd.size(); k-- > ((fxyz || fbrick) ? 3u : fxy ? 2u : 0u);) {
+    const bool l2 = b.level2 && fxyz && bb.vals2 != nullptr;
+    for (size_t k = P.fwd.size(); k-- > (l2 ? 6u : (fxyz || fbrick) ? 3u : fxy ? 2u : 0u);) {
       const LiftPass& ps = P.fwd[k];
       if (k % perLevel == perLevel - 1 && sub_volume(k))
         return -1;
@@ -3450,9 +3505,15 @@
     if (fxyz) {
       if (sub_volume(2))
         return -1;
+      if (l2) {
+        LiftFuse l5;
+        dequant_fuse(5, l5);
+        if (launch_lift2_inv(ss, bb.vals, bb.valsStride, bb.vals2, bb.valsStride, nb, cd, P.fwd[3].region, d.cst, &l5))
+          return -1;
+      }
       LiftFuse lf;
       dequant_fuse(2, lf);
-      if (launch_lift_xyz(ss, false, bb.vals, bb.valsStride, nb, cd, d.cst, io, d_dst, vd, bb.geom, &lf, bb.crop))
+      if (launch_lift_xyz(ss, false, l2 ? bb.vals2 : bb.vals, bb.valsStride, nb, cd, d.cst, io, d_dst, vd, bb.geom, &lf, bb.crop))
         return -1;
     }
     if (fxy && req.slices && sub_volume(1))
diff --git a/sperr_amd/csrc/xform.h b/sperr_amd/csrc/xform.h
--- a/sperr_amd/csrc/xform.h
+++ b/sperr_amd/csrc/xform.h
@@ -65,7 +65,16 @@
 bool lift_xyz_applicable(const uint32_t cdims[3]);
 int launch_lift_xyz(hipStream_t stream, bool forward, double* vals, size_t valsStride, uint32_t nchunks,
                     const uint32_t cdims[3], CoderState* st, int io, void* volume, VolDesc vd,
-                    const ChunkGeom* geom, const LiftFuse* fuse, const CropGeom* crop = nullptr);
+                    const ChunkGeom* geom, const LiftFuse* fuse, const CropGeom* crop = nullptr,
+                    double* box = nullptr, size_t boxStride = 0);
+
+bool lift2_applicable(const uint32_t region[3]);
+int launch_lift2_fwd(hipStream_t stream, const double* box, size_t boxStride, double* vals, size_t valsStride,
+                     uint32_t nchunks, const uint32_t cdims[3], const uint32_t region[3], CoderState* st,
+                     const LiftFuse* fuse);
+int launch_lift2_inv(hipStream_t stream, const double* box, size_t boxStride, double* out, size_t outStride,
+                     uint32_t nchunks, const uint32_t cdims[3], const uint32_t region[3], const CoderState* st,
+                     const LiftFuse* fuse);
 
 int launch_maxabs_q(hipStream_t stream, const double* vals, size_t valsStride, uint32_t nchunks,
                     uint32_t n, CoderState* st, bool have_max = false);
diff --git a/sperr_amd/csrc/xform.hip b/sperr_amd/csrc/xform.hip
--- a/sperr_amd/csrc/xform.hip
+++ b/sperr_amd/csrc/xform.hip
@@ -832,17 +832,12 @@
   }
 }
 
-template <int IO>
-__global__ void __launch_bounds__(kXYZThreadsF) __attribute__((amdgpu_waves_per_eu(kXYZThreadsF / 256, kXYZThreadsF / 256)))
-k_lift_xyz_fwd(double* vals, size_t valsStride, uint32_t cx, uint32_t cy, uint32_t cz, LiftConsts K,
-               CoderState* st, const void* volume, VolDesc vd, const ChunkGeom* geom, int wantMax,
-               uint32_t in0, uint32_t in1, uint32_t in2, uint32_t nseg)
-{
-  static_assert(IO == 1 || IO == 2, "float or double volume");
-  using VT = typename std::conditional<IO == 1, float, double>::type;
-  const uint32_t c = blockIdx.y;
-  if (st[c].is_const != 0)
-    return;
+template <typename VT, int NPOS, int NSTG, bool L2>
+__device__ __forceinline__ void xyz_fwd_body(double* buf, const uint32_t orow, const size_t sliceN, uint32_t cx, uint32_t cy,
+                                             uint32_t cz, const LiftConsts& K, CoderState* stc, const VT* volc, const size_t vsy,
+                                             const size_t vsz, const double mean, int wantMax, uint32_t in0, uint32_t in1,
+                                             uint32_t in2, uint32_t nseg, double* box)
+{
   const uint32_t tid = threadIdx.x;
   const uint32_t seg = blockIdx.x % nseg, npairsAll = (cz + 1) / 2;
   const uint32_t mA = seg == 0 ? 0u : (uint32_t)((uint64_t)npairsAll * seg / nseg);
@@ -855,51 +850,52 @@
   double* sm = reinterpret_cast<double*>(dyn_smem);
   const uint32_t bufN = (uint32_t)kXYZStaged * RS;
   const uint32_t xe = cx - cx / 2, ye = cy - cy / 2, ze = cz - cz / 2;
-  const VT* vol = reinterpret_cast<const VT*>(volume);
-  const size_t vsy = vd.dims[0], vsz = (size_t)vd.dims[0] * vd.dims[1];
-  const VT* volc = vol + ((size_t)geom[c].org[2] * vsz + (size_t)geom[c].org[1] * vsy + geom[c].org[0]);
-  double* buf = vals + c * valsStride;
-  const size_t sliceN = (size_t)cx * cy;
-  const double mean = st[c].mean;
+  const size_t boxSlice = (size_t)in0 * in1;
 
   const uint32_t nstage = (uint32_t)kXYZStaged * cx;
-  uint32_t pk[kXYZStageF];
-#pragma unroll
-  for (int k = 0; k < kXYZStageF; k++) {
+  uint32_t pk[NSTG];
+#pragma unroll
+  for (int k = 0; k < NSTG; k++) {
     const uint32_t q = tid + (uint32_t)k * kXYZThreadsF;
     const uint32_t j = q / cx, x = q - j * cx;
     pk[k] = (j << 27) | (reflect_index((int)y0 - kXYHalo + (int)j, (int)cy) << 12) | x;
   }
   const uint32_t npos = nt * cx;
-  uint32_t srow[kXYZPosF], ooff[kXYZPosF];
+  uint32_t srow[NPOS], ooff[NPOS];
+  uint32_t boff[L2 ? 1 : NPOS];
   uint32_t outerMask = 0;
 #pragma unroll
-  for (int k = 0; k < kXYZPosF; k++) {
+  for (int k = 0; k < NPOS; k++) {
     const uint32_t q = tid + (uint32_t)k * kXYZThreadsF;
     const uint32_t row = q / cx, col = q - row * cx, y = y0 + row;
     srow[k] = ((row + kXYHalo) << 16) | col;
     const uint32_t drow = (y & 1) ? ye + (y >> 1) : (y >> 1), dcol = (col & 1) ? xe + (col >> 1) : (col >> 1);
-    ooff[k] = drow * cx + dcol;
+    ooff[k] = drow * orow + dcol;
+    if constexpr (!L2)
+      boff[k] = drow * in0 + dcol;
     if (!(dcol < in0 && drow < in1))
       outerMask |= 1u << k;
   }
-  double sxe[kXYZPosF], sxo[kXYZPosF], d1p[kXYZPosF], e1p[kXYZPosF], d2p[kXYZPosF];
-#pragma unroll
-  for (int k = 0; k < kXYZPosF; k++)
+  double sxe[NPOS], sxo[NPOS], d1p[NPOS], e1p[NPOS], d2p[NPOS];
+#pragma unroll
+  for (int k = 0; k < NPOS; k++)
     sxe[k] = sxo[k] = d1p[k] = e1p[k] = d2p[k] = 0.0;
   double vmax = 0.0;
   auto emit = [&](int k, uint32_t zp, double v) {
+    bool toBox = false;
+    if constexpr (!L2)
+      toBox = box != nullptr && zp < in2 && !((outerMask >> k) & 1u);
     if (!xyz_off<XYZ_FWD_OFF>(4, nseg))
-      buf[(size_t)zp * sliceN + ooff[k]] = v;
+      *(toBox ? box + ((size_t)zp * boxSlice + boff[L2 ? 0 : k]) : buf + ((size_t)zp * sliceN + ooff[k])) = v;
     if (wantMax && (((outerMask >> k) & 1u) || zp >= in2))
       vmax = fmax(vmax, fabs(v));
   };
 
-  VT pre[kXYZStageF];
+  VT pre[NSTG];
   auto issue = [&](uint32_t z) {
     const VT* src = volc + (size_t)z * vsz;
 #pragma unroll
-    for (int k = 0; k < kXYZStageF; k++) {
+    for (int k = 0; k < NSTG; k++) {
       if (xyz_off<XYZ_FWD_OFF>(1, nseg)) {
         pre[k] = (VT)(((pk[k] + z * 40503u) * 2654435761u) >> 20);
       }
@@ -914,15 +910,20 @@
     uint32_t RSv = RS, tidv = tid;
     asm volatile("" : "+s"(RSv), "+v"(tidv));
 #pragma unroll
-    for (int k = 0; k < kXYZStageF; k++)
+    for (int k = 0; k < NSTG; k++)
       asm volatile("" : "+v"(pk[k]));
 #pragma unroll
-    for (int k = 0; k < kXYZPosF; k++)
+    for (int k = 0; k < NPOS; k++)
       asm volatile("" : "+v"(srow[k]), "+v"(ooff[k]));
+    if constexpr (!L2) {
+#pragma unroll
+      for (int k = 0; k < NPOS; k++)
+        asm volatile("" : "+v"(boff[k]));
+    }
     double* A = sm + ((z & 1) ? bufN : 0u);
     double* B = sm + ((z & 1) ? 0u : bufN);
 #pragma unroll
-    for (int k = 0; k < kXYZStageF; k++)
+    for (int k = 0; k < NSTG; k++)
       if ((tid + (uint32_t)k * kXYZThreadsF) < nstage)
         xyz_put(A + (pk[k] >> 27) * RSv, pk[k] & 0xfffu, cx, (double)pre[k] - mean);
     if (z + 1 < zEnd)
@@ -939,13 +940,13 @@
       continue;
     if (z & 1) {
 #pragma unroll
-      for (int k = 0; k < kXYZPosF; k++)
+      for (int k = 0; k < NPOS; k++)
         if ((tid + (uint32_t)k * kXYZThreadsF) < npos)
           sxo[k] = A[(srow[k] >> 16) * RSv + 4 + (srow[k] & 0xffffu)];
     }
     else {
 #pragma unroll
-      for (int k = 0; k < kXYZPosF; k++) {
+      for (int k = 0; k < NPOS; k++) {
         if ((tid + (uint32_t)k * kXYZThreadsF) >= npos)
           continue;
         const double v = A[(srow[k] >> 16) * RSv + 4 + (srow[k] & 0xffffu)];
@@ -969,7 +970,7 @@
     }
   }
 #pragma unroll
-  for (int k = 0; k < kXYZPosF; k++) {
+  for (int k = 0; k < NPOS; k++) {
     if ((tid + (uint32_t)k * kXYZThreadsF) >= npos || seg + 1 != nseg)
       continue;
     if ((cz & 1) == 0) {
@@ -1000,17 +1001,54 @@
     for (int d = 32; d > 0; d >>= 1)
       vmax = fmax(vmax, __shfl_xor(vmax, d, 64));
     if ((tid & 63) == 0 && vmax > 0.0)
-      atomicMax(reinterpret_cast<unsigned long long*>(&st[c].maxabs),
+      atomicMax(reinterpret_cast<unsigned long long*>(&stc->maxabs),
                 (unsigned long long)__double_as_longlong(vmax));
   }
 }
 
-template <int IO, bool SG, bool kCrop = false>
-__global__ void __launch_bounds__(kXYZThreadsI) __attribute__((amdgpu_waves_per_eu(kXYZThreadsI / 256, kXYZThreadsI / 256)))
-k_lift_xyz_inv(const double* vals, size_t valsStride, uint32_t cx, uint32_t cy, uint32_t cz, LiftConsts K,
-               const CoderState* st, void* volume, VolDesc vd, const GeomOf<kCrop>* geom, LiftFuse F, uint32_t nseg)
+template <int IO>
+__global__ void __launch_bounds__(kXYZThreadsF) __attribute__((amdgpu_waves_per_eu(kXYZThreadsF / 256, kXYZThreadsF / 256)))
+k_lift_xyz_fwd(double* vals, size_t valsStride, uint32_t cx, uint32_t cy, uint32_t cz, LiftConsts K,
+               CoderState* st, const void* volume, VolDesc vd, const ChunkGeom* geom, int wantMax,
+               uint32_t in0, uint32_t in1, uint32_t in2, uint32_t nseg, double* box, size_t boxStride)
 {
   static_assert(IO == 1 || IO == 2, "float or double volume");
+  using VT = typename std::conditional<IO == 1, float, double>::type;
+  const uint32_t c = blockIdx.y;
+  if (st[c].is_const != 0)
+    return;
+  const VT* vol = reinterpret_cast<const VT*>(volume);
+  const size_t vsy = vd.dims[0], vsz = (size_t)vd.dims[0] * vd.dims[1];
+  const VT* volc = vol + ((size_t)geom[c].org[2] * vsz + (size_t)geom[c].org[1] * vsy + geom[c].org[0]);
+  xyz_fwd_body<VT, kXYZPosF, kXYZStageF, false>(vals + c * valsStride, cx, (size_t)cx * cy, cx, cy, cz, K, st + c, volc, vsy, vsz,
+                                                 st[c].mean, wantMax, in0, in1, in2, nseg, box ? box + c * boxStride : nullptr);
+}
+
+constexpr int kL2MaxRow = 128;
+constexpr int kL2PosF = (kXYZRows * kL2MaxRow + kXYZThreadsF - 1) / kXYZThreadsF;
+constexpr int kL2StageF = (kXYZStaged * kL2MaxRow + kXYZThreadsF - 1) / kXYZThreadsF;
+constexpr int kL2PosI = (kXYZStaged * kL2MaxRow + kXYZThreadsI - 1) / kXYZThreadsI;
+__global__ void __launch_bounds__(kXYZThreadsF) __attribute__((amdgpu_waves_per_eu(kXYZThreadsF / 256, kXYZThreadsF / 256)))
+k_lift2_fwd(const double* box, size_t boxStride, double* vals, size_t valsStride, uint32_t orow, size_t oslice, uint32_t cx,
+            uint32_t cy, uint32_t cz, LiftConsts K, CoderState* st, int wantMax, uint32_t in0, uint32_t in1, uint32_t in2,
+            uint32_t nseg)
+{
+  const uint32_t c = blockIdx.y;
+  if (st[c].is_const != 0)
+    return;
+  xyz_fwd_body<double, kL2PosF, kL2StageF, true>(vals + c * valsStride, orow, oslice, cx, cy, cz, K, st + c, box + c * boxStride,
+                                                  (size_t)cx, (size_t)cx * cy, 0.0, wantMax, in0, in1, in2, nseg, nullptr);
+}
+
+template <int IO, bool SG, bool kCrop, int NPOS, bool L2>
+__device__ __forceinline__ void xyz_inv_body(const double* vals, size_t valsStride, uint32_t cx, uint32_t cy, uint32_t cz,
+                                             const LiftConsts& K, const CoderState* st, void* volume, const VolDesc& vd,
+                                             const GeomOf<kCrop>* geom, const LiftFuse& F, uint32_t nseg, uint32_t qrowL2,
+                                             size_t qsliceL2)
+{
+  static_assert(IO == 1 || IO == 2, "float or double volume");
+  static_assert(!L2 || (IO == 2 && !kCrop), "the second level writes doubles into a box");
+  constexpr int NGRP = NPOS < kXYZGroupI ? NPOS : kXYZGroupI;
   using VT = typename std::conditional<IO == 1, float, double>::type;
   const uint32_t c = blockIdx.y;
   const uint32_t tid = threadIdx.x;
@@ -1037,18 +1075,20 @@
       return;
     wy1 -= y0;
   }
-  else
+  else if constexpr (!L2)
     volc = vol + ((size_t)geom[c].org[2] * vsz + (size_t)geom[c].org[1] * vsy + geom[c].org[0]);
   auto crop_row = [&](uint32_t z, uint32_t r) -> VT* { return vol + crop_addr(cg, vd, cg.lo[0], y0 + r, z); };
   (void)crop_row;
   const double* buf = vals + c * valsStride;
-  const size_t sliceN = (size_t)cx * cy;
+  const uint32_t qrow = L2 ? qrowL2 : cx;
+  const size_t sliceN = L2 ? qsliceL2 : (size_t)cx * cy;
   const uint32_t bufx = F.bufx ? F.bufx : cx;
   const size_t bufSlice = (size_t)bufx * (F.bufy ? F.bufy : cy);
   const double mean = st[c].mean;
   const uint32_t lane = tid & 63u, nwaves = kXYZThreadsI / 64;
   const uint32_t wave = (uint32_t)__builtin_amdgcn_readfirstlane((int)(tid >> 6));
 
+  if constexpr (!L2) {
   if (st[c].is_const != 0) {
     if constexpr (kCrop) {
       const uint32_t w = cg.hi[0] - cg.lo[0], nr = wy1 - wy0;
@@ -1062,12 +1102,13 @@
         volc[(size_t)z * vsz + (size_t)(y0 + k / cx) * vsy + k % cx] = (VT)mean;
     return;
   }
+  }
 
   const uint32_t npos = (uint32_t)kXYZStaged * cx;
-  uint32_t pk[kXYZPosI];
+  uint32_t pk[NPOS];
   uint32_t innerMask = 0;
 #pragma unroll
-  for (int k = 0; k < kXYZPosI; k++) {
+  for (int k = 0; k < NPOS; k++) {
     const uint32_t q = tid + (uint32_t)k * kXYZThreadsI;
     const uint32_t j = q / cx, x = q - j * cx, y = reflect_index((int)y0 - kXYHalo + (int)j, (int)cy);
     const uint32_t drow = (y & 1) ? ye + (y >> 1) : (y >> 1), dcol = (x & 1) ? xe + (x >> 1) : (x >> 1);
@@ -1089,7 +1130,7 @@
   auto fetch = [&](int k, uint32_t zp) -> double {
     const uint32_t y = (pk[k] >> 12) & 0x7fffu, x = pk[k] & 0xfffu;
     const uint32_t drow = (y & 1) ? ye + (y >> 1) : (y >> 1), dcol = (x & 1) ? xe + (x >> 1) : (x >> 1);
-    const size_t idx = (size_t)zp * sliceN + drow * cx + dcol;
+    const size_t idx = (size_t)zp * sliceN + drow * qrow + dcol;
     const bool inBox = ((innerMask >> k) & 1u) && zp < F.inner[2];
     if (!dequant && !inBox && F.bufx)
       return 0.0;
@@ -1109,9 +1150,9 @@
     asm volatile("" : "+v"(p));
     (sm + (flip ? bufN : 0u))[(p >> 27) * RS + 4 + (p & 0xfffu)] = v;
   };
-  auto stage_all = [&](const double (&v)[kXYZPosI]) {
-#pragma unroll
-    for (int k = 0; k < kXYZPosI; k++)
+  auto stage_all = [&](const double (&v)[NPOS]) {
+#pragma unroll
+    for (int k = 0; k < NPOS; k++)
       if ((tid + (uint32_t)k * kXYZThreadsI) < npos)
         stage(k, v[k]);
   };
@@ -1172,9 +1213,9 @@
     }
   };
 
-  double o1p[kXYZPosI], e1p[kXYZPosI], o2p[kXYZPosI], e2p[kXYZPosI];
-#pragma unroll
-  for (int k = 0; k < kXYZPosI; k++)
+  double o1p[NPOS], e1p[NPOS], o2p[NPOS], e2p[NPOS];
+#pragma unroll
+  for (int k = 0; k < NPOS; k++)
     o1p[k] = e1p[k] = o2p[k] = e2p[k] = 0.0;
   const uint32_t npairs = cz / 2;
   auto zstep = [&](int k, uint32_t m, bool mine, bool active, double E, double O) {
@@ -1193,20 +1234,20 @@
     e1p[k] = e1;
   };
 #if XYZ_INV_PREFETCH == 2
-  uint32_t* myPre = reinterpret_cast<uint32_t*>(sm + 2 * (size_t)bufN) + (size_t)wave * (kXYZPosI * 2 * 64);
+  uint32_t* myPre = reinterpret_cast<uint32_t*>(sm + 2 * (size_t)bufN) + (size_t)wave * (NPOS * 2 * 64);
   const uint32_t* sign32 = reinterpret_cast<const uint32_t*>(sign);
   const uint32_t* mNew32 = reinterpret_cast<const uint32_t*>(mNew);
   const uint32_t* mOld32 = reinterpret_cast<const uint32_t*>(mOld);
   uint32_t activeMask = 0;
 #pragma unroll
-  for (int k = 0; k < kXYZPosI; k++)
+  for (int k = 0; k < NPOS; k++)
     if ((tid + (uint32_t)k * kXYZThreadsI) < npos)
       activeMask |= 1u << k;
     else
       pk[k] = pk[0];
   uint32_t boxAny = 0;
 #pragma unroll
-  for (int k = 0; k < kXYZPosI; k++)
+  for (int k = 0; k < NPOS; k++)
     boxAny |= __ballot((innerMask >> k) & 1u) != 0ull ? 1u << k : 0u;
   boxAny = (uint32_t)__builtin_amdgcn_readfirstlane((int)boxAny);
   auto pos_off = [&](int k, uint32_t& drow, uint32_t& dcol) {
@@ -1216,11 +1257,11 @@
   };
   const bool fastLoads = dequant && F.inner[2] <= ze && (!SG || scheme != 0);
   uint32_t boxLds = 0, boxSlot0 = 0;
-  uint32_t* boxRows = reinterpret_cast<uint32_t*>(sm + 2 * (size_t)bufN) + (size_t)nwaves * (kXYZPosI * 2 * 64);
+  uint32_t* boxRows = reinterpret_cast<uint32_t*>(sm + 2 * (size_t)bufN) + (size_t)nwaves * (NPOS * 2 * 64);
   if (SG && fastLoads) {
     uint32_t reg = 0;
 #pragma unroll
-    for (int k = 0; k < kXYZPosI; k++) {
+    for (int k = 0; k < NPOS; k++) {
       const uint64_t inb = __ballot((innerMask >> k) & 1u), act = __ballot((activeMask >> k) & 1u);
       if (inb == 0x5555555555555555ull && act == ~0ull && (cx & 63u) == 0)
         reg |= 1u << k;
@@ -1237,7 +1278,7 @@
       total += v;
     }
     XYZ_LDS_BARRIER();
-    if (total <= (uint32_t)kXYZBoxSlots && reg == (1u << kXYZPosI) - 1u) {
+    if (total <= (uint32_t)kXYZBoxSlots && reg == (1u << NPOS) - 1u) {
       boxLds = reg;
       boxSlot0 = (uint32_t)__builtin_amdgcn_readfirstlane((int)before);
     }
@@ -1248,7 +1289,7 @@
       return;
     if (SG && boxLds != 0 && m < F.inner[2]) {
 #pragma unroll
-      for (int k = 0; k < kXYZPosI; k++) {
+      for (int k = 0; k < NPOS; k++) {
         uint32_t drow, dcol;
         pos_off(k, drow, dcol);
         const uint32_t x0h = ((pk[k] & 0xfffu) - lane) >> 1;
@@ -1257,10 +1298,10 @@
       }
     }
 #pragma unroll
-    for (int k = 0; k < kXYZPosI; k++) {
+    for (int k = 0; k < NPOS; k++) {
       uint32_t drow, dcol;
       pos_off(k, drow, dcol);
-      const uint32_t off = drow * cx + dcol;
+      const uint32_t off = drow * qrow + dcol;
       __builtin_amdgcn_global_load_lds(coef + ((size_t)m * sliceN + off), myPre + (k * 2) * 64, 4, 0, 0);
       __builtin_amdgcn_global_load_lds(coef + ((size_t)(ze + m) * sliceN + off), myPre + (k * 2 + 1) * 64, 4, 0, 0);
     }
@@ -1271,7 +1312,7 @@
   for (uint32_t m = mFirst; m < mB; m++) {
     const bool mine = m >= mA;
 #pragma unroll
-    for (int k = 0; k < kXYZPosI; k++)
+    for (int k = 0; k < NPOS; k++)
       asm volatile("" : "+v"(pk[k]));
 #if XYZ_INV_PREFETCH == 2
     if (SG && fastLoads) {
@@ -1280,7 +1321,7 @@
       const bool zOn = !xyz_off<XYZ_INV_OFF>(8, nseg);
       if (zOn && boxWave && boxLds != 0) {
 #pragma unroll
-        for (int k = 0; k < kXYZPosI; k++) {
+        for (int k = 0; k < NPOS; k++) {
           const double lo = sg_value(myPre[(k * 2) * 64 + lane]);
           const double hi = sg_value(myPre[(k * 2 + 1) * 64 + lane]);
           const double bxv = reinterpret_cast<const double*>(myBox + k * 64)[lane >> 1];
@@ -1289,15 +1330,15 @@
       }
       else if (zOn) {
 #pragma unroll
-      for (int g = 0; g < kXYZPosI; g += kXYZGroupI) {
+      for (int g = 0; g < NPOS; g += NGRP) {
         __builtin_amdgcn_sched_barrier(0);
-        double bx[kXYZGroupI];
+        double bx[NGRP];
         uint32_t boxm = 0;
         if (boxWave) {
 #pragma unroll
-          for (int kk = 0; kk < kXYZGroupI; kk++) {
+          for (int kk = 0; kk < NGRP; kk++) {
             const int k = g + kk;
-            if (k >= kXYZPosI)
+            if (k >= NPOS)
               continue;
             uint32_t drow, dcol;
             pos_off(k, drow, dcol);
@@ -1307,9 +1348,9 @@
           }
         }
 #pragma unroll
-        for (int kk = 0; kk < kXYZGroupI; kk++) {
+        for (int kk = 0; kk < NGRP; kk++) {
           const int k = g + kk;
-          if (k >= kXYZPosI)
+          if (k >= NPOS)
             continue;
           const double lo = sg_value(myPre[(k * 2) * 64 + lane]);
           const double hi = sg_value(myPre[(k * 2 + 1) * 64 + lane]);
@@ -1325,20 +1366,20 @@
     else if (!SG && fastLoads) {
       asm volatile("s_waitcnt vmcnt(0)" ::: "memory");
 #pragma unroll
-      for (int g = 0; g < kXYZPosI; g += kXYZGroupI) {
+      for (int g = 0; g < NPOS; g += NGRP) {
         __builtin_amdgcn_sched_barrier(0);
-        constexpr int NV = 2 * kXYZGroupI;
+        constexpr int NV = 2 * NGRP;
         uint32_t sgw[NV], mnw[NV], mow[NV], cv[NV], shv[NV], boxm = 0;
-        double bx[kXYZGroupI];
+        double bx[NGRP];
 #pragma unroll
         for (int j = 0; j < NV; j++) {
           const int k = g + j / 2;
-          if (k >= kXYZPosI)
+          if (k >= NPOS)
             continue;
           const uint32_t zp = (j & 1) ? ze + m : m;
           uint32_t drow, dcol;
           pos_off(k, drow, dcol);
-          const size_t idx = (size_t)zp * sliceN + drow * cx + dcol;
+          const size_t idx = (size_t)zp * sliceN + drow * qrow + dcol;
           sgw[j] = sign32[idx >> 5];
           mnw[j] = mNew32[idx >> 5];
           mow[j] = mOld32[idx >> 5];
@@ -1353,14 +1394,14 @@
         double val[NV];
 #pragma unroll
         for (int j = 0; j < NV; j++) {
-          if (g + j / 2 >= kXYZPosI)
+          if (g + j / 2 >= NPOS)
             continue;
           const double dq = dequant_masks(rule, cv[j], mnw[j], mow[j], sgw[j], shv[j]);
           val[j] = ((j & 1) == 0 && ((boxm >> j) & 1u)) ? bx[j / 2] : dq;
         }
 #pragma unroll
-        for (int kk = 0; kk < kXYZGroupI; kk++)
-          if (g + kk < kXYZPosI)
+        for (int kk = 0; kk < NGRP; kk++)
+          if (g + kk < NPOS)
             zstep(g + kk, m, mine, ((activeMask >> (g + kk)) & 1u) != 0, val[2 * kk], val[2 * kk + 1]);
       }
       __builtin_amdgcn_sched_barrier(0);
@@ -1372,7 +1413,7 @@
 #endif
     {
 #pragma unroll
-      for (int k = 0; k < kXYZPosI; k++) {
+      for (int k = 0; k < NPOS; k++) {
         if ((k % 3) == 0)
           __builtin_amdgcn_sched_barrier(0);
         if ((tid + (uint32_t)k * kXYZThreadsI) >= npos)
@@ -1392,9 +1433,9 @@
     return;
   if ((cz & 1) == 0) {
     const uint32_t M = npairs - 1;
-    double outC[kXYZPosI];
-#pragma unroll
-    for (int k = 0; k < kXYZPosI; k++) {
+    double outC[NPOS];
+#pragma unroll
+    for (int k = 0; k < NPOS; k++) {
       outC[k] = 0.0;
       if ((tid + (uint32_t)k * kXYZThreadsI) >= npos)
         continue;
@@ -1412,9 +1453,9 @@
   }
   else {
     const uint32_t M = npairs;
-    double outC[kXYZPosI], outD[kXYZPosI];
-#pragma unroll
-    for (int k = 0; k < kXYZPosI; k++) {
+    double outC[NPOS], outD[NPOS];
+#pragma unroll
+    for (int k = 0; k < NPOS; k++) {
       outC[k] = outD[k] = 0.0;
       if ((tid + (uint32_t)k * kXYZThreadsI) >= npos)
         continue;
@@ -1437,6 +1478,26 @@
     stage_all(outD);
     finish_slice(2 * M);
   }
+}
+
+template <int IO, bool SG, bool kCrop = false>
+__global__ void __launch_bounds__(kXYZThreadsI) __attribute__((amdgpu_waves_per_eu(kXYZThreadsI / 256, kXYZThreadsI / 256)))
+k_lift_xyz_inv(const double* vals, size_t valsStride, uint32_t cx, uint32_t cy, uint32_t cz, LiftConsts K,
+               const CoderState* st, void* volume, VolDesc vd, const GeomOf<kCrop>* geom, LiftFuse F, uint32_t nseg)
+{
+  xyz_inv_body<IO, SG, kCrop, kXYZPosI, false>(vals, valsStride, cx, cy, cz, K, st, volume, vd, geom, F, nseg, 0u, 0);
+}
+
+template <bool SG>
+__global__ void __launch_bounds__(kXYZThreadsI) __attribute__((amdgpu_waves_per_eu(kXYZThreadsI / 256, kXYZThreadsI / 256)))
+k_lift2_inv(const double* vals, size_t valsStride, uint32_t cx, uint32_t cy, uint32_t cz, LiftConsts K, const CoderState* st,
+            double* out, size_t outStride, LiftFuse F, uint32_t nseg, uint32_t qrow, size_t qslice)
+{
+  if (st[blockIdx.y].is_const != 0)
+    return;
+  const VolDesc vd{{cx, cy, cz}};
+  xyz_inv_body<2, SG, false, kL2PosI, true>(vals, valsStride, cx, cy, cz, K, st, out + blockIdx.y * outStride, vd, nullptr, F, nseg,
+                                            qrow, qslice);
 }
 
 
@@ -1836,11 +1897,21 @@
          (size_t)kXYZRows * cdims[0] <= (size_t)kXYZPosF * kXYZThreadsF && cdims[0] < 4096 && cdims[1] < 32768;
 }
 
+static uint32_t xyz_segments(uint32_t ntile, uint32_t nchunks, uint32_t cz)
+{
+  uint32_t nseg = 1;
+  while (nseg < 4 && (size_t)ntile * nchunks * nseg < 512 && cz / (2 * nseg) >= 24)
+    nseg *= 2;
+  return nseg;
+}
+
 int launch_lift_xyz(hipStream_t stream, bool forward, double* vals, size_t valsStride, uint32_t nchunks,
                     const uint32_t cdims[3], CoderState* st, int io, void* volume, VolDesc vd,
-                    const ChunkGeom* geom, const LiftFuse* fuse, const CropGeom* crop)
+                    const ChunkGeom* geom, const LiftFuse* fuse, const CropGeom* crop, double* box, size_t boxStride)
 {
   if (!lift_xyz_applicable(cdims) || (io != 1 && io != 2) || (crop && forward))
+    return -1;
+  if (box && !forward)
     return -1;
   const LiftFuse F = fuse ? *fuse : LiftFuse{};
   size_t smem = 2 * (size_t)kXYZStaged * xyz_row_stride(cdims[0]) * sizeof(double);
@@ -1860,19 +1931,17 @@
         return -1;
   }
   const uint32_t ntile = (cdims[1] + kXYZRows - 1) / kXYZRows;
-  uint32_t nseg = 1;
-  while (nseg < 4 && (size_t)ntile * nchunks * nseg < 512 && cdims[2] / (2 * nseg) >= 24)
-    nseg *= 2;
+  const uint32_t nseg = xyz_segments(ntile, nchunks, cdims[2]);
   const dim3 grid(ntile * nseg, nchunks);
   const LiftConsts K = lift_consts();
   if (forward) {
     const int wantMax = F.mode == 1 ? 1 : 0;
     if (io == 1)
       LAUNCH_K((k_lift_xyz_fwd<1>), grid, dim3(kXYZThreadsF), smem, stream, vals, valsStride, cdims[0], cdims[1],
-               cdims[2], K, st, volume, vd, geom, wantMax, F.inner[0], F.inner[1], F.inner[2], nseg);
+               cdims[2], K, st, volume, vd, geom, wantMax, F.inner[0], F.inner[1], F.inner[2], nseg, box, boxStride);
     else
       LAUNCH_K((k_lift_xyz_fwd<2>), grid, dim3(kXYZThreadsF), smem, stream, vals, valsStride, cdims[0], cdims[1],
-               cdims[2], K, st, volume, vd, geom, wantMax, F.inner[0], F.inner[1], F.inner[2], nseg);
+               cdims[2], K, st, volume, vd, geom, wantMax, F.inner[0], F.inner[1], F.inner[2], nseg, box, boxStride);
   }
   else {
     const bool sg = F.mode == 2 && F.src.coefSigned != 0;
@@ -1907,6 +1976,68 @@
 #undef XYZ_INV_LAUNCH
 #undef XYZ_CROP_LAUNCH
   }
+  HIP_CHECK(hipGetLastError());
+  return 0;
+}
+
+bool lift2_applicable(const uint32_t region[3])
+{
+  return lift_xyz_applicable(region) && region[0] <= (uint32_t)kL2MaxRow;
+}
+
+static uint32_t lift2_segments(uint32_t ntile, uint32_t nchunks, uint32_t cz)
+{
+  static const int forced = tune_getenv("SPERR_HIP_L2_NSEG") ? atoi(tune_getenv("SPERR_HIP_L2_NSEG")) : 0;
+  if ((forced == 1 || forced == 2 || forced == 4) && cz / (2 * (uint32_t)forced) >= 8)
+    return (uint32_t)forced;
+  return xyz_segments(ntile, nchunks, cz);
+}
+
+int launch_lift2_fwd(hipStream_t stream, const double* box, size_t boxStride, double* vals, size_t valsStride,
+                     uint32_t nchunks, const uint32_t cdims[3], const uint32_t region[3], CoderState* st,
+                     const LiftFuse* fuse)
+{
+  if (!lift2_applicable(region) || !box || region[0] > cdims[0] || region[1] > cdims[1] || region[2] > cdims[2])
+    return -1;
+  const LiftFuse F = fuse ? *fuse : LiftFuse{};
+  const size_t smem = 2 * (size_t)kXYZStaged * xyz_row_stride(region[0]) * sizeof(double);
+  if (set_max_dyn_lds(reinterpret_cast<const void*>(&k_lift2_fwd), 160 * 1024))
+    return -1;
+  const uint32_t ntile = (region[1] + kXYZRows - 1) / kXYZRows;
+  const uint32_t nseg = lift2_segments(ntile, nchunks, region[2]);
+  LAUNCH_K(k_lift2_fwd, dim3(ntile * nseg, nchunks), dim3(kXYZThreadsF), smem, stream, box, boxStride, vals, valsStride,
+           cdims[0], (size_t)cdims[0] * cdims[1], region[0], region[1], region[2], lift_consts(), st, F.mode == 1 ? 1 : 0,
+           F.inner[0], F.inner[1], F.inner[2], nseg);
+  HIP_CHECK(hipGetLastError());
+  return 0;
+}
+
+int launch_lift2_inv(hipStream_t stream, const double* box, size_t boxStride, double* out, size_t outStride,
+                     uint32_t nchunks, const uint32_t cdims[3], const uint32_t region[3], const CoderState* st,
+                     const LiftFuse* fuse)
+{
+  if (!lift2_applicable(region) || !box || !out || !fuse || fuse->mode != 2 || region[0] > cdims[0] ||
+      region[1] > cdims[1] || region[2] > cdims[2] || outStride < (size_t)region[0] * region[1] * region[2])
+    return -1;
+  LiftFuse F = *fuse;
+  F.noMean = 1;
+  size_t smem = 2 * (size_t)kXYZStaged * xyz_row_stride(region[0]) * sizeof(double);
+#if XYZ_INV_PREFETCH == 2
+  smem += (size_t)kXYZThreadsI * kL2PosI * 2 * sizeof(uint32_t) + (size_t)kXYZBoxSlots * 64 * sizeof(uint32_t);
+#endif
+  if (set_max_dyn_lds(reinterpret_cast<const void*>(&k_lift2_inv<false>), 160 * 1024) ||
+      set_max_dyn_lds(reinterpret_cast<const void*>(&k_lift2_inv<true>), 160 * 1024))
+    return -1;
+  const uint32_t ntile = (region[1] + kXYZRows - 1) / kXYZRows;
+  const uint32_t nseg = lift2_segments(ntile, nchunks, region[2]);
+  const dim3 grid(ntile * nseg, nchunks);
+  const LiftConsts K = lift_consts();
+  if (F.src.coefSigned != 0)
+    LAUNCH_K((k_lift2_inv<true>), grid, dim3(kXYZThreadsI), smem, stream, box, boxStride, region[0], region[1], region[2], K,
+             st, out, outStride, F, nseg, cdims[0], (size_t)cdims[0] * cdims[1]);
+  else
+    LAUNCH_K((k_lift2_inv<false>), grid, dim3(kXYZThreadsI), smem, stream, box, boxStride, region[0], region[1], region[2], K,
+             st, out, outStride, F, nseg, cdims[0], (size_t)cdims[0] * cdims[1]);
   HIP_CHECK(hipGetLastError());
   return 0;
 }
```

New measurement: 70.18 GB/s, median of 6. +1.6%, better.
